# Lagrange-Labs/mapreduce-plonky2

Measured on AMD Instinct MI355X. Metric: leaf proofs/sec (whole node) + NTT GB/s vs HBM peak, 2^20-row table build, 1/2/4/8 GPU, higher is better.
Workload: dtype u64 (Goldilocks field)

## Files before the change

mapreduce-plonky2_amd/csrc/fri.hip:

```cpp
#include "fri.h"
#include "poseidon_wave.cuh"

namespace mp2g {

template <int V>
__device__ void ch_duplex(ChState& c) {
  for (u32 i = 0; i < c.n_in; i++) c.state[i] = c.in[i];
  c.n_in = 0;
  u64 s[12];
#pragma unroll
  for (int i = 0; i < 12; i++) s[i] = c.state[i];
  perm<V>(s);
#pragma unroll
  for (int i = 0; i < 12; i++) c.state[i] = s[i];
#pragma unroll
  for (int i = 0; i < 8; i++) c.out[i] = s[i];
  c.n_out = 8;
}
template <int V>
__global__ void ch_kernel(ChState* st, u32 B, const u64* obs, u64 obs_bstride, u32 n_obs, u64* out, u64 out_bstride, u32 n_get) {
  u32 b = blockIdx.x * blockDim.x + threadIdx.x;
  if (b >= B) return;
  ChState c = st[b];
  const u64* o = obs + b * obs_bstride;
  for (u32 i = 0; i < n_obs; i++) {
    c.n_out = 0;
    c.in[c.n_in++] = o[i];
    if (c.n_in == 8) ch_duplex<V>(c);
  }
  u64* dst = out + b * out_bstride;
  for (u32 i = 0; i < n_get; i++) {
    if (c.n_in || !c.n_out) ch_duplex<V>(c);
    dst[i] = c.out[--c.n_out];
  }
  st[b] = c;
}
__global__ void __launch_bounds__(64) ch_wave_kernel(ChState* st, u32 B, const u64* obs, u64 obs_bstride, u32 n_obs, u64* out,
                                                     u64 out_bstride, u32 n_get) {
  const u32 gid = blockIdx.x * blockDim.x + threadIdx.x;
  const u32 braw = gid >> 4, l = gid & 15;
  const bool active = braw < B;
  const u32 b = active ? braw : B - 1;
  ChState* c = st + b;
  u64 x = l < 12 ? c->state[l] : 0;
  u64 inb = l < 8 ? c->in[l] : 0, outb = l < 8 ? c->out[l] : 0;
  u32 n_in = c->n_in, n_out = c->n_out;
  const u64* o = obs + b * obs_bstride;
  auto duplex = [&]() {
    if (l < n_in) x = inb;
    n_in = 0;
    x = wp2_perm(x, (int)l);
    outb = x;
    n_out = 8;
  };
  for (u32 i = 0; i < n_obs; i++) {
    u64 e = o[i];
    n_out = 0;
    if (l == n_in) inb = e;
    if (++n_in == 8) duplex();
  }
  u64* dst = out + b * out_bstride;
  for (u32 i = 0; i < n_get; i++) {
    if (n_in || !n_out) duplex();
    --n_out;
    if (active && l == n_out) dst[i] = outb;
  }
  if (!active) return;
  if (l < 12) c->state[l] = x;
  if (l < 8) { c->in[l] = inb; c->out[l] = outb; }
  if (l == 0) { c->n_in = n_in; c->n_out = n_out; }
}
__global__ void ch_init_kernel(ChState* st, u32 B) {
  u32 b = blockIdx.x * blockDim.x + threadIdx.x;
  if (b >= B) return;
  ChState c;
  for (int i = 0; i < 12; i++) c.state[i] = 0;
  for (int i = 0; i < 8; i++) { c.in[i] = 0; c.out[i] = 0; }
  c.n_in = c.n_out = 0;
  st[b] = c;
}
hipError_t challenger_init(hipStream_t s, ChState* st, u32 B) {
  hipLaunchKernelGGL(ch_init_kernel, dim3((B + 63) / 64), dim3(64), 0, s, st, B);
  return hipGetLastError();
}
hipError_t challenger_step(hipStream_t s, int variant, ChState* st, u32 B, const u64* obs, u64 obs_bstride, u32 n_obs,
                           u64* out, u64 out_bstride, u32 n_get) {
  if (variant == MP2G_POSEIDON2)
    hipLaunchKernelGGL(ch_wave_kernel, dim3((B * 16 + 63) / 64), dim3(64), 0, s, st, B, obs, obs_bstride, n_obs, out, out_bstride, n_get);
  else
    hipLaunchKernelGGL((ch_kernel<MP2G_POSEIDON>), dim3((B + 63) / 64), dim3(64), 0, s, st, B, obs, obs_bstride, n_obs, out, out_bstride, n_get);
  return hipGetLastError();
}

#define EP_RUN 16
__global__ void __launch_bounds__(256) ext_powers_kernel(const u64* __restrict__ x, u64 x_bstride, u64 scale, u32 count,
                                                         u64* __restrict__ out, u64 out_bstride) {
  const u32 b = blockIdx.y, e0 = blockIdx.x * 256 * EP_RUN + threadIdx.x;
  if (e0 >= count) return;
  const gl2 xb = gl2_scale(gl2_make(x[b * x_bstride], x[b * x_bstride + 1]), scale);
  const gl2 step = gl2_pow(xb, 256);
  gl2 pw = gl2_pow(xb, e0);
  u64* o = out + b * out_bstride;
  for (u32 r = 0, e = e0; r < EP_RUN && e < count; r++, e += 256) {
    o[e] = pw.a;
    o[count + e] = pw.b;
    pw = gl2_mul(pw, step);
  }
}
static hipError_t ext_powers(hipStream_t s, u32 B, const u64* x, u64 x_bstride, u64 scale, u32 count, u64* out, u64 out_bstride) {
  hipLaunchKernelGGL(ext_powers_kernel, dim3((count + 256 * EP_RUN - 1) / (256 * EP_RUN), B), dim3(256), 0, s, x, x_bstride, scale, count, out,
                     out_bstride);
  return hipGetLastError();
}

#define OP_POLYS 4
__global__ void __launch_bounds__(256) openings_kernel(FriShape sh, const u64* __restrict__ zpw, u64 zpw_bstride, u64* out ) {
  const u32 b = blockIdx.y, t = threadIdx.x;
  const u32 n = 1u << sh.log_n, n_open = sh.n_polys + sh.zs_count + sh.lookup_count;
  const u32 blocks0 = (sh.n_polys + OP_POLYS - 1) / OP_POLYS;
  const bool shifted = blockIdx.x >= blocks0;
  const u32 j0 = shifted ? sh.n_polys + (blockIdx.x - blocks0) * OP_POLYS : blockIdx.x * OP_POLYS;
  const u32 nq = min(OP_POLYS, (shifted ? n_open : sh.n_polys) - j0);
  const u64* pa = zpw + b * zpw_bstride + (shifted ? 2 * (u64)n : 0);
  const u64* pb = pa + n;
  const u64* c[OP_POLYS];
#pragma unroll
  for (u32 q = 0; q < OP_POLYS; q++) {
    u32 o, p;
    const u32 j = j0 + (q < nq ? q : 0);
    if (shifted) fri_batch_poly(sh, 1, j - sh.n_polys, o, p);
    else fri_batch_poly(sh, 0, j, o, p);
    c[q] = sh.o[o].coeffs + b * sh.o[o].coeff_bstride + ((u64)p << sh.log_n);
  }
  gl_cols sa[OP_POLYS], sb[OP_POLYS];
  for (u32 i = t; i < n; i += 256) {
    const u64 za = pa[i], zb = pb[i];
#pragma unroll
    for (u32 q = 0; q < OP_POLYS; q++)
      if (q < nq) {
        const u64 v = c[q][i];
        sa[q].add(v, za);
        sb[q].add(v, zb);
      }
  }
  __shared__ u64 ra[OP_POLYS][256], rb[OP_POLYS][256];
#pragma unroll
  for (u32 q = 0; q < OP_POLYS; q++) { ra[q][t] = sa[q].value(); rb[q][t] = sb[q].value(); }
  __syncthreads();
  for (u32 s = 128; s > 0; s >>= 1) {
    if (t < s)
#pragma unroll
      for (u32 q = 0; q < OP_POLYS; q++) { ra[q][t] = gl_add(ra[q][t], ra[q][t + s]); rb[q][t] = gl_add(rb[q][t], rb[q][t + s]); }
    __syncthreads();
  }
  if (t < nq) {
    u64* d = out + ((u64)b * n_open + j0 + t) * 2;
    d[0] = ra[t][0]; d[1] = rb[t][0];
  }
}

__global__ void __launch_bounds__(256) compose_kernel(FriShape sh, const u64* __restrict__ apw, u64 apw_bstride, u32 apw_len, u64* comp) {
  const u32 n = 1u << sh.log_n;
  const u32 i = blockIdx.x * 256 + threadIdx.x, b = blockIdx.y, batch = blockIdx.z;
  if (i >= n) return;
  const u64* pa = apw + b * apw_bstride;
  const u64* pb = pa + apw_len;
  gl_cols sa, sb;
  u32 m = 0;
  const u32 zo = sh.zs_oracle, wz = sh.o[zo].w - sh.lookup_count;
  auto run = [&](u32 o, u32 first, u32 count) {
    const u64* base = sh.o[o].coeffs + b * sh.o[o].coeff_bstride + i;
    for (u32 p = first; p < first + count; p++, m++) {
      const u64 v = base[(u64)p << sh.log_n];
      sa.add(v, pa[m]);
      sb.add(v, pb[m]);
    }
  };
  if (batch == 0) {
    for (u32 o = 0; o < sh.n_oracles; o++) run(o, 0, o == zo ? wz : sh.o[o].w);
  } else {
    run(zo, 0, sh.zs_count);
  }
  if (sh.lookup_count) run(zo, wz, sh.lookup_count);
  u64* d = comp + (((u64)b * 2 + batch) * 2) * n;
  d[i] = sa.value();
  d[n + i] = sb.value();
}

__global__ void __launch_bounds__(1024) divide_kernel(u32 log_n, const u64* zeta, u64 zeta_bstride, const u64* comp, u64* quot) {
  const u32 n = 1u << log_n, batch = blockIdx.x, b = blockIdx.y, t = threadIdx.x;
  const u32 T = n < 1024 ? n : 1024, S = n / T;
  gl2 z = gl2_make(zeta[b * zeta_bstride], zeta[b * zeta_bstride + 1]);
  if (batch == 1) z = gl2_scale(z, gl_root_of_unity(log_n));
  const u64* c0 = comp + (((u64)b * 2 + batch) * 2) * n;
  const u64* c1 = c0 + n;
  u64* q0 = quot + (((u64)b * 2 + batch) * 2) * n;
  u64* q1 = q0 + n;
  __shared__ u64 la[1024], lb[1024];
  gl2 L = gl2_make(0, 0);
  if (t < T) {
    for (int k = (int)S - 1; k >= 0; k--) {
      L = gl2_mul(L, z);
      L.a = gl_add(L.a, c0[t * S + k]);
      L.b = gl_add(L.b, c1[t * S + k]);
    }
  }
  la[t] = 0; lb[t] = 0;
  __syncthreads();
  if (t < T && t >= 1) { la[t - 1] = L.a; lb[t - 1] = L.b; }
  __syncthreads();
  gl2 zp = gl2_pow(z, S);
  for (u32 d = 1; d < T; d <<= 1) {
    gl2 add = gl2_make(0, 0);
    if (t + d < T) add = gl2_mul(zp, gl2_make(la[t + d], lb[t + d]));
    __syncthreads();
    if (t < T) { la[t] = gl_add(la[t], add.a); lb[t] = gl_add(lb[t], add.b); }
    __syncthreads();
    zp = gl2_mul(zp, zp);
  }
  if (t < T) {
    gl2 s = gl2_make(la[t], lb[t]);
    for (int k = (int)S - 1; k >= 0; k--) {
      u32 i = t * S + k;
      s = gl2_mul(s, z);
      s.a = gl_add(s.a, c0[i]);
      s.b = gl_add(s.b, c1[i]);
      if (i >= 1) { q0[i - 1] = s.a; q1[i - 1] = s.b; }
    }
    if (t == T - 1) { q0[n - 1] = 0; q1[n - 1] = 0; }
  }
}
__global__ void __launch_bounds__(256) combine_kernel(u32 log_n, u32 zs_count, const u64* __restrict__ apw, u64 apw_bstride, u32 apw_len,
                                                      const u64* quot, u64* final_poly) {
  const u32 n = 1u << log_n, i = blockIdx.x * 256 + threadIdx.x, b = blockIdx.y;
  if (i >= n) return;
  const gl2 sh = gl2_make(apw[b * apw_bstride + zs_count], apw[b * apw_bstride + apw_len + zs_count]);
  const u64* q = quot + (u64)b * 4 * n;
  gl2 r = gl2_add(gl2_mul(gl2_make(q[i], q[n + i]), sh), gl2_make(q[2 * n + i], q[3 * n + i]));
  final_poly[(u64)b * 2 * n + i] = r.a;
  final_poly[(u64)b * 2 * n + n + i] = r.b;
}

template <int AB>
__global__ void __launch_bounds__(256) fold_values_kernel(u32 log_m, const u64* in, u64 in_bstride, u64* out, u64 out_bstride,
                                                            const u64* beta, u64 beta_bstride, u64 shift_inv, u64 w_m_inv, u64 arity_inv) {
  constexpr int A = 1 << AB;
  const u32 m = 1u << log_m, chunks = m >> AB;
  const u32 c = blockIdx.x * 256 + threadIdx.x, b = blockIdx.y;
  if (c >= chunks) return;
  const u64* v0 = in + b * in_bstride + ((u64)c << AB);
  const u64* v1 = v0 + m;
  gl2 x[A];
#pragma unroll
  for (int k = 0; k < A; k++) x[k] = gl2_make(v0[k], v1[k]);
  const u64 wA_inv = gl_pow(w_m_inv, m >> AB);
#pragma unroll
  for (int s = 1; s <= AB; s++) {
    const int mm = 1 << s, h = mm >> 1;
    u64 wstep = wA_inv;
    for (int e = s; e < AB; e++) wstep = gl_sqr(wstep);
    u64 w = 1;
#pragma unroll
    for (int j = 0; j < h; j++) {
#pragma unroll
      for (int k = 0; k < A; k += mm) {
        gl2 t = j == 0 ? x[k + j + h] : gl2_scale(x[k + j + h], w);
        gl2 u = x[k + j];
        x[k + j] = gl2_add(u, t);
        x[k + j + h] = gl2_sub(u, t);
      }
      w = gl_mul(w, wstep);
    }
  }
  u64 x0_inv = gl_mul(shift_inv, gl_pow(w_m_inv, bitrev32(c, log_m - AB)));
  gl2 g = gl2_scale(gl2_make(beta[b * beta_bstride], beta[b * beta_bstride + 1]), x0_inv);
  gl2 acc = x[A - 1];
#pragma unroll
  for (int j = A - 2; j >= 0; j--) acc = gl2_add(gl2_mul(acc, g), x[j]);
  acc = gl2_scale(acc, arity_inv);
  u64* o = out + b * out_bstride;
  o[c] = acc.a;
  o[chunks + c] = acc.b;
}
__global__ void __launch_bounds__(256) fold_coeffs_kernel(u32 n_out, u32 ab, const u64* in, u64 in_bstride, u32 n_in, u64* out, u64 out_bstride,
                                                            const u64* beta, u64 beta_bstride, int aos_out) {
  const u32 i = blockIdx.x * 256 + threadIdx.x, b = blockIdx.y;
  if (i >= n_out) return;
  const u32 A = 1u << ab;
  const u64* c0 = in + b * in_bstride + ((u64)i << ab);
  const u64* c1 = c0 + n_in;
  gl2 be = gl2_make(beta[b * beta_bstride], beta[b * beta_bstride + 1]);
  gl2 acc = gl2_make(0, 0);
  for (int j = (int)A - 1; j >= 0; j--) acc = gl2_add(gl2_mul(acc, be), gl2_make(c0[j], c1[j]));
  u64* o = out + b * out_bstride;
  if (aos_out) { o[2 * i] = acc.a; o[2 * i + 1] = acc.b; }
  else { o[i] = acc.a; o[n_out + i] = acc.b; }
}
__global__ void soa_to_aos_kernel(u32 n, const u64* in, u64 in_bstride, u32 n_in, u64* out, u64 out_bstride) {
  const u32 i = blockIdx.x * blockDim.x + threadIdx.x, b = blockIdx.y;
  if (i >= n) return;
  out[b * out_bstride + 2 * i] = in[b * in_bstride + i];
  out[b * out_bstride + 2 * i + 1] = in[b * in_bstride + n_in + i];
}

#define POW_THREADS 256
#define POW_STRIDE 16
template <int V>
__global__ void __launch_bounds__(POW_THREADS) pow_kernel(const ChState* st, u32 bits, unsigned long long* witness) {
  const u32 b = blockIdx.y;
  const ChState& c = st[b];
  unsigned long long* wit = witness + (u64)b * POW_STRIDE;
  __shared__ unsigned long long s_best;
  u64 base[12];
#pragma unroll
  for (int i = 0; i < 12; i++) base[i] = c.state[i];
  const u32 pos = c.n_in;
#pragma unroll
  for (int i = 0; i < 8; i++)
    if ((u32)i < pos) base[i] = c.in[i];
  const u64 stride = (u64)gridDim.x * blockDim.x;
  for (u64 cand = (u64)blockIdx.x * blockDim.x + threadIdx.x;; cand += stride) {
    if (threadIdx.x == 0) s_best = atomicMin(wit, ~0ull);
    __syncthreads();
    const unsigned long long best = s_best;
    __syncthreads();
    if (cand - threadIdx.x > best) break;
    u64 s[12];
#pragma unroll
    for (int i = 0; i < 12; i++) s[i] = base[i];
#pragma unroll
    for (int i = 0; i < 8; i++)
      if ((u32)i == pos) s[i] = cand;
    perm<V>(s);
    if (cand < GL_P && (bits == 0 || (s[7] >> (64 - bits)) == 0)) atomicMin(wit, (unsigned long long)cand);
  }
}
__global__ void fill_u64_kernel(u64* p, u64 v, u32 n) {
  u32 i = blockIdx.x * blockDim.x + threadIdx.x;
  if (i < n) p[i] = v;
}

__global__ void __launch_bounds__(256) query_kernel(FriShape sh, FriLayers ly, FriProofLayout L, const u64* chal ,
                                                      u64 chal_bstride, u64* proof) {
  const u32 q = blockIdx.x, b = blockIdx.y, t = threadIdx.x;
  const u32 lg = L.lg;
  const u64 N = (u64)1 << lg;
  u64 x = chal[b * chal_bstride + q] % N;
  u64* const qs = proof + b * L.proof_words + L.q_off + q * L.q_words;
  auto siblings = [&](u64* o, const u64* lv, u32 clg, u32 n_sib, u64 x) {
    for (u32 e = t; e < n_sib * 4; e += 256) {
      u32 l = e >> 2, k = e & 3;
      u64 off = 0;
      for (u32 j = 0; j < l; j++) off += (u64)4 << (clg - j);
      o[e] = lv[off + 4 * ((x >> l) ^ 1) + k];
    }
  };
  for (u32 oi = 0; oi < sh.n_oracles; oi++) {
    const OracleRef& r = sh.o[oi];
    u64* o = qs + L.leaf_off[oi];
    const u64* vals = r.values + b * r.value_bstride;
    for (u32 p = t; p < r.w; p += 256) o[p] = vals[(u64)p * N + x];
    siblings(o + r.w, r.levels + b * r.level_bstride, lg, L.n_sib[oi], x);
  }
  u32 clg = lg;
  for (u32 li = 0; li < ly.n_layers; li++) {
    const u32 ab = ly.arity_bits[li], A = 1u << ab, p = sh.n_oracles + li;
    const u64 m = (u64)1 << clg;
    x >>= ab;
    clg -= ab;
    u64* o = qs + L.leaf_off[p];
    const u64* v = ly.values[li] + b * ly.value_bstride[li];
    for (u32 e = t; e < 2 * A; e += 256) o[e] = v[(e & 1) * m + (x << ab) + (e >> 1)];
    siblings(o + 2 * A, ly.levels[li] + b * ly.level_bstride[li], clg, L.n_sib[p], x);
  }
}
__global__ void copy_rows_kernel(const u64* src, u64 src_bstride, u64* dst, u64 dst_bstride, u32 words) {
  u32 i = blockIdx.x * blockDim.x + threadIdx.x, b = blockIdx.y;
  if (i < words) dst[b * dst_bstride + i] = src[b * src_bstride + i];
}

__global__ void bind_pi_kernel(u64* wires, u64 wires_bstride, u64 n, u32 row, const u64* pi_hash, u32 B) {
  u32 t = blockIdx.x * blockDim.x + threadIdx.x;
  if (t < 4 * B) wires[(t >> 2) * wires_bstride + (u64)(t & 3) * n + row] = pi_hash[t];
}

#define HIPCHK(x) do { hipError_t e_ = (x); if (e_ != hipSuccess) return e_; } while (0)

hipError_t fri_openings(hipStream_t s, const FriShape& sh, u32 B, const u64* zeta, u64 zeta_bstride, u64* zpw, u64* out) {
  const u32 n = 1u << sh.log_n, n_shifted = sh.zs_count + sh.lookup_count;
  HIPCHK(ext_powers(s, B, zeta, zeta_bstride, 1, n, zpw, 4 * (u64)n));
  if (n_shifted) HIPCHK(ext_powers(s, B, zeta, zeta_bstride, gl_root_of_unity(sh.log_n), n, zpw + 2 * (u64)n, 4 * (u64)n));
  const u32 blocks = (sh.n_polys + OP_POLYS - 1) / OP_POLYS + (n_shifted + OP_POLYS - 1) / OP_POLYS;
  hipLaunchKernelGGL(openings_kernel, dim3(blocks, B), dim3(256), 0, s, sh, zpw, 4 * (u64)n, out);
  return hipGetLastError();
}
hipError_t fri_final_poly(hipStream_t s, const FriShape& sh, u32 B, const u64* alpha, u64 alpha_bstride, const u64* zeta, u64 zeta_bstride,
                          u64* apw, u64* comp, u64* quot, u64* final_poly) {
  const u32 n = 1u << sh.log_n, apw_len = fri_alpha_powers_len(sh);
  HIPCHK(ext_powers(s, B, alpha, alpha_bstride, 1, apw_len, apw, 2 * (u64)apw_len));
  hipLaunchKernelGGL(compose_kernel, dim3((n + 255) / 256, B, 2), dim3(256), 0, s, sh, apw, 2 * (u64)apw_len, apw_len, comp);
  hipLaunchKernelGGL(divide_kernel, dim3(2, B), dim3(1024), 0, s, sh.log_n, zeta, zeta_bstride, comp, quot);
  hipLaunchKernelGGL(combine_kernel, dim3((n + 255) / 256, B), dim3(256), 0, s, sh.log_n, sh.zs_count + sh.lookup_count, apw, 2 * (u64)apw_len,
                     apw_len, quot, final_poly);
  return hipGetLastError();
}
hipError_t fri_fold_values(hipStream_t s, u32 B, u32 log_m, u32 ab, const u64* in, u64 in_bstride, u64* out, u64 out_bstride,
                           const u64* beta, u64 beta_bstride, u64 shift) {
  const u32 chunks = (1u << log_m) >> ab;
  const u64 shift_inv = gl_inv(shift), w_m_inv = gl_inv(gl_root_of_unity(log_m)), a_inv = gl_inv((u64)1 << ab);
  dim3 g((chunks + 255) / 256, B), bl(256);
#define FV(N) case N: hipLaunchKernelGGL((fold_values_kernel<N>), g, bl, 0, s, log_m, in, in_bstride, out, out_bstride, beta, beta_bstride, shift_inv, w_m_inv, a_inv); break;
  switch (ab) { FV(1) FV(2) FV(3) FV(4) default: return hipErrorInvalidValue; }
#undef FV
  return hipGetLastError();
}
hipError_t fri_fold_coeffs(hipStream_t s, u32 B, u32 n_in, u32 ab, const u64* in, u64 in_bstride, u64* out, u64 out_bstride,
                           const u64* beta, u64 beta_bstride, bool aos_out) {
  const u32 n_out = n_in >> ab;
  hipLaunchKernelGGL(fold_coeffs_kernel, dim3((n_out + 255) / 256, B), dim3(256), 0, s, n_out, ab, in, in_bstride, n_in, out, out_bstride, beta, beta_bstride, aos_out ? 1 : 0);
  return hipGetLastError();
}
hipError_t fri_soa_to_aos(hipStream_t s, u32 B, u32 n, const u64* in, u64 in_bstride, u32 n_in, u64* out, u64 out_bstride) {
  hipLaunchKernelGGL(soa_to_aos_kernel, dim3((n + 255) / 256, B), dim3(256), 0, s, n, in, in_bstride, n_in, out, out_bstride);
  return hipGetLastError();
}
hipError_t fri_pow(hipStream_t s, int variant, const ChState* st, u32 B, u32 bits, u64* witness) {
  hipLaunchKernelGGL(fill_u64_kernel, dim3((B * POW_STRIDE + 63) / 64), dim3(64), 0, s, witness, ~(u64)0, B * POW_STRIDE);
  const u32 lanes = 1u << 19;
  u32 blocks = lanes / POW_THREADS / (B ? B : 1);
  if (blocks < 8) blocks = 8;
  if (blocks > 1024) blocks = 1024;
  dim3 g(blocks, B), bl(POW_THREADS);
  if (variant == MP2G_POSEIDON2) hipLaunchKernelGGL((pow_kernel<MP2G_POSEIDON2>), g, bl, 0, s, st, bits, (unsigned long long*)witness);
  else hipLaunchKernelGGL((pow_kernel<MP2G_POSEIDON>), g, bl, 0, s, st, bits, (unsigned long long*)witness);
  return hipGetLastError();
}
hipError_t fri_queries(hipStream_t s, const FriShape& sh, const FriLayers& ly, const FriProofLayout& L, u32 B, u32 num_queries,
                       const u64* chal, u64 chal_bstride, u64* proof) {
  if (!num_queries) return hipSuccess;
  hipLaunchKernelGGL(query_kernel, dim3(num_queries, B), dim3(256), 0, s, sh, ly, L, chal, chal_bstride, proof);
  return hipGetLastError();
}
hipError_t bind_public_inputs(hipStream_t s, u32 B, u64* wires, u64 wires_bstride, u64 n, u32 row, const u64* pi_hash) {
  hipLaunchKernelGGL(bind_pi_kernel, dim3((4 * B + 63) / 64), dim3(64), 0, s, wires, wires_bstride, n, row, pi_hash, B);
  return hipGetLastError();
}
hipError_t copy_rows(hipStream_t s, u32 B, const u64* src, u64 src_bstride, u64* dst, u64 dst_bstride, u32 words) {
  if (!words) return hipSuccess;
  hipLaunchKernelGGL(copy_rows_kernel, dim3((words + 255) / 256, B), dim3(256), 0, s, src, src_bstride, dst, dst_bstride, words);
  return hipGetLastError();
}
}
```

mapreduce-plonky2_amd/csrc/gates.h:

```cpp
#pragma once
#include "gl.cuh"
#include "mp2g.h"
namespace mp2g {
struct GateTable {
  u32 n_gates, num_selectors;
  u32 num_lookup_selectors;
  mp2g_gate g[MP2G_MAX_GATES];
};
const char* gate_table_check(const GateTable& t, u32 num_constants, u32 wires_w);
u32 gate_num_constraints(const mp2g_gate& g);
u32 gate_degree(const mp2g_gate& g);
inline u32 gate_filtered_degree(const mp2g_gate& g, u32 num_selectors) {
  return gate_degree(g) + (g.group_end - g.group_start - 1) + (num_selectors > 1 ? 1 : 0);
}
inline const char* gate_table_make(const mp2g_gate* gates, u32 n_gates, u32 num_selectors, u32 num_lookup_selectors, u32 num_constants,
                                   u32 wires_w, GateTable& out, u32* max_j) {
  out = GateTable{};
  out.n_gates = n_gates; out.num_selectors = num_selectors; out.num_lookup_selectors = num_lookup_selectors;
  u32 mj = 0;
  for (u32 i = 0; i < n_gates; i++) {
    out.g[i] = gates[i];
    const u32 k = gate_num_constraints(gates[i]);
    if (k > mj) mj = k;
  }
  if (max_j) *max_j = mj;
  return n_gates ? gate_table_check(out, num_constants, wires_w) : nullptr;
}
hipError_t gate_constraints_lde(hipStream_t s, u32 B, const GateTable& t, const u64* C, const u64* W, u64 w_bstride, u32 lg,
                                const u64* apw, u32 nc, const u64* pi_hash, u64* q);
hipError_t alpha_powers(hipStream_t s, u32 B, const u64* alphas, u64 al_bstride, u32 nc, u64* apw);
hipError_t gate_constraints_points(hipStream_t s, const GateTable& t, const u64* consts, const u64* wires, u64 npts, u32 max_j,
                                   const u64* pi_hash, u64* out);
hipError_t gate_constraints_points_batch(hipStream_t s, u32 B, const GateTable& t, const u64* consts, u64 c_bstride, const u64* wires,
                                         u64 w_bstride, u32 npts, u32 max_j, const u64* pi_hash, u64* out);
hipError_t gate_check(hipStream_t s, u32 B, const GateTable& t, const u64* consts, const u64* wires, u64 w_bstride, u64 npts,
                      const u64* pi_hash, u32* flags);
}
```

mapreduce-plonky2_amd/csrc/gates.hip:

```cpp
#include "gates.h"
#include "poseidon.cuh"
#include "coset_constants.h"

namespace mp2g {

u32 gate_num_constraints(const mp2g_gate& g) {
  switch (g.kind) {
    case MP2G_GATE_CONSTANT: return g.p0;
    case MP2G_GATE_PUBLIC_INPUT: return 4;
    case MP2G_GATE_ARITHMETIC: return g.p0;
    case MP2G_GATE_BASE_SUM: return 1 + g.p0;
    case MP2G_GATE_ARITHMETIC_EXT: case MP2G_GATE_MUL_EXT: return 2 * g.p0;
    case MP2G_GATE_POSEIDON2: case MP2G_GATE_POSEIDON: return 1 + 4 + 36 + 22 + 48 + 12;
    case MP2G_GATE_POSEIDON_MDS: return 24;
    case MP2G_GATE_COSET_INTERPOLATION: return 4 + 4 * (((1u << g.p0) - 2) / (g.p1 - 1));
    case MP2G_GATE_U32_ARITHMETIC: return 36 * g.p0;
    case MP2G_GATE_U32_RANGE_CHECK: return 17 * g.p0;
    case MP2G_GATE_U32_SUBTRACTION: return 19 * g.p0;
    case MP2G_GATE_U32_ADD_MANY: return 21 * g.p1;
    case MP2G_GATE_COMPARISON: return g.p1 ? 6 + 5 * g.p1 + (g.p0 + g.p1 - 1) / g.p1 : 0;
    case MP2G_GATE_EXPONENTIATION: return g.p0 + 1;
    case MP2G_GATE_REDUCING: case MP2G_GATE_REDUCING_EXT: return 2 * g.p0;
    case MP2G_GATE_RANDOM_ACCESS: return (g.p0 + 2) * g.p1 + g.p2;
    case MP2G_GATE_U32_INTERLEAVE: return 34 * g.p0;
    case MP2G_GATE_UNINTERLEAVE_TO_B32: case MP2G_GATE_UNINTERLEAVE_TO_U32: return 67 * g.p0;
    default: return 0;
  }
}
u32 gate_degree(const mp2g_gate& g) {
  switch (g.kind) {
    case MP2G_GATE_CONSTANT: case MP2G_GATE_PUBLIC_INPUT: return 1;
    case MP2G_GATE_ARITHMETIC: case MP2G_GATE_ARITHMETIC_EXT: case MP2G_GATE_MUL_EXT: return 3;
    case MP2G_GATE_BASE_SUM: return g.p1;
    case MP2G_GATE_POSEIDON2: case MP2G_GATE_POSEIDON: return 7;
    case MP2G_GATE_POSEIDON_MDS: return 1;
    case MP2G_GATE_COSET_INTERPOLATION: return g.p1;
    case MP2G_GATE_U32_ARITHMETIC: case MP2G_GATE_U32_RANGE_CHECK: case MP2G_GATE_U32_SUBTRACTION: case MP2G_GATE_U32_ADD_MANY: return 4;
    case MP2G_GATE_COMPARISON: return g.p1 ? 1u << ((g.p0 + g.p1 - 1) / g.p1) : 0;
    case MP2G_GATE_EXPONENTIATION: return 4;
    case MP2G_GATE_REDUCING: case MP2G_GATE_REDUCING_EXT: return 2;
    case MP2G_GATE_RANDOM_ACCESS: return g.p0 + 1;
    case MP2G_GATE_U32_INTERLEAVE: case MP2G_GATE_UNINTERLEAVE_TO_B32: case MP2G_GATE_UNINTERLEAVE_TO_U32: return 2;
    default: return 0;
  }
}
static void gate_footprint(const mp2g_gate& g, u32& wires, u32& consts) {
  wires = 0; consts = 0;
  switch (g.kind) {
    case MP2G_GATE_CONSTANT: wires = g.p0; consts = g.p0; break;
    case MP2G_GATE_PUBLIC_INPUT: wires = 4; break;
    case MP2G_GATE_ARITHMETIC: wires = 4 * g.p0; consts = 2; break;
    case MP2G_GATE_BASE_SUM: wires = 1 + g.p0; break;
    case MP2G_GATE_ARITHMETIC_EXT: wires = 8 * g.p0; consts = 2; break;
    case MP2G_GATE_MUL_EXT: wires = 6 * g.p0; consts = 1; break;
    case MP2G_GATE_POSEIDON2: case MP2G_GATE_POSEIDON: wires = 135; break;
    case MP2G_GATE_POSEIDON_MDS: wires = 48; break;
    case MP2G_GATE_COSET_INTERPOLATION: wires = 1 + 2 * (1u << g.p0) + 6 + 4 * (((1u << g.p0) - 2) / (g.p1 - 1)); break;
    case MP2G_GATE_U32_ARITHMETIC: wires = 38 * g.p0; break;
    case MP2G_GATE_U32_RANGE_CHECK: wires = 17 * g.p0; break;
    case MP2G_GATE_U32_SUBTRACTION: wires = 21 * g.p0; break;
    case MP2G_GATE_U32_ADD_MANY: wires = (g.p0 + 3 + 18) * g.p1; break;
    case MP2G_GATE_COMPARISON: wires = g.p1 ? 4 + 5 * g.p1 + (g.p0 + g.p1 - 1) / g.p1 + 1 : 0; break;
    case MP2G_GATE_EXPONENTIATION: wires = 2 * g.p0 + 2; break;
    case MP2G_GATE_REDUCING: wires = 6 + g.p0 + 2 * (g.p0 - 1); break;
    case MP2G_GATE_REDUCING_EXT: wires = 6 + 2 * g.p0 + 2 * (g.p0 - 1); break;
    case MP2G_GATE_RANDOM_ACCESS: wires = (2 + (1u << g.p0)) * g.p1 + g.p2 + g.p0 * g.p1; consts = g.p2; break;
    case MP2G_GATE_LOOKUP: wires = 2 * g.p0; break;
    case MP2G_GATE_LOOKUP_TABLE: wires = 3 * g.p0; break;
    case MP2G_GATE_U32_INTERLEAVE: wires = 34 * g.p0; break;
    case MP2G_GATE_UNINTERLEAVE_TO_B32: case MP2G_GATE_UNINTERLEAVE_TO_U32: wires = 67 * g.p0; break;
    default: break;
  }
}
const char* gate_table_check(const GateTable& t, u32 num_constants, u32 wires_w) {
  if (t.n_gates > MP2G_MAX_GATES) return "too many gates";
  if (t.num_selectors == 0 || t.num_selectors > num_constants) return "num_selectors must be in 1..num_constants";
  for (u32 i = 0; i < t.n_gates; i++) {
    const mp2g_gate& g = t.g[i];
    if (g.kind > MP2G_GATE_UNINTERLEAVE_TO_U32) return "unknown gate kind";
    if (g.kind >= MP2G_GATE_LOOKUP && g.p0 < 1) return "gate needs at least one slot / operation";
    if ((g.kind == MP2G_GATE_U32_ARITHMETIC || g.kind == MP2G_GATE_U32_RANGE_CHECK || g.kind == MP2G_GATE_U32_SUBTRACTION) && g.p0 < 1)
      return "u32 gate needs at least one operation";
    if (g.kind == MP2G_GATE_U32_ADD_MANY && (g.p0 < 1 || g.p0 > 16 || g.p1 < 1)) return "U32AddManyGate needs 1..16 addends and an operation";
    if (g.kind == MP2G_GATE_COMPARISON && (g.p1 < 1 || g.p0 < g.p1 || (g.p0 + g.p1 - 1) / g.p1 > 4))
      return "ComparisonGate needs num_chunks >= 1 and chunks of at most 4 bits";
    if (g.kind == MP2G_GATE_COSET_INTERPOLATION && (g.p0 < 2 || g.p0 > 5 || g.p1 < 2 || g.p1 > (1u << g.p0)))
      return "CosetInterpolationGate needs 2..5 subgroup bits and 2 <= degree <= 2^bits";
    if (g.kind == MP2G_GATE_BASE_SUM && (g.p1 < 2 || g.p0 < 1)) return "BaseSumGate needs base >= 2 and a limb";
    if ((g.kind == MP2G_GATE_REDUCING || g.kind == MP2G_GATE_REDUCING_EXT || g.kind == MP2G_GATE_EXPONENTIATION) && g.p0 < 1)
      return "gate needs at least one coefficient / power bit";
    if (g.kind == MP2G_GATE_RANDOM_ACCESS && (g.p0 < 1 || g.p0 > 6 || g.p1 < 1)) return "RandomAccessGate needs 1..6 bits and a copy";
    u32 w, c;
    gate_footprint(g, w, c);
    if (w > wires_w) return "gate needs more wires than the wires oracle has";
    if (t.num_selectors + t.num_lookup_selectors + c > num_constants) return "gate needs more constants than the preprocessed oracle has";
    if (g.selector_index >= t.num_selectors) return "selector_index out of range";
    if (!(g.group_start <= i && i < g.group_end && g.group_end <= t.n_gates)) return "gate is not inside its selector group";
    if (gate_num_constraints(g) > MP2G_MAX_GATE_CONSTRAINTS) return "gate has too many constraints";
  }
  return nullptr;
}

struct Alg { u64 a, b; };
GLD Alg alg_mul_addw(Alg x, Alg y, u64 y7, Alg z) {
  return Alg{gl_mul_addw(x.a, y.a, gl_mul_addw(x.b, y7, z.a)), gl_mul_addw(x.a, y.b, gl_mul_addw(x.b, y.a, z.b))};
}
GLD Alg alg_mulw(Alg x, Alg y, u64 y7) { return Alg{gl_mul_addw(x.a, y.a, gl_mulw(x.b, y7)), gl_mul_addw(x.a, y.b, gl_mulw(x.b, y.a))}; }
GLD Alg alg_scale_addw(Alg x, u64 s, Alg z) { return Alg{gl_mul_addw(x.a, s, z.a), gl_mul_addw(x.b, s, z.b)}; }

GLD u64 gl_subw(u64 a, u64 b) {
  u64 r;
  bool br = __builtin_sub_overflow(a, b, &r);
  return r - (br ? GL_EPS : 0);
}
typedef gl_cols LazySum;
template <int BITS, class WireF, class Emit>
GLD void ra_copy(WireF& wire, Emit& emit, u32 w0, u32 b0) {
  constexpr int VS = 1 << BITS;
  u64 bit[BITS], items[VS];
#pragma unroll
  for (int i = 0; i < BITS; i++) bit[i] = wire(b0 + i);
#pragma unroll
  for (int k = 0; k < VS; k++) items[k] = wire(w0 + 2 + k);
  const u64 access = wire(w0), claimed = wire(w0 + 1);
#pragma unroll
  for (int i = 0; i < BITS; i++) emit(gl_mul(bit[i], gl_sub(bit[i], 1)));
  u64 idx = 0;
#pragma unroll
  for (int i = BITS; i-- > 0;) idx = gl_add(gl_add(idx, idx), bit[i]);
  emit(gl_sub(idx, access));
#pragma unroll
  for (int i = 0; i < BITS; i++) {
#pragma unroll
    for (int k = 0; k < (VS >> (i + 1)); k++) items[k] = gl_mul_add(bit[i], gl_sub(items[2 * k + 1], items[2 * k]), items[2 * k]);
  }
  emit(gl_sub(items[0], claimed));
}

template <bool WEAK, class WireF, class ConstF, class Emit>
__device__ __forceinline__ void eval_gate(const mp2g_gate g, WireF wire, ConstF cst, const u64* __restrict__ pih, Emit emit) {
  auto diff = [](u64 s, u64 rc, u64 in) { return WEAK ? gl_subw(gl_addw(s, rc), in) : gl_sub(gl_add(gl_canon(s), rc), in); };
  auto diff0 = [](u64 s, u64 in) { return WEAK ? gl_subw(s, in) : gl_sub(gl_canon(s), in); };
  auto mulx = [](u64 a, u64 b) { return WEAK ? gl_mulw(a, b) : gl_mul(a, b); };
  auto subx = [](u64 a, u64 b) { return WEAK ? gl_subw(a, b) : gl_sub(a, b); };
  auto outx = [](u64 v) { return WEAK ? v : gl_canon(v); };
  auto load16 = [&](u32 first, u32 count, u64(&buf)[16]) {
#pragma unroll
    for (u32 k = 0; k < 16; k++) buf[k] = k < count ? wire(first + k) : 0;
  };
  auto range4 = [&](u64 limb) {
    const u64 z = mulx(limb, gl_sub(limb, 3));
    return mulx(z, WEAK ? gl_addw(z, 2) : gl_add(z, 2));
  };
  auto horner4 = [](u64 acc, u64 limb) {
    if (!WEAK) return gl_add(gl_mul_small(acc, 4), limb);
    return gl_addw(gl_reduce96w(acc << 2, acc >> 62), limb);
  };
  auto emit_alg = [&](Alg d) { emit(outx(d.a)); emit(outx(d.b)); };
  auto alg_subx = [&](Alg x, Alg y) { return Alg{subx(x.a, y.a), subx(x.b, y.b)}; };
  switch (g.kind) {
    case MP2G_GATE_CONSTANT:
      for (u32 i = 0; i < g.p0; i++) emit(subx(cst(i), wire(i)));
      break;
    case MP2G_GATE_PUBLIC_INPUT:
      for (u32 i = 0; i < 4; i++) emit(subx(wire(i), pih[i]));
      break;
    case MP2G_GATE_ARITHMETIC: {
      const u64 n0 = gl_neg(cst(0)), n1 = gl_neg(cst(1));
      u64 lm[16];
      for (u32 i0 = 0; i0 < g.p0; i0 += 4) {
        const u32 cnt = g.p0 - i0 < 4 ? g.p0 - i0 : 4;
        load16(4 * i0, 4 * cnt, lm);
#pragma unroll
        for (u32 k = 0; k < 4; k++)
          if (k < cnt) emit(outx(gl_mul_addw(gl_mulw(lm[4 * k], lm[4 * k + 1]), n0, gl_mul_addw(lm[4 * k + 2], n1, lm[4 * k + 3]))));
      }
      break;
    }
    case MP2G_GATE_BASE_SUM: {
      u64 acc = 0, lm[16];
      for (u32 hi = g.p0; hi > 0;) {
        const u32 lo = hi > 16 ? hi - 16 : 0, cnt = hi - lo;
        load16(1 + lo, cnt, lm);
#pragma unroll
        for (int j = 15; j >= 0; j--)
          if ((u32)j < cnt) acc = gl_addw(gl_mul_small_w(acc, g.p1), lm[j]);
        hi = lo;
      }
      emit(subx(outx(acc), wire(0)));
      for (u32 lo = 0; lo < g.p0; lo += 16) {
        const u32 cnt = g.p0 - lo < 16 ? g.p0 - lo : 16;
        load16(1 + lo, cnt, lm);
#pragma unroll
        for (int j = 0; j < 16; j++) {
          if ((u32)j < cnt) {
            u64 pr = lm[j];
            for (u32 k = 1; k < g.p1; k++) pr = mulx(pr, subx(lm[j], k));
            emit(pr);
          }
        }
      }
      break;
    }
    case MP2G_GATE_ARITHMETIC_EXT: {
      const u64 n0 = gl_neg(cst(0)), n1 = gl_neg(cst(1));
      u64 lm[16];
      for (u32 i0 = 0; i0 < g.p0; i0 += 2) {
        const u32 cnt = g.p0 - i0 < 2 ? g.p0 - i0 : 2;
        load16(8 * i0, 8 * cnt, lm);
#pragma unroll
        for (u32 k = 0; k < 2; k++) {
          if (k < cnt) {
            const u64* w8 = lm + 8 * k;
            Alg m0{w8[0], w8[1]}, m1{w8[2], w8[3]}, ad{w8[4], w8[5]}, o{w8[6], w8[7]};
            emit_alg(alg_scale_addw(alg_mulw(m0, m1, gl_mul_small_w(m1.b, 7)), n0, alg_scale_addw(ad, n1, o)));
          }
        }
      }
      break;
    }
    case MP2G_GATE_MUL_EXT: {
      const u64 n0 = gl_neg(cst(0));
      u64 lm[16];
      for (u32 i0 = 0; i0 < g.p0; i0 += 2) {
        const u32 cnt = g.p0 - i0 < 2 ? g.p0 - i0 : 2;
        load16(6 * i0, 6 * cnt, lm);
#pragma unroll
        for (u32 k = 0; k < 2; k++) {
          if (k < cnt) {
            const u64* w6 = lm + 6 * k;
            Alg m0{w6[0], w6[1]}, m1{w6[2], w6[3]}, o{w6[4], w6[5]};
            emit_alg(alg_scale_addw(alg_mulw(m0, m1, gl_mul_small_w(m1.b, 7)), n0, o));
          }
        }
      }
      break;
    }
    case MP2G_GATE_POSEIDON2: {
      const u64 swap = wire(24);
      emit(gl_mul(swap, gl_sub(swap, 1)));
      u64 s[12];
#pragma unroll
      for (int i = 0; i < 4; i++) {
        u64 lhs = wire(i), rhs = wire(i + 4), delta = wire(25 + i);
        emit(gl_sub(gl_mul(swap, gl_sub(rhs, lhs)), delta));
        s[i] = gl_add(lhs, delta);
        s[i + 4] = gl_sub(rhs, delta);
      }
#pragma unroll
      for (int i = 8; i < 12; i++) s[i] = wire(i);
      p2_external(s);
#pragma unroll 1
      for (int r = 0; r < 4; r++) {
        if (r != 0) {
#pragma unroll
          for (int i = 0; i < 12; i++) {
            u64 in = wire(29 + 12 * (r - 1) + i);
            emit(diff(s[i], c_p2_ext[12 * r + i], in));
            s[i] = p2_sbox(in, 0);
          }
        } else {
#pragma unroll
          for (int i = 0; i < 12; i++) s[i] = p2_sbox(s[i], c_p2_ext[i]);
        }
        p2_external(s);
      }
      u64 nxt = wire(65);
#pragma unroll 1
      for (int r = 0; r < 22; r++) {
        const u64 in = nxt;
        if (r < 21) nxt = wire(65 + r + 1);
        emit(diff(s[0], c_p2_int[r], in));
        s[0] = p2_sbox(in, 0);
        p2_internal(s);
      }
#pragma unroll 1
      for (int r = 0; r < 4; r++) {
#pragma unroll
        for (int i = 0; i < 12; i++) {
          u64 in = wire(87 + 12 * r + i);
          emit(diff(s[i], c_p2_ext[12 * (4 + r) + i], in));
          s[i] = p2_sbox(in, 0);
        }
        p2_external(s);
      }
#pragma unroll
      for (int i = 0; i < 12; i++) emit(diff0(s[i], wire(12 + i)));
      break;
    }
    case MP2G_GATE_POSEIDON: {
      const u64 swap = wire(24);
      emit(gl_mul(swap, gl_sub(swap, 1)));
      u64 s[12];
#pragma unroll
      for (int i = 0; i < 4; i++) {
        u64 lhs = wire(i), rhs = wire(i + 4), delta = wire(25 + i);
        emit(gl_sub(gl_mul(swap, gl_sub(rhs, lhs)), delta));
        s[i] = gl_add(lhs, delta);
        s[i + 4] = gl_sub(rhs, delta);
      }
#pragma unroll
      for (int i = 8; i < 12; i++) s[i] = wire(i);
#pragma unroll 1
      for (int r = 0; r < 30; r++) {
        if (r >= 4 && r < 26) {
          u64 in = wire(65 + (r - 4));
          emit(diff(s[0], c_p_rc[12 * r], in));
          s[0] = p2_sbox(in, 0);
#pragma unroll
          for (int i = 1; i < 12; i++) s[i] = gl_addw(s[i], c_p_rc[12 * r + i]);
        } else if (r == 0) {
#pragma unroll
          for (int i = 0; i < 12; i++) s[i] = p2_sbox(s[i], c_p_rc[i]);
        } else {
          const int base = r < 4 ? 29 + 12 * (r - 1) : 87 + 12 * (r - 26);
#pragma unroll
          for (int i = 0; i < 12; i++) {
            u64 in = wire(base + i);
            emit(diff(s[i], c_p_rc[12 * r + i], in));
            s[i] = p2_sbox(in, 0);
          }
        }
        poseidon_mds(s);
      }
#pragma unroll
      for (int i = 0; i < 12; i++) emit(diff0(s[i], wire(12 + i)));
      break;
    }
    case MP2G_GATE_POSEIDON_MDS: {
      u64 s0[12], s1[12];
#pragma unroll
      for (int i = 0; i < 12; i++) { s0[i] = wire(2 * i); s1[i] = wire(2 * i + 1); }
      poseidon_mds(s0);
      poseidon_mds(s1);
#pragma unroll
      for (int i = 0; i < 12; i++) {
        emit(gl_sub(wire(24 + 2 * i), gl_canon(s0[i])));
        emit(gl_sub(wire(25 + 2 * i), gl_canon(s1[i])));
      }
      break;
    }
    case MP2G_GATE_COSET_INTERPOLATION: {
      const u32 npts = 1u << g.p0, deg = g.p1, nint = (npts - 2) / (deg - 1);
      const u32 w_pt = 1 + 2 * npts, w_val = w_pt + 2, w_int = w_val + 2, w_sh = w_int + 4 * nint;
      const Alg pt{wire(w_pt), wire(w_pt + 1)}, sh{wire(w_sh), wire(w_sh + 1)};
      emit_alg(alg_scale_addw(sh, gl_neg(wire(0)), pt));
      const u64 sh7 = gl_mul_small_w(sh.b, 7);
      const u64* xs = COSET_POINTS + MP2G_COSET_TABLE(g.p0);
      const u64* ws = COSET_WEIGHTS + MP2G_COSET_TABLE(g.p0);
      Alg ev{0, 0}, pr{1, 0};
      u32 start = 0, end = deg;
      for (u32 c = 0; c <= nint; c++) {
        for (u32 i = start; i < end; i++) {
          const u64 wi = ws[i];
          const Alg val{gl_mulw(wire(1 + 2 * i), wi), gl_mulw(wire(2 + 2 * i), wi)};
          const Alg term{subx(sh.a, xs[i]), sh.b};
          ev = alg_mul_addw(ev, term, sh7, alg_mulw(val, pr, gl_mul_small_w(pr.b, 7)));
          pr = alg_mulw(pr, term, sh7);
        }
        ev = Alg{gl_canon(ev.a), gl_canon(ev.b)};
        if (c == nint) break;
        pr = Alg{gl_canon(pr.a), gl_canon(pr.b)};
        Alg iev{wire(w_int + 2 * c), wire(w_int + 2 * c + 1)}, ipr{wire(w_int + 2 * (nint + c)), wire(w_int + 2 * (nint + c) + 1)};
        emit(subx(iev.a, ev.a)); emit(subx(iev.b, ev.b)); emit(subx(ipr.a, pr.a)); emit(subx(ipr.b, pr.b));
        ev = iev; pr = ipr;
        start = 1 + (deg - 1) * (c + 1);
        end = start + deg - 1 < npts ? start + deg - 1 : npts;
      }
      emit(subx(wire(w_val), ev.a)); emit(subx(wire(w_val + 1), ev.b));
      break;
    }
    case MP2G_GATE_U32_ARITHMETIC: {
      const u32 ops = g.p0;
      for (u32 i = 0; i < ops; i++) {
        const u32 b = 6 * i;
        const u64 computed = gl_mul_add(wire(b), wire(b + 1), wire(b + 2));
        const u64 lo = wire(b + 3), hi = wire(b + 4), inv = wire(b + 5);
        const u64 hi_not_max = gl_sub(gl_mul(inv, gl_sub(0xFFFFFFFFull, hi)), 1);
        emit(gl_mul(hi_not_max, lo));
        emit(gl_sub(gl_mul_add(hi, (u64)1 << 32, lo), computed));
        u64 clo = 0, chi = 0, lm[16];
        load16(6 * ops + 32 * i + 16, 16, lm);
#pragma unroll
        for (int j = 15; j >= 0; j--) { emit(range4(lm[j])); chi = horner4(chi, lm[j]); }
        load16(6 * ops + 32 * i, 16, lm);
#pragma unroll
        for (int j = 15; j >= 0; j--) { emit(range4(lm[j])); clo = horner4(clo, lm[j]); }
        emit(subx(clo, lo));
        emit(subx(chi, hi));
      }
      break;
    }
    case MP2G_GATE_U32_RANGE_CHECK: {
      const u32 k = g.p0;
      for (u32 i = 0; i < k; i++) {
        u64 lm[16];
        load16(k + 16 * i, 16, lm);
        u64 acc = 0;
#pragma unroll
        for (int j = 15; j >= 0; j--) acc = horner4(acc, lm[j]);
        emit(subx(acc, wire(i)));
#pragma unroll
        for (int j = 0; j < 16; j++) emit(range4(lm[j]));
      }
      break;
    }
    case MP2G_GATE_U32_SUBTRACTION: {
      const u32 ops = g.p0;
      for (u32 i = 0; i < ops; i++) {
        const u32 b = 5 * i;
        const u64 initial = gl_sub(gl_sub(wire(b), wire(b + 1)), wire(b + 2));
        const u64 res = wire(b + 3), bo = wire(b + 4);
        emit(gl_sub(res, gl_add(initial, gl_mul((u64)1 << 32, bo))));
        u64 comb = 0, lm[16];
        load16(5 * ops + 16 * i, 16, lm);
#pragma unroll
        for (int j = 15; j >= 0; j--) { emit(range4(lm[j])); comb = horner4(comb, lm[j]); }
        emit(subx(comb, res));
        emit(gl_mul(bo, gl_sub(1, bo)));
      }
      break;
    }
    case MP2G_GATE_U32_ADD_MANY: {
      const u32 na = g.p0, ops = g.p1, per = na + 3;
      for (u32 i = 0; i < ops; i++) {
        const u32 b = per * i;
        u64 computed = wire(b + na);
        for (u32 j = 0; j < na; j++) computed = gl_add(computed, wire(b + j));
        const u64 res = wire(b + na + 1), co = wire(b + na + 2);
        emit(gl_sub(gl_mul_add(co, (u64)1 << 32, res), computed));
        u64 cres = 0, ccar = 0, lm[16];
        {
          const u64 l17 = wire(per * ops + 18 * i + 17), l16 = wire(per * ops + 18 * i + 16);
          load16(per * ops + 18 * i, 16, lm);
          emit(range4(l17)); ccar = l17;
          emit(range4(l16)); ccar = horner4(ccar, l16);
        }
#pragma unroll
        for (int j = 15; j >= 0; j--) { emit(range4(lm[j])); cres = horner4(cres, lm[j]); }
        emit(subx(cres, res));
        emit(subx(ccar, co));
      }
      break;
    }
    case MP2G_GATE_COMPARISON: {
      const u32 nch = g.p1, cb = (g.p0 + nch - 1) / nch, cs = 1u << cb;
      const u32 o_fc = 4, o_sc = 4 + nch, o_ed = 4 + 2 * nch, o_ce = 4 + 3 * nch, o_iv = 4 + 4 * nch, o_bits = 4 + 5 * nch;
      u64 a1 = 0, a2 = 0;
      for (u32 i = nch; i-- > 0;) { a1 = gl_add(gl_mul_small(a1, cs), wire(o_fc + i)); a2 = gl_add(gl_mul_small(a2, cs), wire(o_sc + i)); }
      emit(gl_sub(a1, wire(0)));
      emit(gl_sub(a2, wire(1)));
      u64 msd = 0;
      for (u32 i = 0; i < nch; i++) {
        const u64 f = wire(o_fc + i), sc = wire(o_sc + i), ce = wire(o_ce + i), iv = wire(o_iv + i);
        u64 p1 = f, p2 = sc;
        for (u32 x = 1; x < cs; x++) { p1 = mulx(p1, gl_sub(f, x)); p2 = mulx(p2, gl_sub(sc, x)); }
        emit(p1);
        emit(p2);
        const u64 diff = gl_sub(sc, f);
        emit(gl_sub(gl_mul(diff, wire(o_ed + i)), gl_sub(1, ce)));
        emit(gl_mul(ce, diff));
        emit(gl_sub(iv, gl_mul(ce, msd)));
        msd = gl_add(iv, gl_mul(gl_sub(1, ce), diff));
      }
      const u64 msd_w = wire(3);
      emit(gl_sub(msd_w, msd));
      u64 bc = 0;
      for (u32 i = cb + 1; i-- > 0;) bc = gl_add(gl_add(bc, bc), wire(o_bits + i));
      for (u32 i = 0; i <= cb; i++) { const u64 bit = wire(o_bits + i); emit(gl_mul(bit, gl_sub(1, bit))); }
      emit(gl_sub(gl_add(cs, msd_w), bc));
      emit(gl_sub(wire(2), wire(o_bits + cb)));
      break;
    }
    case MP2G_GATE_EXPONENTIATION: {
      const u32 nb = g.p0;
      const u64 base = wire(0);
      u64 prev_int = 1;
      for (u32 i = 0; i < nb; i++) {
        u64 prev = i == 0 ? 1 : gl_mul(prev_int, prev_int);
        u64 bit = wire(1 + (nb - 1 - i));
        u64 mulby = gl_mul_add(bit, base, gl_sub(1, bit));
        u64 cur = wire(nb + 2 + i);
        emit(gl_sub(gl_mul(prev, mulby), cur));
        prev_int = cur;
      }
      emit(gl_sub(wire(nb + 1), prev_int));
      break;
    }
    case MP2G_GATE_REDUCING:
    case MP2G_GATE_REDUCING_EXT: {
      const u32 n = g.p0;
      const bool ext = g.kind == MP2G_GATE_REDUCING_EXT;
      const u32 start_accs = 6 + (ext ? 2 * n : n);
      Alg alpha{wire(2), wire(3)}, acc{wire(4), wire(5)};
      const u64 alpha7 = gl_mul_small_w(alpha.b, 7);
      for (u32 i = 0; i < n; i++) {
        Alg coeff = ext ? Alg{wire(6 + 2 * i), wire(7 + 2 * i)} : Alg{wire(6 + i), 0};
        Alg nxt = i == n - 1 ? Alg{wire(0), wire(1)} : Alg{wire(start_accs + 2 * i), wire(start_accs + 2 * i + 1)};
        emit_alg(alg_mul_addw(acc, alpha, alpha7, alg_subx(coeff, nxt)));
        acc = nxt;
      }
      break;
    }
    case MP2G_GATE_RANDOM_ACCESS: {
      const u32 bits = g.p0, copies = g.p1, extra = g.p2, vs = 1u << bits;
      const u32 routed = (2 + vs) * copies + extra;
      for (u32 c = 0; c < copies; c++) {
        const u32 w0 = (2 + vs) * c, b0 = routed + c * bits;
        switch (bits) {
          case 1: ra_copy<1>(wire, emit, w0, b0); break;
          case 2: ra_copy<2>(wire, emit, w0, b0); break;
          case 3: ra_copy<3>(wire, emit, w0, b0); break;
          case 4: ra_copy<4>(wire, emit, w0, b0); break;
          default: {
            u64 items[32];
            for (u32 i = 0; i < bits; i++) {
              u64 b = wire(b0 + i);
              emit(gl_mul(b, gl_sub(b, 1)));
            }
            u64 idx = 0;
            for (u32 i = bits; i-- > 0;) idx = gl_add(gl_add(idx, idx), wire(b0 + i));
            emit(gl_sub(idx, wire(w0)));
            {
              const u64 b = wire(b0);
              for (u32 k = 0; k < vs / 2; k++) {
                u64 x = wire(w0 + 2 + 2 * k), y = wire(w0 + 3 + 2 * k);
                items[k] = gl_mul_add(b, gl_sub(y, x), x);
              }
            }
            for (u32 i = 1, len = vs / 2; i < bits; i++, len >>= 1) {
              const u64 b = wire(b0 + i);
              for (u32 k = 0; k < len / 2; k++) items[k] = gl_mul_add(b, gl_sub(items[2 * k + 1], items[2 * k]), items[2 * k]);
            }
            emit(gl_sub(items[0], wire(w0 + 1)));
          }
        }
      }
      for (u32 i = 0; i < extra; i++) emit(gl_sub(cst(i), wire((2 + vs) * copies + i)));
      break;
    }
    case MP2G_GATE_U32_INTERLEAVE: {
      const u32 ops = g.p0;
      u64 bt[16];
      for (u32 i = 0; i < ops; i++) {
        u64 x = 0, xi = 0;
        for (u32 h = 0; h < 2; h++) {
          load16(2 * ops + 32 * i + 16 * h, 16, bt);
#pragma unroll
          for (int j = 0; j < 16; j++) {
            emit(mulx(bt[j], gl_sub(1, bt[j])));
            x = gl_add(gl_add(x, x), bt[j]);
            xi = gl_add(gl_mul_small(xi, 4), bt[j]);
          }
        }
        emit(gl_sub(x, wire(2 * i)));
        emit(gl_sub(xi, wire(2 * i + 1)));
      }
      break;
    }
    case MP2G_GATE_UNINTERLEAVE_TO_B32:
    case MP2G_GATE_UNINTERLEAVE_TO_U32: {
      const u32 ops = g.p0;
      const bool spread = g.kind == MP2G_GATE_UNINTERLEAVE_TO_B32;
      u64 bt[16];
      for (u32 i = 0; i < ops; i++) {
        u64 x = 0, ev = 0, od = 0;
        for (u32 h = 0; h < 4; h++) {
          load16(3 * ops + 64 * i + 16 * h, 16, bt);
#pragma unroll
          for (int j = 0; j < 16; j++) {
            emit(mulx(bt[j], gl_sub(1, bt[j])));
            x = gl_add(gl_add(x, x), bt[j]);
            u64& d = (j & 1) ? ev : od;
            d = gl_add(spread ? gl_mul_small(d, 4) : gl_add(d, d), bt[j]);
          }
        }
        emit(gl_sub(x, wire(3 * i)));
        emit(gl_sub(ev, wire(3 * i + 1)));
        emit(gl_sub(od, wire(3 * i + 2)));
      }
      break;
    }
    default: break;
  }
}

template <class ConstAll>
GLD u64 gate_filter(const GateTable& t, u32 gi, ConstAll call) {
  const mp2g_gate& g = t.g[gi];
  const u64 s = call(g.selector_index);
  u64 f = 1;
  for (u32 r = g.group_start; r < g.group_end; r++)
    if (r != gi) f = gl_mul(f, gl_sub(r, s));
  if (t.num_selectors > 1) f = gl_mul(f, gl_sub(0xFFFFFFFFull, s));
  return f;
}

template <u32 KIND>
__global__ void __launch_bounds__(256) gate_constraints_lde_kernel(mp2g_gate g, u32 gi, u32 num_selectors, u32 cst_off, u32 n_cons,
                                                                   const u64* __restrict__ C, const u64* __restrict__ W,
                                                                   u64 w_bstride, u32 lg, const u64* __restrict__ apw_tab,
                                                                   u32 nc, const u64* __restrict__ pi_hash,
                                                                   u64* __restrict__ q, int first) {
  __shared__ u64 apw[2][MP2G_MAX_GATE_CONSTRAINTS];
  const u64 N = (u64)1 << lg;
  const u32 p = blockIdx.x * 256 + threadIdx.x, b = blockIdx.y;
  for (u32 j = threadIdx.x; j < 2 * n_cons; j += 256) {
    const u32 a = j >= n_cons ? 1 : 0, e = j - a * n_cons;
    apw[a][e] = apw_tab[((u64)b * 2 + a) * MP2G_MAX_GATE_CONSTRAINTS + e];
  }
  __syncthreads();
  if (p >= N) return;
  g.kind = KIND;
  const u64* w = W + b * w_bstride + p;
  const u64* c = C + p;
  const u64* pih = pi_hash + 4 * b;
  auto wire = [&](u32 j) { return w[(u64)j << lg]; };
  auto cst = [&](u32 j) { return c[(u64)(cst_off + j) << lg]; };
  u64 f = 1;
  {
    const u64 s = c[(u64)g.selector_index << lg];
    for (u32 r = g.group_start; r < g.group_end; r++)
      if (r != gi) f = gl_mul(f, gl_sub(r, s));
    if (num_selectors > 1) f = gl_mul(f, gl_sub(0xFFFFFFFFull, s));
  }
  LazySum acc[2];
  u32 j = 0;
  eval_gate<true>(g, wire, cst, pih, [&](u64 v) {
#pragma unroll
    for (u32 a = 0; a < 2; a++) acc[a].add(v, apw[a][j]);
    j++;
  });
  const u32 i = bitrev32(p, lg);
  for (u32 a = 0; a < nc; a++) {
    u64 r = gl_mul(f, acc[a].value());
    u64* dst = q + (((u64)b * nc + a) << lg) + i;
    *dst = first ? r : gl_add(*dst, r);
  }
}

#define MP2G_MAX_LIGHT_GATES 12
struct LightGates {
  u32 n;
  mp2g_gate g[MP2G_MAX_LIGHT_GATES];
  u32 gi[MP2G_MAX_LIGHT_GATES];
};
static bool gate_is_light(const mp2g_gate& g) {
  switch (g.kind) {
    case MP2G_GATE_CONSTANT: case MP2G_GATE_PUBLIC_INPUT: case MP2G_GATE_ARITHMETIC: case MP2G_GATE_BASE_SUM:
    case MP2G_GATE_ARITHMETIC_EXT: case MP2G_GATE_MUL_EXT: return true;
    default: return false;
  }
}
__global__ void __launch_bounds__(256) gate_constraints_lde_light_kernel(LightGates lg_, u32 num_selectors, u32 cst_off, u32 max_cons,
                                                                         const u64* __restrict__ C, const u64* __restrict__ W,
                                                                         u64 w_bstride, u32 lg, const u64* __restrict__ apw_tab,
                                                                         u32 nc, const u64* __restrict__ pi_hash,
                                                                         u64* __restrict__ q, int first) {
  __shared__ u64 apw[2][MP2G_MAX_GATE_CONSTRAINTS];
  const u64 N = (u64)1 << lg;
  const u32 p = blockIdx.x * 256 + threadIdx.x, b = blockIdx.y;
  for (u32 j = threadIdx.x; j < 2 * max_cons; j += 256) {
    const u32 a = j >= max_cons ? 1 : 0, e = j - a * max_cons;
    apw[a][e] = apw_tab[((u64)b * 2 + a) * MP2G_MAX_GATE_CONSTRAINTS + e];
  }
  __syncthreads();
  if (p >= N) return;
  const u64* w = W + b * w_bstride + p;
  const u64* c = C + p;
  const u64* pih = pi_hash + 4 * b;
  auto wire = [&](u32 j) { return w[(u64)j << lg]; };
  auto cst = [&](u32 j) { return c[(u64)(cst_off + j) << lg]; };
  u64 total[2] = {0, 0};
  for (u32 k = 0; k < lg_.n; k++) {
    mp2g_gate g = lg_.g[k];
    const u32 gi = lg_.gi[k];
    u64 f = 1;
    {
      const u64 s = c[(u64)g.selector_index << lg];
      for (u32 r = g.group_start; r < g.group_end; r++)
        if (r != gi) f = gl_mul(f, gl_sub(r, s));
      if (num_selectors > 1) f = gl_mul(f, gl_sub(0xFFFFFFFFull, s));
    }
    LazySum acc[2];
    u32 j = 0;
    auto emit = [&](u64 v) {
#pragma unroll
      for (u32 a = 0; a < 2; a++) acc[a].add(v, apw[a][j]);
      j++;
    };
    switch (g.kind) {
#define LIGHT_CASE(K) case K: g.kind = K; eval_gate<true>(g, wire, cst, pih, emit); break;
      LIGHT_CASE(MP2G_GATE_CONSTANT)
      LIGHT_CASE(MP2G_GATE_PUBLIC_INPUT)
      LIGHT_CASE(MP2G_GATE_ARITHMETIC)
      LIGHT_CASE(MP2G_GATE_BASE_SUM)
      LIGHT_CASE(MP2G_GATE_ARITHMETIC_EXT)
      LIGHT_CASE(MP2G_GATE_MUL_EXT)
#undef LIGHT_CASE
      default: break;
    }
    for (u32 a = 0; a < nc; a++) total[a] = gl_add(total[a], gl_mul(f, acc[a].value()));
  }
  const u32 i = bitrev32(p, lg);
  for (u32 a = 0; a < nc; a++) {
    u64* dst = q + (((u64)b * nc + a) << lg) + i;
    *dst = first ? total[a] : gl_add(*dst, total[a]);
  }
}

__global__ void __launch_bounds__(256) gate_constraints_points_kernel(GateTable t, const u64* __restrict__ consts,
                                                                      const u64* __restrict__ wires, u64 npts, u32 max_j,
                                                                      const u64* __restrict__ pih, u64* __restrict__ out) {
  const u64 p = (u64)blockIdx.x * 256 + threadIdx.x;
  if (p >= npts) return;
  auto wire = [&](u32 j) { return wires[(u64)j * npts + p]; };
  auto call = [&](u32 j) { return consts[(u64)j * npts + p]; };
  const u32 ns = t.num_selectors + t.num_lookup_selectors;
  auto cst = [&](u32 j) { return consts[(u64)(ns + j) * npts + p]; };
  for (u32 j = 0; j < max_j; j++) out[(u64)j * npts + p] = 0;
  for (u32 gi = 0; gi < t.n_gates; gi++) {
    if (t.g[gi].kind == MP2G_GATE_NOOP) continue;
    const u64 f = gate_filter(t, gi, call);
    u32 j = 0;
    eval_gate<false>(t.g[gi], wire, cst, pih, [&](u64 v) {
      u64* o = out + (u64)j * npts + p;
      *o = gl_add(*o, gl_mul(f, v));
      j++;
    });
  }
}

__global__ void __launch_bounds__(256) gate_constraints_points_batch_kernel(GateTable t, u32 B, const u64* __restrict__ consts, u64 c_bstride,
                                                                            const u64* __restrict__ wires, u64 w_bstride, u32 npts,
                                                                            u32 max_j, const u64* __restrict__ pih, u64* __restrict__ out) {
  const u32 idx = blockIdx.x * 256 + threadIdx.x;
  if (idx >= B * npts) return;
  const u32 b = idx / npts, p = idx % npts;
  const u64* cb = consts + b * c_bstride;
  const u64* wb = wires + b * w_bstride;
  u64* ob = out + (u64)b * max_j * npts;
  auto wire = [&](u32 j) { return wb[(u64)j * npts + p]; };
  auto call = [&](u32 j) { return cb[(u64)j * npts + p]; };
  const u32 ns = t.num_selectors + t.num_lookup_selectors;
  auto cst = [&](u32 j) { return cb[(u64)(ns + j) * npts + p]; };
  for (u32 j = 0; j < max_j; j++) ob[(u64)j * npts + p] = 0;
  for (u32 gi = 0; gi < t.n_gates; gi++) {
    if (t.g[gi].kind == MP2G_GATE_NOOP) continue;
    const u64 f = gate_filter(t, gi, call);
    u32 j = 0;
    eval_gate<false>(t.g[gi], wire, cst, pih + 4 * b, [&](u64 v) {
      u64* o = ob + (u64)j * npts + p;
      *o = gl_add(*o, gl_mul(f, v));
      j++;
    });
  }
}

__global__ void __launch_bounds__(256) gate_check_kernel(GateTable t, const u64* __restrict__ consts, const u64* __restrict__ wires,
                                                         u64 w_bstride, u64 npts, const u64* __restrict__ pi_hash, u32* __restrict__ flags) {
  const u64 p = (u64)blockIdx.x * 256 + threadIdx.x;
  const u32 b = blockIdx.y;
  if (p >= npts) return;
  const u64* w = wires + b * w_bstride;
  auto wire = [&](u32 j) { return w[(u64)j * npts + p]; };
  auto call = [&](u32 j) { return consts[(u64)j * npts + p]; };
  const u32 ns = t.num_selectors + t.num_lookup_selectors;
  auto cst = [&](u32 j) { return consts[(u64)(ns + j) * npts + p]; };
  bool bad = false;
  for (u32 gi = 0; gi < t.n_gates; gi++) {
    if (t.g[gi].kind == MP2G_GATE_NOOP) continue;
    if (gate_filter(t, gi, call) == 0) continue;
    eval_gate<false>(t.g[gi], wire, cst, pi_hash + 4 * b, [&](u64 v) { bad |= v != 0; });
  }
  if (bad) atomicOr(&flags[b], 2u);
}
hipError_t gate_check(hipStream_t s, u32 B, const GateTable& t, const u64* consts, const u64* wires, u64 w_bstride, u64 npts,
                      const u64* pi_hash, u32* flags) {
  if (!npts || !B) return hipSuccess;
  hipLaunchKernelGGL(gate_check_kernel, dim3((u32)((npts + 255) / 256), B), dim3(256), 0, s, t, consts, wires, w_bstride, npts, pi_hash,
                     flags);
  return hipGetLastError();
}

__global__ void alpha_powers_kernel(const u64* __restrict__ alphas, u64 al_bstride, u32 nc, u32 B, u64* __restrict__ apw) {
  const u32 t = blockIdx.x * blockDim.x + threadIdx.x;
  if (t >= B * 2 * MP2G_MAX_GATE_CONSTRAINTS) return;
  const u32 e = t % MP2G_MAX_GATE_CONSTRAINTS, a = (t / MP2G_MAX_GATE_CONSTRAINTS) & 1, b = t / (2 * MP2G_MAX_GATE_CONSTRAINTS);
  apw[t] = a < nc ? gl_pow(alphas[b * al_bstride + a], e) : 0;
}
hipError_t alpha_powers(hipStream_t s, u32 B, const u64* alphas, u64 al_bstride, u32 nc, u64* apw) {
  if (nc < 1 || nc > 2) return hipErrorInvalidValue;
  const u32 total = B * 2 * MP2G_MAX_GATE_CONSTRAINTS;
  hipLaunchKernelGGL(alpha_powers_kernel, dim3((total + 255) / 256), dim3(256), 0, s, alphas, al_bstride, nc, B, apw);
  return hipGetLastError();
}

hipError_t gate_constraints_lde(hipStream_t s, u32 B, const GateTable& t, const u64* C, const u64* W, u64 w_bstride, u32 lg,
                                const u64* apw, u32 nc, const u64* pi_hash, u64* q) {
  if (nc < 1 || nc > 2) return hipErrorInvalidValue;
  const u64 N = (u64)1 << lg;
  const dim3 grid((u32)((N + 255) / 256), B), block(256);
  int first = 1;
  LightGates lgs{};
  u32 light_cons = 0;
  for (u32 gi = 0; gi < t.n_gates; gi++) {
    const u32 n_cons = gate_num_constraints(t.g[gi]);
    if (n_cons && gate_is_light(t.g[gi]) && lgs.n < MP2G_MAX_LIGHT_GATES) {
      lgs.g[lgs.n] = t.g[gi]; lgs.gi[lgs.n] = gi; lgs.n++;
      if (n_cons > light_cons) light_cons = n_cons;
    }
  }
  if (lgs.n < 2) lgs.n = 0;
  if (lgs.n) {
    hipLaunchKernelGGL(gate_constraints_lde_light_kernel, grid, block, 0, s, lgs, t.num_selectors, t.num_selectors + t.num_lookup_selectors,
                       light_cons, C, W, w_bstride, lg, apw, nc, pi_hash, q, first);
    first = 0;
  }
  for (u32 gi = 0; gi < t.n_gates; gi++) {
    const mp2g_gate& g = t.g[gi];
    const u32 n_cons = gate_num_constraints(g);
    if (!n_cons) continue;
    bool fused = false;
    for (u32 k = 0; k < lgs.n; k++) fused |= lgs.gi[k] == gi;
    if (fused) continue;
#define GATE_CASE(K)                                                                                                        \
  case K:                                                                                                                   \
    hipLaunchKernelGGL(gate_constraints_lde_kernel<K>, grid, block, 0, s, g, gi, t.num_selectors,                          \
                       t.num_selectors + t.num_lookup_selectors, n_cons, C, W, w_bstride, lg, apw, nc, pi_hash, q,             \
                       first);                                                                                              \
    break;
    switch (g.kind) {
      GATE_CASE(MP2G_GATE_CONSTANT)
      GATE_CASE(MP2G_GATE_PUBLIC_INPUT)
      GATE_CASE(MP2G_GATE_ARITHMETIC)
      GATE_CASE(MP2G_GATE_BASE_SUM)
      GATE_CASE(MP2G_GATE_ARITHMETIC_EXT)
      GATE_CASE(MP2G_GATE_MUL_EXT)
      GATE_CASE(MP2G_GATE_POSEIDON2)
      GATE_CASE(MP2G_GATE_EXPONENTIATION)
      GATE_CASE(MP2G_GATE_REDUCING)
      GATE_CASE(MP2G_GATE_REDUCING_EXT)
      GATE_CASE(MP2G_GATE_RANDOM_ACCESS)
      GATE_CASE(MP2G_GATE_POSEIDON)
      GATE_CASE(MP2G_GATE_POSEIDON_MDS)
      GATE_CASE(MP2G_GATE_COSET_INTERPOLATION)
      GATE_CASE(MP2G_GATE_U32_ARITHMETIC)
      GATE_CASE(MP2G_GATE_U32_RANGE_CHECK)
      GATE_CASE(MP2G_GATE_U32_SUBTRACTION)
      GATE_CASE(MP2G_GATE_U32_ADD_MANY)
      GATE_CASE(MP2G_GATE_COMPARISON)
      GATE_CASE(MP2G_GATE_U32_INTERLEAVE)
      GATE_CASE(MP2G_GATE_UNINTERLEAVE_TO_B32)
      GATE_CASE(MP2G_GATE_UNINTERLEAVE_TO_U32)
      default: return hipErrorInvalidValue;
    }
#undef GATE_CASE
    first = 0;
  }
  if (first) return hipMemsetAsync(q, 0, (size_t)B * nc * N * sizeof(u64), s);
  return hipGetLastError();
}
hipError_t gate_constraints_points(hipStream_t s, const GateTable& t, const u64* consts, const u64* wires, u64 npts, u32 max_j,
                                   const u64* pi_hash, u64* out) {
  if (!npts) return hipSuccess;
  hipLaunchKernelGGL(gate_constraints_points_kernel, dim3((u32)((npts + 255) / 256)), dim3(256), 0, s, t, consts, wires, npts, max_j,
                     pi_hash, out);
  return hipGetLastError();
}
hipError_t gate_constraints_points_batch(hipStream_t s, u32 B, const GateTable& t, const u64* consts, u64 c_bstride, const u64* wires,
                                         u64 w_bstride, u32 npts, u32 max_j, const u64* pi_hash, u64* out) {
  if (!npts || !B) return hipSuccess;
  hipLaunchKernelGGL(gate_constraints_points_batch_kernel, dim3((B * npts + 255) / 256), dim3(256), 0, s, t, B, consts, c_bstride, wires,
                     w_bstride, npts, max_j, pi_hash, out);
  return hipGetLastError();
}
}
```

mapreduce-plonky2_amd/csrc/gl.cuh:

```cuda
#pragma once
#include <hip/hip_runtime.h>
#include <stdint.h>

typedef uint64_t u64;
typedef uint32_t u32;

#define GL_P 0xFFFFFFFF00000001ULL
#define GL_EPS 0xFFFFFFFFULL
#define GL_MULT_GEN 14293326489335486720ULL
#define GL_TWO_GEN 7277203076849721926ULL

#define GLD __device__ __forceinline__
#define GLHD __host__ __device__ __forceinline__

GLHD u64 gl_mk(u32 lo, u32 hi) { return ((u64)hi << 32) | lo; }
GLHD u64 gl_canon(u64 a) {
  u32 c0, c1;
  u32 t0 = __builtin_addc((u32)a, 0xFFFFFFFFu, 0u, &c0);
  u32 t1 = __builtin_addc((u32)(a >> 32), 0u, c0, &c1);
  return c1 ? gl_mk(t0, t1) : a;
}
GLHD u64 gl_add(u64 a, u64 b) {
  u32 c0, c1, d0, d1;
  u32 s0 = __builtin_addc((u32)a, (u32)b, 0u, &c0);
  u32 s1 = __builtin_addc((u32)(a >> 32), (u32)(b >> 32), c0, &c1);
  u32 t0 = __builtin_addc(s0, 0xFFFFFFFFu, 0u, &d0);
  u32 t1 = __builtin_addc(s1, 0u, d0, &d1);
  return (c1 | d1) ? gl_mk(t0, t1) : gl_mk(s0, s1);
}
GLHD u64 gl_sub(u64 a, u64 b) {
  u32 c0, c1, d0, d1;
  u32 s0 = __builtin_subc((u32)a, (u32)b, 0u, &c0);
  u32 s1 = __builtin_subc((u32)(a >> 32), (u32)(b >> 32), c0, &c1);
  u32 m = c1 ? 0xFFFFFFFFu : 0u;
  u32 t0 = __builtin_subc(s0, m, 0u, &d0);
  u32 t1 = __builtin_subc(s1, 0u, d0, &d1);
  return gl_mk(t0, t1);
}
GLHD u64 gl_neg(u64 a) { return a ? GL_P - a : 0; }
GLHD u64 gl_dbl(u64 a) { return gl_add(a, a); }

GLHD u64 gl_addw(u64 a, u64 b) {
  u32 c0, c1;
  u32 s0 = __builtin_addc((u32)a, (u32)b, 0u, &c0);
  u32 s1 = __builtin_addc((u32)(a >> 32), (u32)(b >> 32), c0, &c1);
#if defined(__HIP_DEVICE_COMPILE__)
  return gl_mk(s0, s1) + (u64)(c1 ? 0xFFFFFFFFu : 0u);
#else
  u32 m = c1 ? 0xFFFFFFFFu : 0u, d0, d1;
  u32 t0 = __builtin_addc(s0, m, 0u, &d0);
  u32 t1 = __builtin_addc(s1, 0u, d0, &d1);
  return gl_mk(t0, t1);
#endif
}
GLHD u64 gl_reduce128w(u64 lo, u64 hi) {
#if defined(__HIP_DEVICE_COMPILE__)
  u32 hl = (u32)hi, hh = (u32)(hi >> 32);
  u64 t, c;
  asm("v_mad_u64_u32 %0, %1, %2, -1, %3" : "=&v"(t), "=s"(c) : "v"(hl), "v"(lo));
  u32 t0 = (u32)t, t1 = (u32)(t >> 32), r0, r1, mb, mc;
  asm("v_sub_co_u32 %0, vcc, %4, %6\n\t"
      "v_subbrev_co_u32 %1, vcc, 0, %5, vcc\n\t"
      "v_subb_co_u32 %2, vcc, %0, %0, vcc\n\t"
      "v_cndmask_b32 %3, 0, -1, %7"
      : "=&v"(r0), "=&v"(r1), "=&v"(mb), "=&v"(mc)
      : "v"(t0), "v"(t1), "v"(hh), "s"(c)
      : "vcc");
  return gl_mk(r0, r1) + gl_mk(mc - mb, mb & ~mc);
#else
  u64 hi_hi = hi >> 32, hi_lo = hi & GL_EPS;
  u64 t0;
  bool b = __builtin_sub_overflow(lo, hi_hi, &t0);
  t0 -= b ? GL_EPS : 0;
  u64 t1 = (hi_lo << 32) - hi_lo;
  u64 r;
  bool c = __builtin_add_overflow(t0, t1, &r);
  return r + (c ? GL_EPS : 0);
#endif
}
GLHD u64 gl_reduce96w(u64 lo, u64 hi) {
#if defined(__HIP_DEVICE_COMPILE__)
  u64 t, c;
  asm("v_mad_u64_u32 %0, %1, %2, -1, %3" : "=&v"(t), "=s"(c) : "v"((u32)hi), "v"(lo));
  u32 m;
  asm("s_nop 1\n\t"
      "v_cndmask_b32 %0, 0, -1, %1" : "=v"(m) : "s"(c));
  return t + (u64)m;
#else
  u64 t1 = (hi << 32) - hi;
  u64 r;
  bool c = __builtin_add_overflow(lo, t1, &r);
  return r + (c ? GL_EPS : 0);
#endif
}
GLHD u64 gl_reduce128(u64 lo, u64 hi) { return gl_canon(gl_reduce128w(lo, hi)); }
GLHD void gl_mul_wide(u64 a, u64 b, u64& lo, u64& hi) {
#if defined(__HIP_DEVICE_COMPILE__)
  u64 a0 = (u32)a, a1 = a >> 32, b0 = (u32)b, b1 = b >> 32;
  u64 p00 = a0 * b0;
  u64 m1 = a0 * b1 + (p00 >> 32);
  u64 m2 = a1 * b0 + (m1 & GL_EPS);
  lo = (m2 << 32) | (p00 & GL_EPS);
  hi = a1 * b1 + (m1 >> 32) + (m2 >> 32);
#else
  unsigned __int128 x = (unsigned __int128)a * b;
  lo = (u64)x;
  hi = (u64)(x >> 64);
#endif
}
GLHD void gl_mul_add_wide(u64 a, u64 b, u64 c, u64& lo, u64& hi) {
#if defined(__HIP_DEVICE_COMPILE__)
  u64 a0 = (u32)a, a1 = a >> 32, b0 = (u32)b, b1 = b >> 32;
  u64 p00 = a0 * b0 + (u64)(u32)c;
  u64 m1 = a0 * b1 + ((p00 >> 32) + (c >> 32));
  u64 m2 = a1 * b0 + (m1 & GL_EPS);
  lo = (m2 << 32) | (p00 & GL_EPS);
  hi = a1 * b1 + (m1 >> 32) + (m2 >> 32);
#else
  unsigned __int128 x = (unsigned __int128)a * b + c;
  lo = (u64)x;
  hi = (u64)(x >> 64);
#endif
}
GLHD u64 gl_mul(u64 a, u64 b) {
  u64 lo, hi;
  gl_mul_wide(a, b, lo, hi);
  return gl_reduce128(lo, hi);
}
GLHD u64 gl_sqr(u64 a) { return gl_mul(a, a); }
GLHD u64 gl_mul_small(u64 a, u32 c) {
  u64 p0 = (u64)(u32)a * c;
  u64 p1 = (a >> 32) * c + (p0 >> 32);
  return gl_canon(gl_reduce96w((p1 << 32) | (p0 & GL_EPS), p1 >> 32));
}
GLHD u64 gl_mul_small_w(u64 a, u32 c) {
  u64 p0 = (u64)(u32)a * c;
  u64 p1 = (a >> 32) * c + (p0 >> 32);
  return gl_reduce96w((p1 << 32) | (p0 & GL_EPS), p1 >> 32);
}
GLHD u64 gl_pow7(u64 x) {
  u64 x2 = gl_sqr(x), x4 = gl_sqr(x2), x3 = gl_mul(x, x2);
  return gl_mul(x3, x4);
}
GLHD u64 gl_pow(u64 b, u64 e) {
  u64 r = 1;
  while (e) {
    if (e & 1) r = gl_mul(r, b);
    b = gl_sqr(b);
    e >>= 1;
  }
  return r;
}
GLHD u64 gl_inv(u64 a) { return gl_pow(a, GL_P - 2); }
GLHD u64 gl_root_of_unity(unsigned k) {
  u64 g = GL_TWO_GEN;
  for (unsigned i = k; i < 32; i++) g = gl_sqr(g);
  return g;
}
GLHD u32 bitrev32(u32 x, unsigned bits) {
#if defined(__HIP_DEVICE_COMPILE__)
  return bits ? (__brev(x) >> (32 - bits)) : 0;
#else
  u32 r = 0;
  for (unsigned i = 0; i < bits; i++) { r = (r << 1) | (x & 1); x >>= 1; }
  return r;
#endif
}

GLHD u64 gl_mul_addw(u64 a, u64 b, u64 c) {
  u64 lo, hi;
  gl_mul_add_wide(a, b, c, lo, hi);
  return gl_reduce128w(lo, hi);
}
GLHD u64 gl_mul_add(u64 a, u64 b, u64 c) { return gl_canon(gl_mul_addw(a, b, c)); }
GLHD u64 gl_mulw(u64 a, u64 b) {
  u64 lo, hi;
  gl_mul_wide(a, b, lo, hi);
  return gl_reduce128w(lo, hi);
}

struct gl_cols {
  u64 c0 = 0, c1 = 0, c2 = 0, c3 = 0;
  GLHD void add(u64 a, u64 b) {
    u64 pl, ph;
    gl_mul_wide(a, b, pl, ph);
    c0 += (u32)pl; c1 += pl >> 32; c2 += (u32)ph; c3 += ph >> 32;
  }
  GLHD void add_scaled(u64 a, u64 b, u32 f) {
    u64 pl, ph;
    gl_mul_wide(a, b, pl, ph);
    c0 += (u64)(u32)pl * f; c1 += (pl >> 32) * f; c2 += (u64)(u32)ph * f; c3 += (ph >> 32) * f;
  }
  GLHD u64 value() const {
    const u64 w1 = c1 + (c0 >> 32), w2 = c2 + (w1 >> 32), w3 = c3 + (w2 >> 32);
    return gl_sub(gl_reduce128(gl_mk((u32)c0, (u32)w1), gl_mk((u32)w2, (u32)w3)), (w3 >> 32) << 32);
  }
};

struct gl2 { u64 a, b; };
GLHD gl2 gl2_make(u64 a, u64 b) { gl2 r; r.a = a; r.b = b; return r; }
GLHD gl2 gl2_add(gl2 x, gl2 y) { return gl2_make(gl_add(x.a, y.a), gl_add(x.b, y.b)); }
GLHD gl2 gl2_sub(gl2 x, gl2 y) { return gl2_make(gl_sub(x.a, y.a), gl_sub(x.b, y.b)); }
GLHD gl2 gl2_mul(gl2 x, gl2 y) {
  return gl2_make(gl_mul_add(x.a, y.a, gl_mul_small_w(gl_mulw(x.b, y.b), 7)), gl_mul_add(x.a, y.b, gl_mulw(x.b, y.a)));
}
GLHD gl2 gl2_scale(gl2 x, u64 s) { return gl2_make(gl_mul(x.a, s), gl_mul(x.b, s)); }
GLHD gl2 gl2_inv(gl2 x) {
  u64 n = gl_sub(gl_sqr(x.a), gl_mul_small(gl_sqr(x.b), 7));
  u64 ni = gl_inv(n);
  return gl2_make(gl_mul(x.a, ni), gl_mul(gl_neg(x.b), ni));
}
GLHD gl2 gl2_pow(gl2 b, u64 e) {
  gl2 r = gl2_make(1, 0);
  while (e) {
    if (e & 1) r = gl2_mul(r, b);
    b = gl2_mul(b, b);
    e >>= 1;
  }
  return r;
}
```

mapreduce-plonky2_amd/csrc/gl5.cuh:

```cuda
#pragma once
#include "gl.cuh"
#include "perm_constants.h"

namespace mp2g {

#if defined(__HIP_DEVICE_COMPILE__)
#define GL5D __device__ __forceinline__
#define GL5N __device__ __noinline__
#else
#define GL5D __host__ __device__ __forceinline__
#define GL5N __host__ __device__ inline
#endif
struct gl5 { u64 c[5]; };

GL5D gl5 gl5_zero() { gl5 r; for (int i = 0; i < 5; i++) r.c[i] = 0; return r; }
GL5D gl5 gl5_from(u64 a) { gl5 r = gl5_zero(); r.c[0] = a; return r; }
GL5D gl5 gl5_make(u64 a, u64 b, u64 c, u64 d, u64 e) { gl5 r; r.c[0] = a; r.c[1] = b; r.c[2] = c; r.c[3] = d; r.c[4] = e; return r; }
GL5D bool gl5_is_zero(const gl5& a) { return (a.c[0] | a.c[1] | a.c[2] | a.c[3] | a.c[4]) == 0; }
GL5D bool gl5_eq(const gl5& a, const gl5& b) {
  bool e = true;
#pragma unroll
  for (int i = 0; i < 5; i++) e = e && a.c[i] == b.c[i];
  return e;
}
GL5D gl5 gl5_add(const gl5& a, const gl5& b) { gl5 r;
#pragma unroll
  for (int i = 0; i < 5; i++) r.c[i] = gl_add(a.c[i], b.c[i]);
  return r; }
GL5D gl5 gl5_sub(const gl5& a, const gl5& b) { gl5 r;
#pragma unroll
  for (int i = 0; i < 5; i++) r.c[i] = gl_sub(a.c[i], b.c[i]);
  return r; }
GL5D gl5 gl5_neg(const gl5& a) { gl5 r;
#pragma unroll
  for (int i = 0; i < 5; i++) r.c[i] = gl_neg(a.c[i]);
  return r; }
GL5D gl5 gl5_dbl(const gl5& a) { return gl5_add(a, a); }
GL5D gl5 gl5_scale(const gl5& a, u64 s) { gl5 r;
#pragma unroll
  for (int i = 0; i < 5; i++) r.c[i] = gl_mul(a.c[i], s);
  return r; }
GL5D gl5 gl5_small(const gl5& a, u32 s) { gl5 r;
#pragma unroll
  for (int i = 0; i < 5; i++) r.c[i] = gl_mul_small(a.c[i], s);
  return r; }
GL5D gl5 gl5_mul_kz(const gl5& a, u32 k) {
  gl5 r;
  r.c[0] = gl_mul_small(a.c[4], 3 * k);
#pragma unroll
  for (int i = 1; i < 5; i++) r.c[i] = gl_mul_small(a.c[i - 1], k);
  return r;
}
GL5N gl5 gl5_mul_limbs(u64 x0, u64 x1, u64 x2, u64 x3, u64 x4, u64 y0, u64 y1, u64 y2, u64 y3, u64 y4) {
  const u64 a[5] = {x0, x1, x2, x3, x4}, b[5] = {y0, y1, y2, y3, y4};
  u64 a3[5];
#pragma unroll
  for (int j = 1; j < 5; j++) a3[j] = gl_mul_small_w(a[j], 3);
  a3[0] = 0;
  gl5 r;
#pragma unroll
  for (int i = 0; i < 5; i++) {
    gl_cols acc;
#pragma unroll
    for (int j = 0; j < 5; j++) {
      if (j <= i) acc.add(a[j], b[i - j]); else acc.add(a3[j], b[i + 5 - j]);
    }
    r.c[i] = acc.value();
  }
  return r;
}
GL5D gl5 gl5_mul(const gl5& a, const gl5& b) {
  return gl5_mul_limbs(a.c[0], a.c[1], a.c[2], a.c[3], a.c[4], b.c[0], b.c[1], b.c[2], b.c[3], b.c[4]);
}
GL5N gl5 gl5_sqr_limbs(u64 x0, u64 x1, u64 x2, u64 x3, u64 x4) {
  const u64 a[5] = {x0, x1, x2, x3, x4};
  gl5 r;
#pragma unroll
  for (int i = 0; i < 5; i++) {
    gl_cols acc;
#pragma unroll
    for (int j = 0; j < 5; j++) {
#pragma unroll
      for (int k = j; k < 5; k++) {
        if ((j + k) % 5 != i) continue;
        const u32 f = (j < k ? 2u : 1u) * (j + k >= 5 ? 3u : 1u);
        if (f == 1) acc.add(a[j], a[k]); else acc.add_scaled(a[j], a[k], f);
      }
    }
    r.c[i] = acc.value();
  }
  return r;
}
GL5D gl5 gl5_sqr(const gl5& a) { return gl5_sqr_limbs(a.c[0], a.c[1], a.c[2], a.c[3], a.c[4]); }
GL5D gl5 gl5_frob1(const gl5& a) {
  return gl5_make(a.c[0], gl_mul(a.c[1], 1041288259238279555ULL), gl_mul(a.c[2], 15820824984080659046ULL),
                  gl_mul(a.c[3], 211587555138949697ULL), gl_mul(a.c[4], 1373043270956696022ULL));
}
GL5D gl5 gl5_frob2(const gl5& a) {
  return gl5_make(a.c[0], gl_mul(a.c[1], 15820824984080659046ULL), gl_mul(a.c[2], 1373043270956696022ULL),
                  gl_mul(a.c[3], 1041288259238279555ULL), gl_mul(a.c[4], 211587555138949697ULL));
}
GL5D u64 gl_sqn(u64 x, int k) {
#pragma unroll 1
  for (int i = 0; i < k; i++) x = gl_sqr(x);
  return x;
}
GL5D void gl_ones(u64 a, u64& o31, u64& o32) {
  u64 x2 = gl_mul(gl_sqr(a), a), x4 = gl_mul(gl_sqn(x2, 2), x2), x8 = gl_mul(gl_sqn(x4, 4), x4);
  u64 x16 = gl_mul(gl_sqn(x8, 8), x8), x24 = gl_mul(gl_sqn(x16, 8), x8), x28 = gl_mul(gl_sqn(x24, 4), x4);
  u64 x30 = gl_mul(gl_sqn(x28, 2), x2);
  o31 = gl_mul(gl_sqr(x30), a);
  o32 = gl_mul(gl_sqr(o31), a);
}
GL5D u64 gl_pow_2_32_m1(u64 a) { u64 o31, o32; gl_ones(a, o31, o32); return o32; }
GL5D u64 gl_inv_chain(u64 a) {
  u64 o31, o32;
  gl_ones(a, o31, o32);
  return gl_mul(gl_sqn(gl_sqr(o31), 32), o32);
}
GL5N gl5 gl5_inv(gl5 a) {
  gl5 f1 = gl5_frob1(a), f2 = gl5_frob2(a);
  gl5 f12 = gl5_mul(f1, f2);
  gl5 f34 = gl5_frob2(f12);
  gl5 q = gl5_mul(f12, f34);
  u64 n = 0;
  {
    gl_cols acc;
    acc.add(a.c[0], q.c[0]);
#pragma unroll
    for (int j = 1; j < 5; j++) acc.add(gl_mul_small_w(a.c[j], 3), q.c[5 - j]);
    n = acc.value();
  }
  return gl5_scale(q, gl_inv_chain(n));
}
GL5D u64 gl5_norm(const gl5& a) {
  gl5 f12 = gl5_mul(gl5_frob1(a), gl5_frob2(a));
  gl5 q = gl5_mul(f12, gl5_frob2(f12));
  return gl5_mul(a, q).c[0];
}
GL5D bool gl_is_square(u64 a) {
  if (a == 0) return true;
  u64 t = gl_pow_2_32_m1(a);
#pragma unroll 1
  for (int i = 0; i < 31; i++) t = gl_sqr(t);
  return t == 1;
}
#if defined(__HIP_DEVICE_COMPILE__)
#define GL_TWO_GEN_POW2_AT(k) GL_TWO_GEN_POW2[k]
#else
inline u64 gl_two_gen_pow2_host(u32 k) {
  u64 g = GL_TWO_GEN;
  for (u32 i = 0; i < k; i++) g = gl_sqr(g);
  return g;
}
#define GL_TWO_GEN_POW2_AT(k) gl_two_gen_pow2_host(k)
#endif
GL5N bool gl_sqrt(u64 a, u64& out) {
  if (a == 0) { out = 0; return true; }
  u64 t = gl_pow_2_32_m1(a);
  u64 chk = t;
#pragma unroll 1
  for (int i = 0; i < 31; i++) chk = gl_sqr(chk);
  if (chk != 1) { out = 0; return false; }
  u64 R = a;
#pragma unroll 1
  for (int i = 0; i < 31; i++) R = gl_sqr(R);
#pragma unroll 1
  while (t != 1) {
    u32 i = 0;
    u64 t2 = t;
    while (t2 != 1) { t2 = gl_sqr(t2); i++; }
    u64 b = GL_TWO_GEN_POW2_AT(31 - i);
    t = gl_mul(t, GL_TWO_GEN_POW2_AT(32 - i));
    R = gl_mul(R, b);
  }
  out = R;
  return true;
}
GL5N bool gl5_sqrt(gl5 x, gl5& out) {
  gl5 v = x;
#pragma unroll 1
  for (int i = 0; i < 31; i++) v = gl5_sqr(v);
  gl5 v32 = v;
#pragma unroll 1
  for (int i = 0; i < 32; i++) v32 = gl5_sqr(v32);
  gl5 d = gl5_mul(gl5_mul(x, v32), gl5_inv(v));
  gl5 e = gl5_frob1(gl5_mul(d, gl5_frob2(d)));
  gl5 f = gl5_sqr(e);
  u64 g = gl5_mul(x, f).c[0];
  u64 s;
  if (!gl_sqrt(g, s)) { out = gl5_zero(); return false; }
  out = gl5_scale(gl5_inv(e), s);
  return true;
}
GL5N bool gl5_is_square(const gl5& x) { return gl_is_square(gl5_norm(x)); }
GL5D bool gl5_sgn0(const gl5& x) {
  bool sign = false, zero = true;
#pragma unroll
  for (int i = 0; i < 5; i++) {
    bool sign_i = (x.c[i] & 1) != 0, zero_i = x.c[i] == 0;
    sign = sign || (zero && sign_i);
    zero = zero && zero_i;
  }
  return sign;
}
}
```

mapreduce-plonky2_amd/csrc/prover.hip:

```cpp
#include "ctx.h"
#include "fri.h"
#include "zperm.h"
#include "gates.h"
#include "lookup.h"
#include "lookup_wires.h"
#include <cstring>
#include <new>
#include <vector>

using namespace mp2g;


struct mp2g_challenger {
  mp2g_ctx* ctx = nullptr;
  int variant = 0;
  uint32_t count = 0;
  DevBuf st;
};

struct mp2g_prover {
  mp2g_ctx* ctx = nullptr;
  mp2g_fri_params P{};
  uint32_t B = 0;
  uint32_t Bcap = 0;
  bool have_pre = false;
  FriProofLayout L{};
  size_t levels_words = 0, n_open = 0;
  DevBuf coeffs[8], values[8], levels[8];
  DevBuf ch, chal, zeta, alpha, betas, comp, quot, final_poly, witness, qchal;
  DevBuf fvals[9], flevels[8], fcoeffs[9];
  DevBuf zpw, fapw;
  uint32_t num_routed = 0, degree = 0;
  bool quotient = false;
  DevBuf pre_values, zs_values, chunk_q, bg, alphas, qvals;
  DevBuf ptab, qtab;
  DevBuf apw;
  GateTable gates{};
  LookupDev lookups{};
  DevBuf lut_tables, lut_eval;
  DevBuf lut_index;
  bool lut_inputs_unique = false;
  int64_t pi_row = -1;
  bool wcheck = false;
  DevBuf wflags;
  bool timing = false;
  hipEvent_t ev[MP2G_N_STAGES + 1] = {};
  bool graph_on = false;
  int plain_calls = 0;
  hipGraphExec_t gexec = nullptr;
  const void* gkey[12] = {};
  u64 ggen = 0;
  void drop_graph() {
    if (gexec) (void)hipGraphExecDestroy(gexec);
    gexec = nullptr;
  }
  std::vector<std::pair<DevBuf*, size_t>> shared;
  const u64* bound_base = nullptr;
  size_t bound_total = 0;
  bool counted = false;
  hipError_t want(DevBuf& d, size_t bytes) {
    if (!ctx->share_scratch) return d.alloc(bytes);
    for (auto& e : shared)
      if (e.first == &d) { e.second = bytes; bound_base = nullptr; return hipSuccess; }
    shared.emplace_back(&d, bytes);
    bound_base = nullptr;
    return hipSuccess;
  }
  ~mp2g_prover() {
    drop_graph();
    for (hipEvent_t e : ev)
      if (e) (void)hipEventDestroy(e);
  }
};
#define STAGE_MARK(pr, i) do { if ((pr)->timing) CK(hipEventRecord((pr)->ev[i], (pr)->ctx->stream)); } while (0)

namespace {
struct ProverGuard {
  mp2g_prover* pr = nullptr;
  ~ProverGuard();
};
template <class F>
hipError_t upload_table(mp2g_ctx* c, DevBuf& d, size_t words, F fill) {
  std::vector<u64> h(words);
  fill(h.data());
  hipError_t e = d.alloc(words * sizeof(u64));
  if (e == hipSuccess) e = hipMemcpyAsync(d.p, h.data(), words * sizeof(u64), hipMemcpyHostToDevice, c->stream);
  if (e == hipSuccess) e = hipStreamSynchronize(c->stream);
  return e;
}
}

namespace mp2g {
int params_check(const mp2g_fri_params* p) {
  NEED(p, "params");
  NEED(p->variant <= 1, "variant");
  NEED(p->log_n >= 1 && p->log_n <= 20, "1 <= log_n <= 20");
  NEED(p->rate_bits >= 1 && p->rate_bits <= 6, "rate_bits");
  NEED(p->n_oracles >= 1 && p->n_oracles <= 8, "n_oracles");
  NEED(p->n_layers <= 8, "n_layers");
  NEED(p->pow_bits <= 32, "pow_bits <= 32");
  NEED(p->num_queries <= 64, "num_queries <= 64");
  NEED(p->zs_oracle < p->n_oracles && p->zs_count <= p->oracle_w[p->zs_oracle], "zs_oracle/zs_count");
  uint32_t deg = p->log_n, lg = p->log_n + p->rate_bits;
  NEED(p->cap_height <= lg, "cap_height");
  for (uint32_t i = 0; i < p->n_layers; i++) {
    NEED(p->arity_bits[i] >= 1 && p->arity_bits[i] <= 4, "arity_bits in 1..4");
    NEED(deg >= p->arity_bits[i], "arity exceeds degree");
    deg -= p->arity_bits[i];
    lg -= p->arity_bits[i];
    NEED(lg >= p->cap_height, "layer smaller than cap");
  }
  for (uint32_t o = 0; o < p->n_oracles; o++) NEED(p->oracle_w[o] >= 1, "oracle_w >= 1");
  NEED(p->num_lookup_polys <= 16, "num_lookup_polys <= 16");
  NEED((uint64_t)p->zs_count * (1 + p->num_lookup_polys) <= p->oracle_w[p->zs_oracle], "Z + lookup polynomials exceed the zs oracle");
  return 0;
}
}

extern "C" {

uint32_t mp2g_reduction_arity_bits(uint32_t degree_bits, uint32_t rate_bits, uint32_t cap_height, uint32_t arity_bits,
                                   uint32_t final_poly_bits, uint32_t* out) {
  uint32_t n = 0;
  if (arity_bits == 0) return 0;
  while (degree_bits > final_poly_bits && degree_bits >= arity_bits && degree_bits + rate_bits >= cap_height + arity_bits && n < 8) {
    out[n++] = arity_bits;
    degree_bits -= arity_bits;
  }
  return n;
}
size_t mp2g_fri_n_openings(const mp2g_fri_params* p) { return opening_layout(*p, 0).n_open; }
size_t mp2g_fri_proof_words(const mp2g_fri_params* p) { return fri_proof_layout(*p).proof_words; }

int mp2g_challenger_create(mp2g_ctx* c, int variant, uint32_t count, mp2g_challenger** out) {
  NEED(c && out && count >= 1, "ctx/out/count");
  NEED(variant == 0 || variant == 1, "variant");
  mp2g_challenger* ch = new (std::nothrow) mp2g_challenger();
  if (!ch) return fail("out of memory");
  ch->ctx = c; ch->variant = variant; ch->count = count;
  hipError_t e = ch->st.alloc(sizeof(ChState) * count);
  if (e == hipSuccess) e = challenger_init(c->stream, (ChState*)ch->st.p, count);
  if (e != hipSuccess) { delete ch; return fail("challenger_create: %s", hipGetErrorString(e)); }
  *out = ch;
  return 0;
}
int mp2g_challenger_observe(mp2g_challenger* ch, const uint64_t* elems, uint32_t n) {
  NEED(ch && (elems || !n), "challenger/elems");
  if (!n) return 0;
  mp2g_ctx* c = ch->ctx;
  DevBuf d;
  CK(d.alloc((size_t)ch->count * n * sizeof(u64)));
  CK(hipMemcpyAsync(d.p, elems, (size_t)ch->count * n * sizeof(u64), hipMemcpyHostToDevice, c->stream));
  CK(challenger_step(c->stream, ch->variant, (ChState*)ch->st.p, ch->count, d.p, n, n, d.p, 0, 0));
  CK(hipStreamSynchronize(c->stream));
  return 0;
}
int mp2g_challenger_get(mp2g_challenger* ch, uint32_t n, uint64_t* out) {
  NEED(ch && (out || !n), "challenger/out");
  if (!n) return 0;
  mp2g_ctx* c = ch->ctx;
  DevBuf d;
  CK(d.alloc((size_t)ch->count * n * sizeof(u64)));
  CK(challenger_step(c->stream, ch->variant, (ChState*)ch->st.p, ch->count, d.p, 0, 0, d.p, n, n));
  CK(hipMemcpyAsync(out, d.p, (size_t)ch->count * n * sizeof(u64), hipMemcpyDeviceToHost, c->stream));
  CK(hipStreamSynchronize(c->stream));
  return 0;
}
void mp2g_challenger_free(mp2g_challenger* ch) {
  if (!ch) return;
  (void)hipStreamSynchronize(ch->ctx->stream);
  delete ch;
}

int mp2g_fri_fold(mp2g_ctx* c, const uint64_t* evals, uint32_t log_m, uint32_t arity_bits, const uint64_t beta[2],
                  uint64_t shift, uint64_t* out) {
  NEED(c && evals && beta && out, "ctx/pointers");
  NEED(arity_bits >= 1 && arity_bits <= 4 && log_m >= arity_bits && log_m <= 28, "arity_bits in 1..4, log_m >= arity_bits");
  NEED(shift != 0 && shift < GL_P, "shift");
  const size_t m = (size_t)1 << log_m, m2 = m >> arity_bits;
  std::vector<u64> soa(2 * m);
  for (size_t i = 0; i < m; i++) { soa[i] = evals[2 * i]; soa[m + i] = evals[2 * i + 1]; }
  DevBuf din, dout, db;
  CK(din.alloc(2 * m * sizeof(u64)));
  CK(dout.alloc(2 * m2 * sizeof(u64)));
  CK(db.alloc(2 * sizeof(u64)));
  CK(hipMemcpyAsync(din.p, soa.data(), 2 * m * sizeof(u64), hipMemcpyHostToDevice, c->stream));
  CK(hipMemcpyAsync(db.p, beta, 2 * sizeof(u64), hipMemcpyHostToDevice, c->stream));
  CK(fri_fold_values(c->stream, 1, log_m, arity_bits, din.p, 0, dout.p, 0, db.p, 0, shift));
  std::vector<u64> res(2 * m2);
  CK(hipMemcpyAsync(res.data(), dout.p, 2 * m2 * sizeof(u64), hipMemcpyDeviceToHost, c->stream));
  CK(hipStreamSynchronize(c->stream));
  for (size_t i = 0; i < m2; i++) { out[2 * i] = res[i]; out[2 * i + 1] = res[m2 + i]; }
  return 0;
}
int mp2g_fri_pow(mp2g_ctx* c, int variant, const uint64_t state[12], uint32_t pos, uint32_t bits, uint64_t* witness) {
  NEED(c && state && witness, "ctx/pointers");
  NEED(variant == 0 || variant == 1, "variant");
  NEED(pos < 8 && bits <= 32, "pos < 8, bits <= 32");
  ChState h{};
  for (int i = 0; i < 12; i++) h.state[i] = state[i];
  for (uint32_t i = 0; i < pos; i++) h.in[i] = state[i];
  h.n_in = pos;
  DevBuf ds, dw;
  CK(ds.alloc(sizeof(ChState)));
  CK(dw.alloc(FRI_POW_STRIDE * sizeof(u64)));
  CK(hipMemcpyAsync(ds.p, &h, sizeof h, hipMemcpyHostToDevice, c->stream));
  CK(fri_pow(c->stream, variant, (const ChState*)ds.p, 1, bits, dw.p));
  CK(hipMemcpyAsync(witness, dw.p, sizeof(u64), hipMemcpyDeviceToHost, c->stream));
  CK(hipStreamSynchronize(c->stream));
  return 0;
}

static int prover_create_impl(mp2g_ctx* c, const mp2g_fri_params* params, uint32_t batch, bool alloc_oracles, mp2g_prover** out) {
  NEED(c && out, "ctx/out");
  NEED(batch >= 1 && batch <= 4096, "1 <= batch <= 4096");
  int rc = params_check(params);
  if (rc) return rc;
  mp2g_prover* pr = new (std::nothrow) mp2g_prover();
  if (!pr) return fail("out of memory");
  pr->ctx = c; pr->P = *params; pr->B = pr->Bcap = batch;
  const mp2g_fri_params& P = pr->P;
  const size_t n = (size_t)1 << P.log_n, N = n << P.rate_bits, B = batch;
  const uint32_t lg = P.log_n + P.rate_bits;
  pr->L = fri_proof_layout(P);
  pr->levels_words = merkle_levels_words(lg, P.cap_height);
  pr->n_open = mp2g_fri_n_openings(&P);
  hipError_t e = hipSuccess;
  auto A = [&](DevBuf& d, size_t words) { if (e == hipSuccess) e = d.alloc(words * sizeof(u64)); };
  auto S = [&](DevBuf& d, size_t words) { if (e == hipSuccess) e = pr->want(d, words * sizeof(u64)); };
  for (uint32_t o = 0; o < P.n_oracles && alloc_oracles; o++) {
    if (o == 0) {
      A(pr->coeffs[o], (size_t)P.oracle_w[o] * n); A(pr->values[o], (size_t)P.oracle_w[o] * N); A(pr->levels[o], pr->levels_words);
    } else {
      S(pr->coeffs[o], B * P.oracle_w[o] * n); S(pr->values[o], B * P.oracle_w[o] * N); S(pr->levels[o], B * pr->levels_words);
    }
  }
  if (e == hipSuccess) e = pr->ch.alloc(B * sizeof(ChState));
  A(pr->chal, B * 8); A(pr->zeta, B * 2); A(pr->alpha, B * 2); A(pr->betas, B * 16);
  S(pr->comp, B * 4 * n); S(pr->quot, B * 4 * n); S(pr->final_poly, B * 2 * n);
  S(pr->zpw, B * 4 * n); A(pr->fapw, B * 2 * (pr->n_open + 1));
  A(pr->witness, B * FRI_POW_STRIDE); A(pr->qchal, B * (P.num_queries ? P.num_queries : 1));
  size_t m = N, nc = n;
  uint32_t clg = lg;
  S(pr->fvals[0], B * 2 * m);
  for (uint32_t li = 0; li < P.n_layers; li++) {
    clg -= P.arity_bits[li];
    S(pr->flevels[li], B * merkle_levels_words(clg, P.cap_height));
    m >>= P.arity_bits[li]; nc >>= P.arity_bits[li];
    S(pr->fvals[li + 1], B * 2 * m);
    S(pr->fcoeffs[li + 1], B * 2 * nc);
  }
  if (e != hipSuccess) { delete pr; return fail("prover_create: %s", hipGetErrorString(e)); }
  *out = pr;
  return 0;
}
int mp2g_prover_create(mp2g_ctx* c, const mp2g_fri_params* params, uint32_t batch, mp2g_prover** out) {
  return prover_create_impl(c, params, batch, true, out);
}
}
ProverGuard::~ProverGuard() { if (pr) mp2g_prover_free(pr); }
extern "C" {
void mp2g_prover_free(mp2g_prover* pr) {
  if (!pr) return;
  mp2g_ctx* c = pr->ctx;
  (void)hipStreamSynchronize(c->stream);
  const bool counted = pr->counted;
  delete pr;
  if (counted && c->scratch_users && --c->scratch_users == 0) c->prover_scratch.release();
}
static hipError_t commit_oracle_coeffs(mp2g_prover* pr, uint32_t o, uint32_t nb) {
  mp2g_ctx* c = pr->ctx;
  const mp2g_fri_params& P = pr->P;
  const u64 n = (u64)1 << P.log_n, N = n << P.rate_bits;
  const uint32_t w = P.oracle_w[o], lg = P.log_n + P.rate_bits;
  hipError_t e;
  CosetTables* pre;
  e = c->ntt.coset(P.log_n, P.rate_bits, GL_MULT_GEN, &pre);
  if (e != hipSuccess) return e;
  e = c->ntt.run(pr->coeffs[o].p, pr->values[o].p, P.log_n, nb * w, P.rate_bits, n, N, false, pre, true);
  if (e != hipSuccess) return e;
  e = leaf_hash_poly_major(c->stream, P.variant, pr->values[o].p, w, N, N, pr->levels[o].p, nb, (u64)w * N, pr->levels_words);
  if (e != hipSuccess) return e;
  return merkle_reduce(c->stream, P.variant, pr->levels[o].p, lg, P.cap_height, nb, pr->levels_words);
}
static hipError_t commit_oracle(mp2g_prover* pr, uint32_t o, const u64* d_values, uint32_t nb) {
  const mp2g_fri_params& P = pr->P;
  const u64 n = (u64)1 << P.log_n;
  hipError_t e = pr->ctx->ntt.run(d_values, pr->coeffs[o].p, P.log_n, nb * P.oracle_w[o], 0, n, n, true, nullptr, false);
  if (e != hipSuccess) return e;
  return commit_oracle_coeffs(pr, o, nb);
}
int mp2g_prover_set_preprocessed_dev(mp2g_prover* pr, const uint64_t* d_values) {
  NEED(pr && d_values, "prover/values");
  const size_t words = (size_t)pr->P.oracle_w[0] << pr->P.log_n;
  CK(pr->pre_values.alloc(words * sizeof(u64)));
  CK(hipMemcpyAsync(pr->pre_values.p, d_values, words * sizeof(u64), hipMemcpyDeviceToDevice, pr->ctx->stream));
  CK(commit_oracle(pr, 0, (const u64*)d_values, 1));
  pr->drop_graph();
  pr->have_pre = true;
  return 0;
}
int mp2g_prover_enable_permutation(mp2g_prover* pr, uint32_t num_routed, uint32_t degree) {
  NEED(pr && pr->have_pre, "call mp2g_prover_set_preprocessed_dev first");
  const mp2g_fri_params& P = pr->P;
  NEED(P.n_oracles >= 3 && P.zs_oracle == 2, "needs wires = oracle 1 and Z/partial products = oracle 2");
  NEED(degree >= 1 && num_routed >= degree && num_routed % degree == 0 && num_routed / degree <= 16, "num_routed/degree");
  NEED(num_routed <= P.oracle_w[0] && num_routed <= P.oracle_w[1], "num_routed exceeds the sigma / wire counts");
  NEED(P.zs_count >= 1 && P.zs_count <= 2, "1 or 2 challenges");
  NEED(P.oracle_w[2] == P.zs_count * (num_routed / degree + P.num_lookup_polys), "oracle_w[2] must be zs_count * (num_routed/degree + num_lookup_polys)");
  const size_t n = (size_t)1 << P.log_n;
  CK(pr->want(pr->zs_values, (size_t)pr->Bcap * P.oracle_w[2] * n * sizeof(u64)));
  CK(pr->want(pr->chunk_q, (size_t)pr->Bcap * P.zs_count * (num_routed / degree) * n * sizeof(u64)));
  CK(pr->bg.alloc((size_t)pr->Bcap * 8 * sizeof(u64)));
  CK(pr->alphas.alloc((size_t)pr->Bcap * 2 * sizeof(u64)));
  CK(upload_table(pr->ctx, pr->ptab, perm_table_words(P.log_n, num_routed), [&](u64* h) { perm_tables_host(P.log_n, num_routed, h); }));
  pr->num_routed = num_routed; pr->degree = degree;
  pr->drop_graph();
  return 0;
}
int mp2g_prover_enable_quotient(mp2g_prover* pr) {
  NEED(pr && pr->num_routed, "call mp2g_prover_enable_permutation first");
  const mp2g_fri_params& P = pr->P;
  NEED(P.n_oracles == 4 && P.rate_bits == 3, "needs the four plonky2 oracles and rate_bits 3 (quotient degree factor 8)");
  NEED(P.oracle_w[3] == P.zs_count * 8, "oracle_w[3] must be zs_count * 8 quotient chunks");
  NEED(P.log_n + 3 <= 24, "log_n <= 21");
  CK(pr->want(pr->qvals, (size_t)pr->Bcap * P.zs_count * ((size_t)8 << P.log_n) * sizeof(u64)));
  CK(pr->apw.alloc((size_t)pr->Bcap * 2 * MP2G_MAX_GATE_CONSTRAINTS * sizeof(u64)));
  CK(upload_table(pr->ctx, pr->qtab, quotient_table_words(P.log_n), [&](u64* h) { quotient_tables_host(P.log_n, h); }));
  pr->quotient = true;
  pr->drop_graph();
  return 0;
}
int mp2g_prover_set_gates(mp2g_prover* pr, const mp2g_gate* gates, uint32_t n_gates, uint32_t num_selectors) {
  NEED(pr && pr->quotient, "call mp2g_prover_enable_quotient first");
  NEED(n_gates <= MP2G_MAX_GATES, "at most MP2G_MAX_GATES gates");
  NEED(gates || !n_gates, "gates");
  GateTable t;
  const char* msg = gate_table_make(gates, n_gates, num_selectors, pr->gates.num_lookup_selectors, pr->P.oracle_w[0] - pr->num_routed,
                                    pr->P.oracle_w[1], t, nullptr);
  if (msg) return fail("invalid gate table: %s", msg);
  for (uint32_t i = 0; i < n_gates; i++)
    if (gate_filtered_degree(t.g[i], num_selectors) > 9) return fail("invalid gate table: filtered degree of gate %u exceeds quotient degree factor + 1 = 9", i);
  pr->gates = t;
  pr->drop_graph();
  return 0;
}
}

static int fri_tail(mp2g_prover* pr, const FriShape& sh, ChState* st, u64* d_proof) {
  mp2g_ctx* c = pr->ctx;
  hipStream_t s = c->stream;
  const mp2g_fri_params& P = pr->P;
  const uint32_t B = pr->B, lg = P.log_n + P.rate_bits, V = P.variant;
  const u64 n = (u64)1 << P.log_n, N = n << P.rate_bits;
  const size_t capw = pr->L.capw;
  u64* chal = pr->chal.p;
  CK(challenger_step(s, V, st, B, chal, 0, 0, pr->alpha.p, 2, 2));
  CK(fri_final_poly(s, sh, B, pr->alpha.p, 2, pr->zeta.p, 2, pr->fapw.p, pr->comp.p, pr->quot.p, pr->final_poly.p));
  CosetTables* pre;
  CK(c->ntt.coset(P.log_n, P.rate_bits, GL_MULT_GEN, &pre));
  CK(c->ntt.run(pr->final_poly.p, pr->fvals[0].p, P.log_n, 2 * B, P.rate_bits, n, N, false, pre, true));

  FriLayers ly{};
  ly.n_layers = P.n_layers;
  u64 m = N, nc = n, shift = GL_MULT_GEN;
  uint32_t clg = lg;
  u64* proof = (u64*)d_proof;
  const u64* cur_coeffs = pr->final_poly.p;
  for (uint32_t li = 0; li < P.n_layers; li++) {
    const uint32_t ab = P.arity_bits[li];
    const uint32_t log_leaves = clg - ab;
    const size_t lw = merkle_levels_words(log_leaves, P.cap_height);
    CK(leaf_hash_ext_soa(s, V, pr->fvals[li].p, pr->fvals[li].p + m, ab, (u64)1 << log_leaves, pr->flevels[li].p, B, 2 * m, lw));
    CK(merkle_reduce(s, V, pr->flevels[li].p, log_leaves, P.cap_height, B, lw));
    CK(copy_rows(s, B, pr->flevels[li].p + lw - capw, lw, proof + li * capw, pr->L.proof_words, (u32)capw));
    u64* beta = pr->betas.p + 2 * li;
    CK(challenger_step(s, V, st, B, proof + li * capw, pr->L.proof_words, (u32)capw, beta, 16, 2));
    ly.arity_bits[li] = ab;
    ly.values[li] = pr->fvals[li].p; ly.value_bstride[li] = 2 * m;
    ly.levels[li] = pr->flevels[li].p; ly.level_bstride[li] = lw;
    CK(fri_fold_values(s, B, clg, ab, pr->fvals[li].p, 2 * m, pr->fvals[li + 1].p, 2 * (m >> ab), beta, 16, shift));
    const bool last = li + 1 == P.n_layers;
    if (last) CK(fri_fold_coeffs(s, B, (u32)nc, ab, cur_coeffs, 2 * nc, proof + pr->L.final_off, pr->L.proof_words, beta, 16, true));
    else CK(fri_fold_coeffs(s, B, (u32)nc, ab, cur_coeffs, 2 * nc, pr->fcoeffs[li + 1].p, 2 * (nc >> ab), beta, 16, false));
    cur_coeffs = pr->fcoeffs[li + 1].p;
    shift = gl_pow(shift, (u64)1 << ab);
    m >>= ab; nc >>= ab; clg -= ab;
  }
  if (P.n_layers == 0) CK(fri_soa_to_aos(s, B, (u32)n, pr->final_poly.p, 2 * n, (u32)n, proof + pr->L.final_off, pr->L.proof_words));
  CK(challenger_step(s, V, st, B, proof + pr->L.final_off, pr->L.proof_words, (u32)(2 * pr->L.final_len), chal, 8, 0));
  STAGE_MARK(pr, 5);
  CK(fri_pow(s, V, st, B, P.pow_bits, pr->witness.p));
  STAGE_MARK(pr, 6);
  CK(copy_rows(s, B, pr->witness.p, FRI_POW_STRIDE, proof + pr->L.pow_off, pr->L.proof_words, 1));
  CK(challenger_step(s, V, st, B, pr->witness.p, FRI_POW_STRIDE, 1, chal, 8, 1));
  if (P.num_queries) {
    CK(challenger_step(s, V, st, B, chal, 0, 0, pr->qchal.p, P.num_queries, P.num_queries));
    CK(fri_queries(s, sh, ly, pr->L, B, P.num_queries, pr->qchal.p, P.num_queries, proof));
  }
  return 0;
}

extern "C" {

static int prove_impl(mp2g_prover* pr, const uint64_t* const* d_values, const uint64_t* d_circuit_digest,
                      const uint64_t* d_pi_hash, uint64_t* d_caps, uint64_t* d_openings, uint64_t* d_proof);
static int bind_scratch(mp2g_prover* pr) {
  if (pr->shared.empty()) return 0;
  mp2g_ctx* c = pr->ctx;
  if (!pr->counted) { pr->counted = true; c->scratch_users++; }
  size_t total = 0;
  for (auto& e : pr->shared) total += (e.second + 255) & ~(size_t)255;
  if (c->prover_scratch.bytes < total) {
    CK(hipStreamSynchronize(c->stream));
    hipError_t e = c->prover_scratch.alloc(total);
    if (e != hipSuccess) return fail("prover scratch of %zu bytes: %s", total, hipGetErrorString(e));
  }
  if (pr->bound_base == c->prover_scratch.p && pr->bound_total == total) return 0;
  size_t off = 0;
  for (auto& e : pr->shared) {
    e.first->borrow(c->prover_scratch.p + off / sizeof(u64), e.second);
    off += (e.second + 255) & ~(size_t)255;
  }
  pr->bound_base = c->prover_scratch.p;
  pr->bound_total = total;
  pr->drop_graph();
  return 0;
}
int mp2g_prover_prove_dev(mp2g_prover* pr, const uint64_t* const* d_values, const uint64_t* d_circuit_digest,
                          const uint64_t* d_pi_hash, uint64_t* d_caps, uint64_t* d_openings, uint64_t* d_proof) {
  NEED(pr && d_values && d_circuit_digest && d_pi_hash && d_caps && d_openings && d_proof, "prover/pointers");
  NEED(pr->have_pre, "call mp2g_prover_set_preprocessed_dev first");
  { int rcb = bind_scratch(pr); if (rcb) return rcb; }
  if (!pr->graph_on || pr->timing || pr->plain_calls == 0) {
    pr->plain_calls++;
    return prove_impl(pr, d_values, d_circuit_digest, d_pi_hash, d_caps, d_openings, d_proof);
  }
  const void* key[12] = {d_circuit_digest, d_pi_hash, d_caps, d_openings, d_proof};
  for (uint32_t o = 1; o < pr->P.n_oracles && o < 8; o++) key[4 + o] = d_values[o - 1];
  hipStream_t s = pr->ctx->stream;
  if (pr->gexec && memcmp(key, pr->gkey, sizeof key) == 0 && pr->ggen == pr->ctx->ntt.generation) {
    CK(hipGraphLaunch(pr->gexec, s));
    return 0;
  }
  pr->drop_graph();
  hipGraph_t g = nullptr;
  if (pr->quotient)
    CK(pr->ctx->ntt.ensure_scratch((size_t)pr->B * pr->P.zs_count * ((size_t)8 << pr->P.log_n)));
  for (uint32_t o = 1; o < pr->P.n_oracles; o++) CK(pr->ctx->ntt.ensure_scratch((size_t)pr->B * pr->P.oracle_w[o] << pr->P.log_n));
  const u64 gen0 = pr->ctx->ntt.generation;
  CK(hipStreamBeginCapture(s, hipStreamCaptureModeThreadLocal));
  int rc = prove_impl(pr, d_values, d_circuit_digest, d_pi_hash, d_caps, d_openings, d_proof);
  hipError_t e = hipStreamEndCapture(s, &g);
  if (!rc && e == hipSuccess && pr->ctx->ntt.generation != gen0) {
    if (g) (void)hipGraphDestroy(g);
    return fail("graph capture: an NTT buffer was reallocated inside the capture");
  }
  if (rc || e != hipSuccess) {
    if (g) (void)hipGraphDestroy(g);
    return rc ? rc : fail("graph capture: %s", hipGetErrorString(e));
  }
  e = hipGraphInstantiate(&pr->gexec, g, nullptr, nullptr, 0);
  (void)hipGraphDestroy(g);
  if (e != hipSuccess) { pr->gexec = nullptr; return fail("hipGraphInstantiate: %s", hipGetErrorString(e)); }
  memcpy(pr->gkey, key, sizeof key);
  pr->ggen = gen0;
  CK(hipGraphLaunch(pr->gexec, s));
  return 0;
}
int mp2g_prover_enable_graph(mp2g_prover* pr, int on) {
  NEED(pr, "prover");
  pr->graph_on = on != 0;
  if (!on) pr->drop_graph();
  return 0;
}
static int prove_impl(mp2g_prover* pr, const uint64_t* const* d_values, const uint64_t* d_circuit_digest,
                      const uint64_t* d_pi_hash, uint64_t* d_caps, uint64_t* d_openings, uint64_t* d_proof) {
  mp2g_ctx* c = pr->ctx;
  hipStream_t s = c->stream;
  const mp2g_fri_params& P = pr->P;
  const uint32_t B = pr->B, V = P.variant;
  const u64 n = (u64)1 << P.log_n, N = n << P.rate_bits;
  const size_t capw = pr->L.capw, LW = pr->levels_words;
  ChState* st = (ChState*)pr->ch.p;
  u64* chal = pr->chal.p;
  const u64 caps_b = P.n_oracles * capw;

  STAGE_MARK(pr, 0);
  if (pr->pi_row >= 0)
    CK(bind_public_inputs(s, B, (u64*)d_values[0], (u64)P.oracle_w[1] * n, n, (u32)pr->pi_row, (const u64*)d_pi_hash));
  if (pr->wcheck) {
    CK(hipMemsetAsync(pr->wflags.p, 0, B * sizeof(u32), s));
    if (pr->gates.n_gates)
      CK(gate_check(s, B, pr->gates, pr->pre_values.p, (const u64*)d_values[0], (u64)P.oracle_w[1] * n, n, (const u64*)d_pi_hash,
                    (u32*)pr->wflags.p));
  }
  CK(challenger_init(s, st, B));
  CK(challenger_step(s, V, st, B, (const u64*)d_circuit_digest, 0, 4, chal, 8, 0));
  CK(challenger_step(s, V, st, B, (const u64*)d_pi_hash, 4, 4, chal, 8, 0));
  CK(copy_rows(s, B, pr->levels[0].p + LW - capw, 0, (u64*)d_caps, caps_b, (u32)capw));
  for (uint32_t o = 1; o < P.n_oracles; o++) {
    const u64* vals = (const u64*)d_values[o - 1];
    if (o == 2 && pr->num_routed) {
      CK(zpp_compute(s, B, (const u64*)d_values[0], (u64)P.oracle_w[1] * n, pr->pre_values.p + (u64)(P.oracle_w[0] - pr->num_routed) * n,
                     P.log_n, pr->num_routed, pr->degree, pr->bg.p, pr->bg.p + P.zs_count, 8, P.zs_count, pr->ptab.p, pr->chunk_q.p,
                     pr->zs_values.p, (u64)P.oracle_w[2] * n));
      if (pr->lookups.n_luts) {
        CK(lookup_table_polys(s, B, pr->lookups, pr->bg.p, 8, P.zs_count, pr->lut_eval.p));
        CK(lookup_polys(s, B, pr->lookups, (const u64*)d_values[0], (u64)P.oracle_w[1] * n, P.log_n, pr->bg.p, 8, P.zs_count,
                        pr->zs_values.p + (u64)P.zs_count * (pr->num_routed / pr->degree) * n, (u64)P.oracle_w[2] * n, pr->lut_eval.p,
                        pr->wcheck ? (u32*)pr->wflags.p : nullptr));
      }
      vals = pr->zs_values.p;
      if (pr->wcheck)
        CK(zpp_wrap_check(s, B, pr->chunk_q.p, pr->zs_values.p, (u64)P.oracle_w[2] * n, P.log_n, pr->num_routed / pr->degree, P.zs_count,
                          (u32*)pr->wflags.p));
    }
    if (o == 3 && pr->quotient) {
      const u32 nc = P.zs_count;
      CK(alpha_powers(s, B, pr->alphas.p, 2, nc, pr->apw.p));
      if (pr->gates.n_gates)
        CK(gate_constraints_lde(s, B, pr->gates, pr->values[0].p, pr->values[1].p, (u64)P.oracle_w[1] * N, P.log_n + 3, pr->apw.p, nc,
                                (const u64*)d_pi_hash, pr->qvals.p));
      if (pr->lookups.n_luts)
        CK(quotient_lookup_values(s, B, pr->lookups, pr->values[0].p, pr->gates.num_selectors, pr->values[1].p, (u64)P.oracle_w[1] * N,
                                  pr->values[2].p, (u64)P.oracle_w[2] * N, nc * (pr->num_routed / pr->degree), P.log_n, pr->bg.p, 8,
                                  pr->lut_eval.p, pr->alphas.p, 2, nc, pr->qvals.p));
      CK(quotient_perm_values(s, B, pr->values[1].p, (u64)P.oracle_w[1] * N, pr->values[0].p + (u64)(P.oracle_w[0] - pr->num_routed) * N,
                              pr->values[2].p, (u64)P.oracle_w[2] * N, P.log_n, pr->num_routed, pr->degree, pr->bg.p, 8,
                              pr->apw.p, MP2G_MAX_GATE_CONSTRAINTS, nc, pr->gates.n_gates != 0, pr->ptab.p, pr->qtab.p, pr->qvals.p));
      CK(c->ntt.run(pr->qvals.p, pr->coeffs[3].p, P.log_n + 3, B * nc, 0, N, N, true, nullptr, false));
      CK(c->ntt.scale_table(pr->coeffs[3].p, P.log_n + 3, B * nc, pr->qtab.p + quotient_unshift_offset(P.log_n)));
      CK(commit_oracle_coeffs(pr, 3, B));
    } else {
      NEED(vals, "d_values[o]");
      CK(commit_oracle(pr, o, vals, B));
    }
    u64* cap_dst = (u64*)d_caps + o * capw;
    CK(copy_rows(s, B, pr->levels[o].p + LW - capw, LW, cap_dst, caps_b, (u32)capw));
    const uint32_t nch = P.zs_count >= 1 && P.zs_count <= 2 ? P.zs_count : 2;
    const uint32_t n_get = plonk_challenges_after_cap(o, nch, pr->lookups.n_luts != 0);
    u64* dst = chal;
    u64 dst_stride = 8;
    if (pr->num_routed && o == 1) { dst = pr->bg.p; dst_stride = 8; }
    if (pr->num_routed && o == 2) { dst = pr->alphas.p; dst_stride = 2; }
    CK(challenger_step(s, V, st, B, cap_dst, caps_b, (u32)capw, dst, dst_stride, n_get));
    if (o <= 3) STAGE_MARK(pr, o);
  }
  if (P.n_oracles < 4) for (uint32_t o = P.n_oracles; o <= 3; o++) STAGE_MARK(pr, o);
  CK(challenger_step(s, V, st, B, chal, 0, 0, pr->zeta.p, 2, 2));

  FriShape sh = fri_shape(P);
  for (uint32_t o = 0; o < P.n_oracles; o++) {
    OracleRef& r = sh.o[o];
    r.coeffs = pr->coeffs[o].p; r.values = pr->values[o].p; r.levels = pr->levels[o].p;
    r.coeff_bstride = o ? (u64)r.w * n : 0;
    r.value_bstride = o ? (u64)r.w * N : 0;
    r.level_bstride = o ? LW : 0;
  }
  CK(fri_openings(s, sh, B, pr->zeta.p, 2, pr->zpw.p, (u64*)d_openings));
  CK(challenger_step(s, V, st, B, (const u64*)d_openings, 2 * pr->n_open, (u32)(2 * pr->n_open), chal, 8, 0));
  STAGE_MARK(pr, 4);
  int rc = fri_tail(pr, sh, st, (u64*)d_proof);
  if (rc) return rc;
  STAGE_MARK(pr, 7);
  return 0;
}
int mp2g_prover_set_lookups(mp2g_prover* pr, const mp2g_lookup* luts, uint32_t n_luts) {
  NEED(pr && pr->quotient, "call mp2g_prover_enable_quotient first");
  NEED(n_luts <= MP2G_MAX_LUTS, "at most MP2G_MAX_LUTS lookup tables");
  const mp2g_fri_params& P = pr->P;
  LookupDev L{};
  if (!n_luts) {
    NEED(P.num_lookup_polys == 0, "params.num_lookup_polys != 0 needs lookup tables");
    pr->lookups = L;
    pr->gates.num_lookup_selectors = 0;
    pr->drop_graph();
    return 0;
  }
  NEED(luts && pr->gates.n_gates, "luts; call mp2g_prover_set_gates first");
  lookup_geometry(pr->num_routed, pr->degree, L);
  NEED(L.lu_degree >= 1 && L.num_lu_slots <= 40 && L.num_lut_slots >= 1, "slot geometry (num_routed <= 80, degree >= 2)");
  NEED(P.num_lookup_polys == L.num_sldc + 1, "params.num_lookup_polys must be ceil((num_routed/2) / (degree-1)) + 1");
  NEED(P.oracle_w[1] >= 3 * L.num_lut_slots && P.oracle_w[1] >= 2 * L.num_lu_slots, "wires");
  const uint32_t n_sel = 4 + n_luts, num_constants = P.oracle_w[0] - pr->num_routed;
  NEED(pr->gates.num_selectors + n_sel <= num_constants, "the constants must hold 4 + n_luts lookup selectors after the selectors");
  const uint64_t n = (uint64_t)1 << P.log_n;
  for (uint32_t r = 0; r < n_luts; r++) {
    const mp2g_lookup& u = luts[r];
    NEED(u.table && u.table_len >= 1 && u.table_len <= 65536, "table");
    NEED(u.last_lu_row < u.last_lut_row && u.last_lut_row <= u.first_lut_row && (uint64_t)u.first_lut_row + 1 < n, "lookup rows");
    NEED((uint64_t)(u.first_lut_row - u.last_lut_row + 1) * L.num_lut_slots >= u.table_len, "the table does not fit its LookupTableGate rows");
  }
  pr->drop_graph();
  pr->lookups = LookupDev{};
  pr->gates.num_lookup_selectors = 0;
  { int rc = lookup_upload(pr->ctx->stream, luts, n_luts, pr->lut_tables, L); if (rc) return rc; }
  CK(pr->lut_eval.alloc((size_t)pr->Bcap * P.zs_count * MP2G_MAX_LUTS * sizeof(u64)));
  {
    std::vector<u32> index;
    pr->lut_inputs_unique = lut_build_index(luts, n_luts, index);
    CK(pr->lut_index.alloc(index.size() * sizeof(u32)));
    CK(hipMemcpy(pr->lut_index.p, index.data(), index.size() * sizeof(u32), hipMemcpyHostToDevice));
  }
  pr->lookups = L;
  pr->gates.num_lookup_selectors = n_sel;
  const char* msg = gate_table_check(pr->gates, num_constants, P.oracle_w[1]);
  if (msg) { pr->lookups = LookupDev{}; pr->gates.num_lookup_selectors = 0; return fail("invalid gate table with lookups: %s", msg); }
  pr->drop_graph();
  return 0;
}
int mp2g_prover_lookup_wires_dev(mp2g_prover* pr, const uint32_t* n_lookups, uint64_t* d_wires, uint32_t batch) {
  NEED(pr && n_lookups && d_wires && batch >= 1, "prover / n_lookups / wires / batch");
  const LookupDev& D = pr->lookups;
  NEED(D.n_luts, "call mp2g_prover_set_lookups first");
  NEED(pr->lut_inputs_unique, "a lookup table holds an input twice: its multiplicities are not defined");
  LutIndex L{};
  L.n_luts = D.n_luts; L.lu_slots = D.num_lu_slots; L.lut_slots = D.num_lut_slots;
  for (uint32_t t = 0; t < D.n_luts; t++) {
    NEED((uint64_t)n_lookups[t] <= (uint64_t)(D.last_lut_row[t] - D.last_lu_row[t]) * D.num_lu_slots, "n_lookups exceeds the table's LookupGate slots");
    L.last_lu_row[t] = D.last_lu_row[t]; L.last_lut_row[t] = D.last_lut_row[t]; L.first_lut_row[t] = D.first_lut_row[t];
    L.table_len[t] = D.table_len[t]; L.n_lookups[t] = n_lookups[t];
    L.table[t] = D.table[t];
    L.index[t] = (const u32*)pr->lut_index.p + (size_t)t * LUT_INPUTS;
  }
  const u64 n = (u64)1 << pr->P.log_n;
  CK(lookup_wires_launch(pr->ctx->stream, L, (u64*)d_wires, batch, (u64)pr->P.oracle_w[1] * n, n, 1));
  return 0;
}
int mp2g_prover_bind_public_inputs(mp2g_prover* pr, int64_t row) {
  NEED(pr, "prover");
  NEED(row < (int64_t)1 << pr->P.log_n, "row < 2^log_n");
  NEED(pr->P.n_oracles >= 2 && pr->P.oracle_w[1] >= 4, "needs a wires oracle of at least 4 columns");
  pr->pi_row = row < 0 ? -1 : row;
  pr->drop_graph();
  return 0;
}
int mp2g_prover_set_active(mp2g_prover* pr, uint32_t n) {
  NEED(pr && n >= 1 && n <= pr->Bcap, "1 <= n <= the batch the prover was created for");
  if (n != pr->B) pr->drop_graph();
  pr->B = n;
  return 0;
}
int mp2g_prover_enable_witness_check(mp2g_prover* pr, int on) {
  NEED(pr && pr->num_routed, "call mp2g_prover_enable_permutation first");
  if (on && !pr->wflags.p) CK(pr->wflags.alloc((size_t)pr->Bcap * sizeof(u32)));
  pr->wcheck = on != 0;
  pr->drop_graph();
  return 0;
}
int mp2g_prover_witness_check_enabled(const mp2g_prover* pr) { return pr && pr->wcheck ? 1 : 0; }
int mp2g_prover_witness_status(mp2g_prover* pr, uint32_t* flags) {
  NEED(pr && pr->wcheck, "call mp2g_prover_enable_witness_check first");
  std::vector<uint32_t> h(pr->B);
  CK(hipMemcpyAsync(h.data(), pr->wflags.p, pr->B * sizeof(u32), hipMemcpyDeviceToHost, pr->ctx->stream));
  CK(hipStreamSynchronize(pr->ctx->stream));
  if (flags) memcpy(flags, h.data(), pr->B * sizeof(u32));
  for (uint32_t b = 0; b < pr->B; b++)
    if (h[b])
      return fail("invalid witness: proof %u of the batch violates%s%s%s", b, (h[b] & 1) ? " a copy constraint" : "",
                  (h[b] & 2) ? " a gate constraint" : "", (h[b] & 4) ? " the lookup argument" : "");
  return 0;
}
}
namespace mp2g { int prover_flags_to_host_async(mp2g_prover* pr, uint32_t* h_dst); }
int mp2g::prover_flags_to_host_async(mp2g_prover* pr, uint32_t* h_dst) {
  NEED(pr && pr->wcheck && h_dst, "prover with the witness check on / destination");
  CK(hipMemcpyAsync(h_dst, pr->wflags.p, pr->B * sizeof(u32), hipMemcpyDeviceToHost, pr->ctx->stream));
  return 0;
}
extern "C" {
int mp2g_prover_enable_timing(mp2g_prover* pr, int on) {
  NEED(pr, "prover");
  if (on)
    for (hipEvent_t& e : pr->ev)
      if (!e) CK(hipEventCreate(&e));
  pr->timing = on != 0;
  return 0;
}
int mp2g_prover_stage_ms(mp2g_prover* pr, float out[MP2G_N_STAGES]) {
  NEED(pr && out, "prover/out");
  NEED(pr->timing, "call mp2g_prover_enable_timing first");
  CK(hipStreamSynchronize(pr->ctx->stream));
  for (int i = 0; i < MP2G_N_STAGES; i++) CK(hipEventElapsedTime(&out[i], pr->ev[i], pr->ev[i + 1]));
  return 0;
}

int mp2g_partial_products_and_zs(mp2g_ctx* c, const uint64_t* wires, uint32_t wires_w, const uint64_t* sigmas, uint32_t log_n,
                                 uint32_t num_routed, uint32_t degree, const uint64_t* betas, const uint64_t* gammas, uint32_t nc,
                                 uint64_t* out) {
  NEED(c && wires && sigmas && betas && gammas && out, "ctx/pointers");
  NEED(log_n >= 1 && log_n <= 20 && nc >= 1 && nc <= 4, "log_n/nc");
  NEED(degree >= 1 && num_routed >= degree && num_routed % degree == 0 && num_routed / degree <= 16 && num_routed <= wires_w, "num_routed/degree");
  const size_t n = (size_t)1 << log_n, chunks = num_routed / degree;
  DevBuf dw, ds, dc, dq, dout, dt;
  CK(upload_table(c, dt, perm_table_words(log_n, num_routed), [&](u64* h) { perm_tables_host(log_n, num_routed, h); }));
  CK(dw.alloc(wires_w * n * sizeof(u64)));
  CK(ds.alloc(num_routed * n * sizeof(u64)));
  CK(dc.alloc(2 * nc * sizeof(u64)));
  CK(dq.alloc(nc * chunks * n * sizeof(u64)));
  CK(dout.alloc(nc * chunks * n * sizeof(u64)));
  CK(hipMemcpyAsync(dw.p, wires, wires_w * n * sizeof(u64), hipMemcpyHostToDevice, c->stream));
  CK(hipMemcpyAsync(ds.p, sigmas, num_routed * n * sizeof(u64), hipMemcpyHostToDevice, c->stream));
  CK(hipMemcpyAsync(dc.p, betas, nc * sizeof(u64), hipMemcpyHostToDevice, c->stream));
  CK(hipMemcpyAsync(dc.p + nc, gammas, nc * sizeof(u64), hipMemcpyHostToDevice, c->stream));
  CK(zpp_compute(c->stream, 1, dw.p, 0, ds.p, log_n, num_routed, degree, dc.p, dc.p + nc, 0, nc, dt.p, dq.p, dout.p, 0));
  CK(hipMemcpyAsync(out, dout.p, nc * chunks * n * sizeof(u64), hipMemcpyDeviceToHost, c->stream));
  CK(hipStreamSynchronize(c->stream));
  return 0;
}

uint32_t mp2g_gate_num_constraints(const mp2g_gate* g) { return g ? gate_num_constraints(*g) : 0; }
uint32_t mp2g_gate_degree(const mp2g_gate* g) { return g ? gate_degree(*g) : 0; }
int mp2g_eval_gate_constraints(mp2g_ctx* c, const mp2g_gate* gates, uint32_t n_gates, uint32_t num_selectors, const uint64_t* consts,
                               uint32_t num_constants, const uint64_t* wires, uint32_t wires_w, uint64_t npts,
                               const uint64_t pi_hash[4], uint64_t* out) {
  NEED(c && gates && consts && wires && pi_hash && out, "ctx/pointers");
  NEED(n_gates >= 1 && n_gates <= MP2G_MAX_GATES, "1..MP2G_MAX_GATES gates");
  NEED(npts >= 1 && npts <= ((uint64_t)1 << 28), "npts");
  GateTable t;
  uint32_t max_j = 0;
  const char* msg = gate_table_make(gates, n_gates, num_selectors, 0, num_constants, wires_w, t, &max_j);
  if (msg) return fail("invalid gate table: %s", msg);
  if (!max_j) return 0;
  DevBuf dc, dw, dp, dout;
  CK(dc.alloc((size_t)num_constants * npts * sizeof(u64)));
  CK(dw.alloc((size_t)wires_w * npts * sizeof(u64)));
  CK(dp.alloc(4 * sizeof(u64)));
  CK(dout.alloc((size_t)max_j * npts * sizeof(u64)));
  CK(hipMemcpyAsync(dc.p, consts, (size_t)num_constants * npts * sizeof(u64), hipMemcpyHostToDevice, c->stream));
  CK(hipMemcpyAsync(dw.p, wires, (size_t)wires_w * npts * sizeof(u64), hipMemcpyHostToDevice, c->stream));
  CK(hipMemcpyAsync(dp.p, pi_hash, 4 * sizeof(u64), hipMemcpyHostToDevice, c->stream));
  CK(gate_constraints_points(c->stream, t, dc.p, dw.p, npts, max_j, dp.p, dout.p));
  CK(hipMemcpyAsync(out, dout.p, (size_t)max_j * npts * sizeof(u64), hipMemcpyDeviceToHost, c->stream));
  CK(hipStreamSynchronize(c->stream));
  return 0;
}

int mp2g_batch_eval_ext(const mp2g_batch* b, const uint64_t point[2], uint64_t* out) {
  NEED(b && point && out, "batch/point/out");
  NEED(point[0] < GL_P && point[1] < GL_P, "point canonical");
  mp2g_ctx* c = b->ctx;
  FriShape sh{};
  sh.log_n = b->log_n; sh.rate_bits = b->rate_bits; sh.cap_h = b->cap_h; sh.n_oracles = 1; sh.n_polys = b->w;
  sh.o[0].coeffs = b->coeffs.p; sh.o[0].w = b->w;
  DevBuf dz, dout, dzpw;
  CK(dz.alloc(2 * sizeof(u64)));
  CK(dout.alloc((size_t)b->w * 2 * sizeof(u64)));
  CK(dzpw.alloc(((size_t)4 << b->log_n) * sizeof(u64)));
  CK(hipMemcpyAsync(dz.p, point, 2 * sizeof(u64), hipMemcpyHostToDevice, c->stream));
  CK(fri_openings(c->stream, sh, 1, dz.p, 0, dzpw.p, dout.p));
  CK(hipMemcpyAsync(out, dout.p, (size_t)b->w * 2 * sizeof(u64), hipMemcpyDeviceToHost, c->stream));
  CK(hipStreamSynchronize(c->stream));
  return 0;
}

int mp2g_fri_prove(mp2g_ctx* c, const mp2g_fri_params* params, mp2g_batch* const* oracles, const uint64_t zeta[2],
                   mp2g_challenger* ch, uint64_t* proof) {
  NEED(c && params && oracles && zeta && ch && proof, "ctx/pointers");
  NEED(ch->ctx == c && ch->count == 1, "challenger must live on this context with count 1");
  NEED(ch->variant == (int)params->variant, "challenger / params hash variant differ");
  mp2g_prover* pr;
  int rc = prover_create_impl(c, params, 1, false, &pr);
  if (rc) return rc;
  ProverGuard guard;
  guard.pr = pr;
  const mp2g_fri_params& P = pr->P;
  FriShape sh = fri_shape(P);
  for (uint32_t o = 0; o < P.n_oracles; o++) {
    const mp2g_batch* b = oracles[o];
    if (!b || b->ctx != c || b->log_n != P.log_n || b->w != P.oracle_w[o] || b->rate_bits != P.rate_bits ||
        b->cap_h != P.cap_height || b->variant != (int)P.variant) {
      return fail("oracle %u does not match the FRI parameters", o);
    }
    OracleRef& r = sh.o[o];
    r.coeffs = b->coeffs.p; r.values = b->values.p; r.levels = b->levels.p;
  }
  DevBuf dproof;
  hipError_t e = dproof.alloc(pr->L.proof_words * sizeof(u64));
  if (e == hipSuccess) e = hipMemcpyAsync(pr->zeta.p, zeta, 2 * sizeof(u64), hipMemcpyHostToDevice, c->stream);
  if (e != hipSuccess) return fail("fri_prove setup: %s", hipGetErrorString(e));
  rc = bind_scratch(pr);
  if (!rc) rc = fri_tail(pr, sh, (ChState*)ch->st.p, dproof.p);
  if (!rc) {
    e = hipMemcpyAsync(proof, dproof.p, pr->L.proof_words * sizeof(u64), hipMemcpyDeviceToHost, c->stream);
    if (e == hipSuccess) e = hipStreamSynchronize(c->stream);
    if (e != hipSuccess) rc = fail("fri_prove copy-out: %s", hipGetErrorString(e));
  }
  return rc;
}

int mp2g_pcs_prove(mp2g_ctx* c, const mp2g_fri_params* params, const uint64_t* const* values, const uint64_t circuit_digest[4],
                   const uint64_t pi_hash[4], uint64_t* caps, uint64_t* openings, uint64_t* proof) {
  NEED(c && values && circuit_digest && pi_hash && caps && openings && proof, "ctx/pointers");
  mp2g_prover* pr;
  int rc = mp2g_prover_create(c, params, 1, &pr);
  if (rc) return rc;
  ProverGuard guard;
  guard.pr = pr;
  const mp2g_fri_params& P = pr->P;
  const size_t n = (size_t)1 << P.log_n;
  DevBuf dv[8], dd, dp, dcaps, dopen, dproof;
  const uint64_t* dptr[8] = {};
  hipError_t e = hipSuccess;
  for (uint32_t o = 0; o < P.n_oracles && e == hipSuccess; o++) {
    e = dv[o].alloc(P.oracle_w[o] * n * sizeof(u64));
    if (e == hipSuccess) e = hipMemcpyAsync(dv[o].p, values[o], P.oracle_w[o] * n * sizeof(u64), hipMemcpyHostToDevice, c->stream);
    if (o) dptr[o - 1] = dv[o].p;
  }
  if (e == hipSuccess) e = dd.alloc(32);
  if (e == hipSuccess) e = dp.alloc(32);
  if (e == hipSuccess) e = dcaps.alloc(P.n_oracles * pr->L.capw * sizeof(u64));
  if (e == hipSuccess) e = dopen.alloc(pr->n_open * 2 * sizeof(u64));
  if (e == hipSuccess) e = dproof.alloc(pr->L.proof_words * sizeof(u64));
  if (e == hipSuccess) e = hipMemcpyAsync(dd.p, circuit_digest, 32, hipMemcpyHostToDevice, c->stream);
  if (e == hipSuccess) e = hipMemcpyAsync(dp.p, pi_hash, 32, hipMemcpyHostToDevice, c->stream);
  if (e != hipSuccess) return fail("pcs_prove setup: %s", hipGetErrorString(e));
  rc = mp2g_prover_set_preprocessed_dev(pr, dv[0].p);
  if (!rc) rc = mp2g_prover_prove_dev(pr, dptr, dd.p, dp.p, dcaps.p, dopen.p, dproof.p);
  if (!rc) {
    e = hipMemcpyAsync(caps, dcaps.p, P.n_oracles * pr->L.capw * sizeof(u64), hipMemcpyDeviceToHost, c->stream);
    if (e == hipSuccess) e = hipMemcpyAsync(openings, dopen.p, pr->n_open * 2 * sizeof(u64), hipMemcpyDeviceToHost, c->stream);
    if (e == hipSuccess) e = hipMemcpyAsync(proof, dproof.p, pr->L.proof_words * sizeof(u64), hipMemcpyDeviceToHost, c->stream);
    if (e == hipSuccess) e = hipStreamSynchronize(c->stream);
    if (e != hipSuccess) rc = fail("pcs_prove copy-out: %s", hipGetErrorString(e));
  }
  return rc;
}

}
```

mapreduce-plonky2_amd/csrc/verifier.hip:

```cpp
#include "verifier.h"
#include "fri.h"
#include "gates.h"
#include "lookup.h"
#include "poseidon.cuh"
#include <algorithm>
#include <cstring>
#include <new>
#include <vector>

using namespace mp2g;


#define V_MAX_LINE_POINTS 32
#define V_NO_FAIL 0xFFFFFFFFu

namespace {
struct Parts {
  const u64* p[4];
  u64 s[4];
  u32 n[4];
};
struct VShape {
  u32 log_n, n_oracles, n_layers, num_queries, pow_bits;
  u32 arity_bits[8];
  u32 nc, nlp;
  u32 num_routed, degree, num_constants, num_selectors, max_j, T;
};

__device__ __forceinline__ gl2 open_at(const u64* op, u32 i) { return gl2_make(op[2 * i], op[2 * i + 1]); }
__device__ __forceinline__ bool gl2_same(gl2 x, gl2 y) { return x.a == y.a && x.b == y.b; }
__device__ __forceinline__ gl2 gl2_from(u64 a) { return gl2_make(a, 0); }

__global__ void __launch_bounds__(256) verifier_canon_kernel(Parts pt, u32* __restrict__ status) {
  const u32 b = blockIdx.y;
  bool bad = false;
  for (u32 k = 0; k < 4; k++) {
    const u64* w = pt.p[k] + b * pt.s[k];
    for (u32 i = blockIdx.x * 256 + threadIdx.x; i < pt.n[k]; i += gridDim.x * 256) bad |= w[i] >= GL_P;
  }
  if (bad) status[b] = 20;
}

template <int V>
__global__ void verifier_pi_hash_kernel(Parts pt, u32 n_pi, int given, u32 B, const u32* __restrict__ status, u64* __restrict__ pih) {
  const u32 b = blockIdx.x * blockDim.x + threadIdx.x;
  if (b >= B) return;
  u64* out = pih + 4 * b;
  if (status[b]) { out[0] = out[1] = out[2] = out[3] = 0; return; }
  const u64* in = pt.p[0] + b * pt.s[0];
  if (given) { for (int i = 0; i < 4; i++) out[i] = in[i]; return; }
  u64 s[12];
  for (int i = 0; i < 12; i++) s[i] = 0;
  for (u32 i = 0; i < n_pi; i += 8) {
    const u32 k = n_pi - i < 8 ? n_pi - i : 8;
    for (u32 j = 0; j < k; j++) s[j] = in[i + j];
    perm<V>(s);
  }
  for (int i = 0; i < 4; i++) out[i] = s[i];
}

__global__ void __launch_bounds__(256) verifier_line_kernel(VShape sh, OpeningLayout ol, Parts pt, u32 B, const u32* __restrict__ status,
                                                            u64* __restrict__ lc, u64* __restrict__ lw) {
  const u32 wires_w = ol.oracle[1].len, per = (sh.num_constants + wires_w) * sh.T;
  const u32 idx = blockIdx.x * 256 + threadIdx.x;
  if (idx >= B * per) return;
  const u32 b = idx / per, r = idx % per, j = r / sh.T, t = r % sh.T;
  u64 v = 0;
  if (!status[b]) {
    const u64* op = pt.p[2] + b * pt.s[2];
    const u32 o = j < sh.num_constants ? ol.constants + j : ol.oracle[1].off + (j - sh.num_constants);
    v = gl_mul_add(op[2 * o + 1], t, op[2 * o]);
  }
  if (j < sh.num_constants) lc[((u64)b * sh.num_constants + j) * sh.T + t] = v;
  else lw[((u64)b * wires_w + (j - sh.num_constants)) * sh.T + t] = v;
}

__global__ void __launch_bounds__(64) verifier_identity_kernel(VShape sh, OpeningLayout ol, LookupGeometry lu, Parts pt, u32 B,
                                                               const u64* __restrict__ bg,
                                                               const u64* __restrict__ alphas, const u64* __restrict__ zetas,
                                                               const u64* __restrict__ lut_eval, const u64* __restrict__ gate_vals,
                                                               const u64* __restrict__ interp, u32* __restrict__ status) {
  const u32 b = blockIdx.x * blockDim.x + threadIdx.x;
  if (b >= B || status[b]) return;
  const u64* op = pt.p[2] + b * pt.s[2];
  const u32 nc = sh.nc, chunks = sh.num_routed / sh.degree, num_prods = chunks - 1;
  const u64* betas = bg + 8 * b;
  const u64* gammas = betas + nc;
  const gl2 zeta = gl2_make(zetas[2 * b], zetas[2 * b + 1]);
  gl2 zn = zeta;
  for (u32 i = 0; i < sh.log_n; i++) zn = gl2_mul(zn, zn);
  const gl2 zh = gl2_sub(zn, gl2_from(1));
  const gl2 l0 = gl2_mul(zh, gl2_inv(gl2_scale(gl2_sub(zeta, gl2_from(1)), ((u64)1 << sh.log_n) % GL_P)));
  u64 al[2] = {alphas[2 * b], nc > 1 ? alphas[2 * b + 1] : 0}, apow[2] = {1, 1};
  gl2 van[2] = {gl2_from(0), gl2_from(0)};
  auto term = [&](gl2 v) {
#pragma unroll
    for (int a = 0; a < 2; a++) {
      van[a] = gl2_add(van[a], gl2_scale(v, apow[a]));
      apow[a] = gl_mul(apow[a], al[a]);
    }
  };
  for (u32 c = 0; c < nc; c++) term(gl2_mul(l0, gl2_sub(open_at(op, ol.zs + c), gl2_from(1))));
  for (u32 c = 0; c < nc; c++) {
    u64 kj = 1;
    for (u32 ch = 0; ch < chunks; ch++) {
      gl2 num = gl2_from(1), den = gl2_from(1);
      for (u32 j = ch * sh.degree; j < (ch + 1) * sh.degree; j++) {
        const gl2 wv = open_at(op, ol.wires + j);
        num = gl2_mul(num, gl2_add(gl2_add(wv, gl2_scale(zeta, gl_mul(betas[c], kj))), gl2_from(gammas[c])));
        den = gl2_mul(den, gl2_add(gl2_add(wv, gl2_scale(open_at(op, ol.sigmas + j), betas[c])), gl2_from(gammas[c])));
        kj = gl_mul(kj, GL_MULT_GEN);
      }
      const gl2 prev = ch == 0 ? open_at(op, ol.zs + c) : open_at(op, ol.partial_products + c * num_prods + ch - 1);
      const gl2 next = ch == chunks - 1 ? open_at(op, ol.zs_next + c) : open_at(op, ol.partial_products + c * num_prods + ch);
      term(gl2_sub(gl2_mul(prev, num), gl2_mul(next, den)));
    }
  }
  if (lu.n_luts) {
    const u32 ns = lu.num_sldc, nlp = sh.nlp;
    auto sel = [&](u32 i) { return open_at(op, sh.num_selectors + i); };
    auto wire = [&](u32 i) { return open_at(op, ol.wires + i); };
    for (u32 c = 0; c < nc; c++) {
      const u64* d = bg + 8 * b + 4 * c;
      const u64 dA = d[0], dB = d[1], dAl = d[2], dDe = d[3];
      auto zs = [&](u32 q) { return open_at(op, ol.lookup + c * nlp + q); };
      auto zsn = [&](u32 q) { return open_at(op, ol.lookup_next + c * nlp + q); };
      auto combo = [&](u32 i, u32 stride) {
        const gl2 x = gl2_add(wire(stride * i), gl2_scale(wire(stride * i + 1), dA));
        return gl2_make(gl_sub(dAl, x.a), gl_neg(x.b));
      };
      term(gl2_mul(sel(3), zs(ns)));
      term(gl2_mul(sel(2), zs(1)));
      term(gl2_mul(sel(2), zs(0)));
      for (u32 r = 0; r < lu.n_luts; r++)
        term(gl2_mul(sel(4 + r), gl2_sub(zs(0), gl2_from(lut_eval[((u64)b * nc + c) * MP2G_MAX_LUTS + r]))));
      gl2 cur = zsn(0);
      for (u32 s = 0; s < lu.num_lut_slots; s++)
        cur = gl2_add(gl2_scale(cur, dDe), gl2_add(wire(3 * s), gl2_scale(wire(3 * s + 1), dB)));
      term(gl2_mul(sel(0), gl2_sub(zs(0), cur)));
      for (u32 poly = 0; poly < ns; poly++) {
        u32 t0 = poly * lu.lut_degree, t1 = t0 + lu.lut_degree < lu.num_lut_slots ? t0 + lu.lut_degree : lu.num_lut_slots;
        const u32 u0 = poly * lu.lu_degree, u1 = u0 + lu.lu_degree < lu.num_lu_slots ? u0 + lu.lu_degree : lu.num_lu_slots;
        if (t0 > lu.num_lut_slots) t0 = t1 = lu.num_lut_slots;
        gl2 lut_prod = gl2_from(1), lut_sum = gl2_from(0), lu_prod = gl2_from(1), lu_sum = gl2_from(0);
        for (u32 i = t0; i < t1; i++) lut_prod = gl2_mul(lut_prod, combo(i, 3));
        for (u32 i = t0; i < t1; i++) {
          gl2 pr = gl2_from(1);
          for (u32 j = t0; j < t1; j++)
            if (j != i) pr = gl2_mul(pr, combo(j, 3));
          lut_sum = gl2_add(lut_sum, gl2_mul(wire(3 * i + 2), pr));
        }
        for (u32 i = u0; i < u1; i++) lu_prod = gl2_mul(lu_prod, combo(i, 2));
        for (u32 i = u0; i < u1; i++) {
          gl2 pr = gl2_from(1);
          for (u32 j = u0; j < u1; j++)
            if (j != i) pr = gl2_mul(pr, combo(j, 2));
          lu_sum = gl2_add(lu_sum, pr);
        }
        const gl2 prev = poly == 0 ? zsn(ns) : zs(poly);
        const gl2 diff = gl2_sub(zs(1 + poly), prev);
        term(gl2_mul(sel(0), gl2_sub(gl2_mul(lut_prod, diff), lut_sum)));
        term(gl2_mul(sel(1), gl2_add(gl2_mul(lu_prod, diff), lu_sum)));
      }
    }
  }
  const u64* gv = gate_vals + (u64)b * sh.max_j * sh.T;
  for (u32 j = 0; j < sh.max_j; j++) {
    gl_cols c0, c1;
    for (u32 t = 0; t < sh.T; t++) {
      const u64 v = gv[j * sh.T + t];
      c0.add(v, interp[t]);
      c1.add(v, interp[V_MAX_LINE_POINTS + t]);
    }
    term(gl2_make(c0.value(), c1.value()));
  }
  for (u32 a = 0; a < nc; a++) {
    gl2 tz = gl2_from(0);
    for (u32 i = 8; i-- > 0;) tz = gl2_add(gl2_mul(tz, zn), open_at(op, ol.quotient + a * 8 + i));
    if (!gl2_same(van[a], gl2_mul(zh, tz))) { status[b] = 10 + a; return; }
  }
}

__global__ void __launch_bounds__(64) verifier_pow_kernel(VShape sh, OpeningLayout ol, Parts pt, u32 B, const u64* __restrict__ pow_resp,
                                                          const u64* __restrict__ fri_alpha, u32* __restrict__ status,
                                                          u64* __restrict__ red) {
  const u32 b = blockIdx.x * blockDim.x + threadIdx.x;
  if (b >= B || status[b]) return;
  if (sh.pow_bits && (pow_resp[b] >> (64 - sh.pow_bits)) != 0) { status[b] = 1; return; }
  const u64* op = pt.p[2] + b * pt.s[2];
  const gl2 alpha = gl2_make(fri_alpha[2 * b], fri_alpha[2 * b + 1]);
  gl2 acc = gl2_from(0);
  for (u32 i = ol.n_zeta; i-- > 0;) acc = gl2_add(gl2_mul(acc, alpha), open_at(op, i));
  red[4 * b] = acc.a; red[4 * b + 1] = acc.b;
  acc = gl2_from(0);
  for (u32 i = ol.n_open; i-- > ol.n_zeta;) acc = gl2_add(gl2_mul(acc, alpha), open_at(op, i));
  red[4 * b + 2] = acc.a; red[4 * b + 3] = acc.b;
}

__device__ __forceinline__ void query_fail(u32* qstat, u32 b, u32 q, u32 pos, u32 code) { atomicMin(&qstat[b], (q << 16) | (pos << 8) | code); }

template <int V>
__global__ void __launch_bounds__(256) verifier_paths_kernel(FriProofLayout L, VShape sh, Parts pt, u32 B, const u64* __restrict__ cap0,
                                                             const u64* __restrict__ qchal, const u32* __restrict__ status,
                                                             u32* __restrict__ qstat) {
  const u32 idx = blockIdx.x * 256 + threadIdx.x, per = B * sh.num_queries;
  if (idx >= per * L.n_paths) return;
  const u32 p = idx / per, r = idx % per, b = r / sh.num_queries, q = r % sh.num_queries;
  if (status[b]) return;
  const u64* proof = pt.p[3] + b * pt.s[3];
  const u64* leaf = proof + L.q_off + (u64)q * L.q_words + L.leaf_off[p];
  const u32 len = L.leaf_len[p];
  const u64* sib = leaf + len;
  u32 x = (u32)(qchal[(u64)b * sh.num_queries + q] & (((u64)1 << L.lg) - 1)) >> L.x_shift[p];
  const u64* cap = p == 0 ? cap0 : p < sh.n_oracles ? pt.p[1] + b * pt.s[1] + (u64)(p - 1) * L.capw : proof + (u64)(p - sh.n_oracles) * L.capw;
  u64 s[12];
#pragma unroll
  for (int i = 0; i < 12; i++) s[i] = 0;
  if (len <= 4) {
    for (u32 i = 0; i < len; i++) s[i] = leaf[i];
  } else {
    for (u32 i = 0; i < len; i += 8) {
      const u32 k = len - i < 8 ? len - i : 8;
      if (k == 8) {
#pragma unroll
        for (int j = 0; j < 8; j++) s[j] = leaf[i + j];
      } else {
#pragma unroll
        for (int j = 0; j < 8; j++)
          if ((u32)j < k) s[j] = leaf[i + j];
      }
      perm<V>(s);
    }
  }
  for (u32 i = 0; i < L.n_sib[p]; i++) {
    const u64* sb = sib + 4 * i;
    const bool right = x & 1;
#pragma unroll
    for (int j = 0; j < 4; j++) {
      const u64 c = s[j], o = sb[j];
      s[j] = right ? o : c;
      s[4 + j] = right ? c : o;
      s[8 + j] = 0;
    }
    perm<V>(s);
    x >>= 1;
  }
  const u64* want = cap + 4 * x;
  if (s[0] != want[0] || s[1] != want[1] || s[2] != want[2] || s[3] != want[3]) {
    if (p < sh.n_oracles) query_fail(qstat, b, q, 0, 2);
    else query_fail(qstat, b, q, 2 + 2 * (p - sh.n_oracles), 4);
  }
}

__global__ void __launch_bounds__(64) verifier_fold_kernel(VShape sh, FriShape fs, FriProofLayout L, Parts pt, u32 B, const u64* __restrict__ qchal,
                                                           const u64* __restrict__ zetas, const u64* __restrict__ fri_alpha,
                                                           const u64* __restrict__ fri_betas, const u64* __restrict__ red,
                                                           const u32* __restrict__ status, u32* __restrict__ qstat) {
  const u32 idx = blockIdx.x * blockDim.x + threadIdx.x;
  if (idx >= B * sh.num_queries) return;
  const u32 b = idx / sh.num_queries, q = idx % sh.num_queries;
  if (status[b]) return;
  const u64* proof = pt.p[3] + b * pt.s[3];
  const u64* qw = proof + L.q_off + (u64)q * L.q_words;
  const u32 lg = fs.log_n + fs.rate_bits;
  u32 x = (u32)(qchal[(u64)b * sh.num_queries + q] & (((u64)1 << lg) - 1));
  const gl2 alpha = gl2_make(fri_alpha[2 * b], fri_alpha[2 * b + 1]);
  const gl2 zeta = gl2_make(zetas[2 * b], zetas[2 * b + 1]);
  const gl2 g_zeta = gl2_scale(zeta, gl_root_of_unity(fs.log_n));
  u64 sx = gl_mul(GL_MULT_GEN, gl_pow(gl_root_of_unity(lg), bitrev32(x, lg)));
  gl2 sum = gl2_from(0);
  for (u32 batch = 0; batch < 2; batch++) {
    const u32 count = fri_batch_len(fs, batch);
    gl2 acc = gl2_from(0);
    for (u32 j = count; j-- > 0;) {
      u32 o, p;
      fri_batch_poly(fs, batch, j, o, p);
      acc = gl2_mul(acc, alpha);
      acc.a = gl_add(acc.a, qw[L.leaf_off[o] + p]);
    }
    const gl2 num = gl2_sub(acc, gl2_make(red[4 * b + 2 * batch], red[4 * b + 2 * batch + 1]));
    const gl2 den = gl2_sub(gl2_from(sx), batch == 0 ? zeta : g_zeta);
    sum = gl2_mul(sum, gl2_pow(alpha, count));
    sum = gl2_add(sum, gl2_mul(num, gl2_inv(den)));
  }
  gl2 old_eval = sum;
  for (u32 li = 0; li < sh.n_layers; li++) {
    const u32 ab = sh.arity_bits[li], arity = 1u << ab;
    const u32 coset = x >> ab, within = x & (arity - 1);
    const u64* ev = qw + L.leaf_off[fs.n_oracles + li];
    if (ev[2 * within] != old_eval.a || ev[2 * within + 1] != old_eval.b) query_fail(qstat, b, q, 1 + 2 * li, 3);
    const gl2 beta = gl2_make(fri_betas[16 * b + 2 * li], fri_betas[16 * b + 2 * li + 1]);
    const u64 g = gl_root_of_unity(ab);
    const u64 start = gl_mul(sx, gl_pow(g, arity - bitrev32(within, ab)));
    u64 S = start;
    for (u32 i = 0; i < ab; i++) S = gl_sqr(S);
    const u64 inv_as = gl_inv(gl_mul(S, arity));
    gl2 res = gl2_from(0);
    u64 xi = start;
    for (u32 i = 0; i < arity; i++) {
      const u32 src = bitrev32(i, ab);
      gl2 numr = gl2_from(1);
      u64 xj = start;
      for (u32 j = 0; j < arity; j++) {
        if (j != i) numr = gl2_mul(numr, gl2_make(gl_sub(beta.a, xj), beta.b));
        xj = gl_mul(xj, g);
      }
      res = gl2_add(res, gl2_mul(gl2_make(ev[2 * src], ev[2 * src + 1]), gl2_scale(numr, gl_mul(xi, inv_as))));
      xi = gl_mul(xi, g);
    }
    old_eval = res;
    for (u32 i = 0; i < ab; i++) sx = gl_sqr(sx);
    x = coset;
  }
  const u64* fin = proof + L.final_off;
  gl2 fe = gl2_from(0);
  for (u32 i = L.final_len; i-- > 0;) fe = gl2_add(gl2_scale(fe, sx), gl2_make(fin[2 * i], fin[2 * i + 1]));
  if (!gl2_same(fe, old_eval)) query_fail(qstat, b, q, 1 + 2 * sh.n_layers, 5);
}

__global__ void verifier_status_kernel(u32 B, const u32* __restrict__ qstat, u32* __restrict__ status) {
  const u32 b = blockIdx.x * blockDim.x + threadIdx.x;
  if (b >= B) return;
  if (!status[b] && qstat[b] != V_NO_FAIL) status[b] = qstat[b] & 0xFF;
}

__global__ void verifier_challenges_kernel(VShape sh, u32 lg, u32 has_lookup, u32 B, const u64* bg, const u64* alphas, const u64* zetas, const u64* fri_alpha,
                                           const u64* fri_betas, const u64* pow_resp, const u64* qchal, u64* out, u32 wpp) {
  const u32 b = blockIdx.x * blockDim.x + threadIdx.x;
  if (b >= B) return;
  u64* o = out + (u64)b * wpp;
  for (u32 i = 0; i < 2; i++) {
    o[i] = i < sh.nc ? bg[8 * b + i] : 0;
    o[2 + i] = i < sh.nc ? bg[8 * b + sh.nc + i] : 0;
    o[4 + i] = i < sh.nc ? alphas[2 * b + i] : 0;
    o[6 + i] = zetas[2 * b + i];
    o[16 + i] = fri_alpha[2 * b + i];
  }
  for (u32 i = 0; i < 8; i++) o[8 + i] = has_lookup && i < 4 * sh.nc ? bg[8 * b + i] : 0;
  for (u32 i = 0; i < 2 * sh.n_layers; i++) o[18 + i] = fri_betas[16 * b + i];
  o[18 + 2 * sh.n_layers] = pow_resp[b];
  for (u32 i = 0; i < sh.num_queries; i++) o[19 + 2 * sh.n_layers + i] = qchal[(u64)b * sh.num_queries + i] & (((u64)1 << lg) - 1);
}

void interpolation_rows(u32 T, u64* out) {
  std::vector<u64> basis(T), next(T);
  for (u32 t = 0; t < T; t++) {
    std::fill(basis.begin(), basis.end(), 0);
    basis[0] = 1;
    u64 den = 1;
    u32 deg = 0;
    for (u32 s = 0; s < T; s++) {
      if (s == t) continue;
      std::fill(next.begin(), next.end(), 0);
      for (u32 k = 0; k <= deg; k++) {
        next[k + 1] = gl_add(next[k + 1], basis[k]);
        next[k] = gl_sub(next[k], gl_mul(basis[k], s));
      }
      basis.swap(next);
      deg++;
      den = gl_mul(den, gl_sub(t, s));
    }
    const u64 di = gl_inv(den);
    u64 r0 = 0, r1 = 0, p7 = 1;
    for (u32 k = 0; k < T; k++) {
      const u64 c = gl_mul(gl_mul(basis[k], di), p7);
      if (k & 1) { r1 = gl_add(r1, c); p7 = gl_mul(p7, 7); } else r0 = gl_add(r0, c);
    }
    out[t] = r0;
    out[V_MAX_LINE_POINTS + t] = r1;
  }
}
}

struct mp2g_verifier {
  mp2g_ctx* ctx = nullptr;
  mp2g_fri_params P{};
  uint32_t capacity = 0, n_pi = 0, last_count = 0, wpp = 0;
  bool pi_given = false;
  ProofParts parts{};
  FriProofLayout fl{};
  OpeningLayout ol{};
  VShape sh{};
  FriShape fs{};
  GateTable gates{};
  LookupDev lookups{};
  DevBuf lut_tables, lut_eval;
  DevBuf cap0, digest, interp;
  DevBuf ch, pih, chal, bg, alphas, zeta, fri_alpha, fri_betas, pow_resp, qchal, red;
  DevBuf lc, lw, gate_vals;
  DevBuf status, qstat, staging, chal_out;
};

namespace mp2g {
mp2g_ctx* verifier_ctx(const mp2g_verifier* v) { return v ? v->ctx : nullptr; }
uint32_t verifier_capacity(const mp2g_verifier* v) { return v ? v->capacity : 0; }
}

static Parts contiguous_parts(const mp2g_verifier* v, const u64* d_words) {
  Parts pt{};
  for (int k = 0; k < 4; k++) { pt.p[k] = d_words + v->parts.off[k]; pt.s[k] = v->parts.words; pt.n[k] = v->parts.n[k]; }
  return pt;
}

static int verify_parts(mp2g_verifier* v, const Parts& pt, uint32_t B, uint32_t* status) {
  mp2g_ctx* c = v->ctx;
  hipStream_t s = c->stream;
  const mp2g_fri_params& P = v->P;
  const VShape& sh = v->sh;
  const FriProofLayout& L = v->fl;
  const bool has_lookup = v->lookups.n_luts != 0;
  const int V = (int)P.variant;
  ChState* st = (ChState*)v->ch.p;
  u32* d_status = (u32*)v->status.p;
  u32* d_qstat = (u32*)v->qstat.p;
  u64* chal = v->chal.p;
  const u32 nch = sh.nc, capw = L.capw;
  v->last_count = 0;
  CK(hipMemsetAsync(d_status, 0, B * sizeof(u32), s));
  CK(hipMemsetAsync(d_qstat, 0xFF, B * sizeof(u32), s));
  hipLaunchKernelGGL(verifier_canon_kernel, dim3(16, B), dim3(256), 0, s, pt, d_status);
  if (V == MP2G_POSEIDON2)
    hipLaunchKernelGGL((verifier_pi_hash_kernel<MP2G_POSEIDON2>), dim3((B + 63) / 64), dim3(64), 0, s, pt, v->n_pi, (int)v->pi_given, B, d_status, v->pih.p);
  else
    hipLaunchKernelGGL((verifier_pi_hash_kernel<MP2G_POSEIDON>), dim3((B + 63) / 64), dim3(64), 0, s, pt, v->n_pi, (int)v->pi_given, B, d_status, v->pih.p);
  CK(hipGetLastError());
  CK(challenger_init(s, st, B));
  CK(challenger_step(s, V, st, B, v->digest.p, 0, 4, chal, 8, 0));
  CK(challenger_step(s, V, st, B, v->pih.p, 4, 4, chal, 8, 0));
  for (u32 o = 1; o < P.n_oracles; o++) {
    u64* dst = o == 1 ? v->bg.p : o == 2 ? v->alphas.p : chal;
    const u64 dst_stride = o == 2 ? 2 : 8;
    CK(challenger_step(s, V, st, B, pt.p[1] + (u64)(o - 1) * capw, pt.s[1], capw, dst, dst_stride, plonk_challenges_after_cap(o, nch, has_lookup)));
  }
  CK(challenger_step(s, V, st, B, chal, 0, 0, v->zeta.p, 2, 2));
  CK(challenger_step(s, V, st, B, pt.p[2], pt.s[2], pt.n[2], chal, 8, 0));
  CK(challenger_step(s, V, st, B, chal, 0, 0, v->fri_alpha.p, 2, 2));
  for (u32 li = 0; li < P.n_layers; li++)
    CK(challenger_step(s, V, st, B, pt.p[3] + (u64)li * capw, pt.s[3], capw, v->fri_betas.p + 2 * li, 16, 2));
  CK(challenger_step(s, V, st, B, pt.p[3] + L.final_off, pt.s[3], 2 * L.final_len, chal, 8, 0));
  CK(challenger_step(s, V, st, B, pt.p[3] + L.pow_off, pt.s[3], 1, v->pow_resp.p, 1, 1));
  if (P.num_queries) CK(challenger_step(s, V, st, B, chal, 0, 0, v->qchal.p, P.num_queries, P.num_queries));
  if (has_lookup) CK(lookup_table_polys(s, B, v->lookups, v->bg.p, 8, nch, v->lut_eval.p));
  if (sh.max_j) {
    const u32 total = B * (sh.num_constants + P.oracle_w[1]) * sh.T;
    hipLaunchKernelGGL(verifier_line_kernel, dim3((total + 255) / 256), dim3(256), 0, s, sh, v->ol, pt, B, d_status, v->lc.p, v->lw.p);
    CK(hipGetLastError());
    CK(gate_constraints_points_batch(s, B, v->gates, v->lc.p, (u64)sh.num_constants * sh.T, v->lw.p, (u64)P.oracle_w[1] * sh.T, sh.T,
                                     sh.max_j, v->pih.p, v->gate_vals.p));
  }
  hipLaunchKernelGGL(verifier_identity_kernel, dim3((B + 63) / 64), dim3(64), 0, s, sh, v->ol, (LookupGeometry)v->lookups, pt, B, v->bg.p, v->alphas.p,
                     v->zeta.p, v->lut_eval.p, v->gate_vals.p, v->interp.p, d_status);
  hipLaunchKernelGGL(verifier_pow_kernel, dim3((B + 63) / 64), dim3(64), 0, s, sh, v->ol, pt, B, v->pow_resp.p, v->fri_alpha.p, d_status, v->red.p);
  CK(hipGetLastError());
  if (P.num_queries) {
    const u32 n_tasks = B * P.num_queries * L.n_paths;
    if (V == MP2G_POSEIDON2)
      hipLaunchKernelGGL((verifier_paths_kernel<MP2G_POSEIDON2>), dim3((n_tasks + 255) / 256), dim3(256), 0, s, L, sh, pt, B, v->cap0.p, v->qchal.p, d_status, d_qstat);
    else
      hipLaunchKernelGGL((verifier_paths_kernel<MP2G_POSEIDON>), dim3((n_tasks + 255) / 256), dim3(256), 0, s, L, sh, pt, B, v->cap0.p, v->qchal.p, d_status, d_qstat);
    hipLaunchKernelGGL(verifier_fold_kernel, dim3((B * P.num_queries + 63) / 64), dim3(64), 0, s, sh, v->fs, L, pt, B, v->qchal.p, v->zeta.p,
                       v->fri_alpha.p, v->fri_betas.p, v->red.p, d_status, d_qstat);
    hipLaunchKernelGGL(verifier_status_kernel, dim3((B + 63) / 64), dim3(64), 0, s, B, d_qstat, d_status);
    CK(hipGetLastError());
  }
  CK(hipMemcpyAsync(status, d_status, B * sizeof(u32), hipMemcpyDeviceToHost, s));
  CK(hipStreamSynchronize(s));
  v->last_count = B;
  return 0;
}

namespace mp2g {
// ... 167 lines not shown
```

mapreduce-plonky2_amd/csrc/zperm.h:

```cpp
#pragma once
#include "gl.cuh"
namespace mp2g {
size_t perm_table_words(u32 log_n, u32 num_routed);
size_t quotient_table_words(u32 log_n);
void perm_tables_host(u32 log_n, u32 num_routed, u64* out);
void quotient_tables_host(u32 log_n, u64* out);
inline size_t quotient_unshift_offset(u32 log_n) { return ((size_t)16 << log_n) + 8; }
hipError_t zpp_compute(hipStream_t s, u32 B, const u64* wires, u64 wires_bstride, const u64* sigmas, u32 log_n, u32 num_routed,
                       u32 degree, const u64* betas, const u64* gammas, u64 chal_bstride, u32 nc, const u64* ptab, u64* chunk_q,
                       u64* out, u64 out_bstride);
hipError_t quotient_perm_values(hipStream_t s, u32 B, const u64* W, u64 w_bstride, const u64* S, const u64* Z, u64 z_bstride,
                                u32 log_n, u32 num_routed, u32 degree, const u64* bg, u64 bg_bstride, const u64* apw, u32 apw_len,
                                u32 nc, bool gates, const u64* ptab, const u64* qtab, u64* q);
hipError_t zpp_wrap_check(hipStream_t s, u32 B, const u64* chunk_q, const u64* zs, u64 zs_bstride, u32 log_n, u32 chunks, u32 nc,
                          u32* flags);
}
```

mapreduce-plonky2_amd/csrc/zperm.hip:

```cpp
#include "zperm.h"
#include <vector>

namespace mp2g {

#define ZP_MAX_CHUNKS 16
#define ZP_MAX_ROUTED 256
#define ZP_MAX_TERMS (2 * (1 + ZP_MAX_CHUNKS))
__device__ __forceinline__ void fill_k_is(u64* kis, const u64* __restrict__ ktab, u32 num_routed) {
  for (u32 j = threadIdx.x; j < num_routed; j += blockDim.x) kis[j] = ktab[j];
  __syncthreads();
}

__global__ void __launch_bounds__(256) zpp_chunk_kernel(const u64* __restrict__ wires, u64 wires_bstride, const u64* __restrict__ sigmas,
                                                        u32 log_n, u32 num_routed, u32 degree, const u64* __restrict__ betas,
                                                        const u64* __restrict__ gammas, u64 chal_bstride, u32 nc,
                                                        const u64* __restrict__ ptab, u64* __restrict__ chunk_q) {
  const u32 n = 1u << log_n, i = blockIdx.x * 256 + threadIdx.x, c = blockIdx.y, b = blockIdx.z;
  __shared__ u64 kis[ZP_MAX_ROUTED];
  fill_k_is(kis, ptab + n, num_routed);
  if (i >= n) return;
  const u32 chunks = num_routed / degree;
  const u64 beta = betas[b * chal_bstride + c], gamma = gammas[b * chal_bstride + c];
  const u64 bx = gl_mul(beta, ptab[i]);
  const u64* w = wires + b * wires_bstride + i;
  const u64* sg = sigmas + i;
  u64 num[ZP_MAX_CHUNKS], den[ZP_MAX_CHUNKS];
  u32 j = 0;
  for (u32 k = 0; k < chunks; k++) {
    u64 pn = 1, pd = 1;
    for (u32 t = 0; t < degree; t++, j++) {
      u64 wv = w[(u64)j << log_n];
      const u64 wg = gl_addw(wv, gamma);
      pn = gl_mulw(pn, gl_mul_addw(bx, kis[j], wg));
      pd = gl_mulw(pd, gl_mul_addw(beta, sg[(u64)j << log_n], wg));
    }
    num[k] = pn; den[k] = gl_canon(pd);
  }
  u64 pre[ZP_MAX_CHUNKS];
  u64 acc = 1;
  for (u32 k = 0; k < chunks; k++) { pre[k] = acc; acc = gl_mul(acc, den[k] ? den[k] : 1); }
  u64 inv = gl_inv(acc);
  u64* out = chunk_q + ((u64)(b * nc + c) * chunks << log_n) + i;
  for (int k = (int)chunks - 1; k >= 0; k--) {
    u64 dinv = den[k] ? gl_mul(inv, pre[k]) : 0;
    inv = gl_mul(inv, den[k] ? den[k] : 1);
    out[(u64)k << log_n] = gl_mul(num[k], dinv);
  }
}
__global__ void __launch_bounds__(1024) zpp_scan_kernel(const u64* __restrict__ chunk_q, u32 log_n, u32 chunks, u32 nc, u64* __restrict__ out,
                                                        u64 out_bstride) {
  const u32 n = 1u << log_n, c = blockIdx.x, b = blockIdx.y, t = threadIdx.x;
  const u32 T = n < 1024 ? n : 1024, S = n / T;
  const u32 num_prods = chunks - 1;
  const u64* q = chunk_q + ((u64)(b * nc + c) * chunks << log_n);
  __shared__ u64 sc[1024];
  u64 local = 1;
  if (t < T)
    for (u32 r = 0; r < S; r++)
      for (u32 k = 0; k < chunks; k++) local = gl_mul(local, q[((u64)k << log_n) + t * S + r]);
  sc[t] = local;
  __syncthreads();
  for (u32 d = 1; d < T; d <<= 1) {
    u64 v = (t >= d && t < T) ? sc[t - d] : 1;
    __syncthreads();
    if (t < T) sc[t] = gl_mul(sc[t], v);
    __syncthreads();
  }
  if (t >= T) return;
  u64 z = t ? sc[t - 1] : 1;
  u64* zrow = out + b * out_bstride + ((u64)c << log_n);
  u64* pp = out + b * out_bstride + ((u64)nc << log_n) + ((u64)c * num_prods << log_n);
  for (u32 r = 0; r < S; r++) {
    u32 i = t * S + r;
    zrow[i] = z;
    u64 acc = z;
    for (u32 k = 0; k < chunks; k++) {
      acc = gl_mul(acc, q[((u64)k << log_n) + i]);
      if (k < num_prods) pp[((u64)k << log_n) + i] = acc;
    }
    z = acc;
  }
}

__global__ void __launch_bounds__(256) quotient_perm_kernel(const u64* __restrict__ W, u64 w_bstride, const u64* __restrict__ S,
                                                            const u64* __restrict__ Z, u64 z_bstride, u32 log_n, u32 num_routed,
                                                            u32 degree, const u64* __restrict__ bg, u64 bg_bstride,
                                                            const u64* __restrict__ apw, u32 apw_len, u32 nc, bool gates,
                                                            const u64* __restrict__ ptab, const u64* __restrict__ qtab,
                                                            u64* __restrict__ q) {
  const u32 lg = log_n + 3;
  const u64 N = (u64)1 << lg;
  const u32 p = blockIdx.x * 256 + threadIdx.x, b = blockIdx.y;
  const u32 i = bitrev32(p, lg);
  const u32 chunks = num_routed / degree, num_prods = chunks - 1, n_terms = nc * (1 + chunks);
  __shared__ u64 zh_inv[8];
  __shared__ u64 kis[ZP_MAX_ROUTED];
  __shared__ u64 al[2][ZP_MAX_TERMS + 1];
  if (threadIdx.x < 8) zh_inv[threadIdx.x] = qtab[2 * N + threadIdx.x];
  for (u32 e = threadIdx.x; e < 2 * (n_terms + 1); e += 256) {
    const u32 a = e / (n_terms + 1), k = e % (n_terms + 1);
    al[a][k] = apw[((u64)b * 2 + a) * apw_len + k];
  }
  fill_k_is(kis, ptab + (N >> 3), num_routed);
  if (p >= N) return;
  const u64 pn = bitrev32((i + 8) & (u32)(N - 1), lg);
  const u64 x = qtab[p], l0 = qtab[N + p];
  const u64* w = W + b * w_bstride + p;
  const u64* sg = S + p;
  const u64* z = Z + b * z_bstride;
  gl_cols acc[2];
  u32 kt = 0;
  auto push = [&](u64 term) {
    for (u32 a = 0; a < nc; a++) acc[a].add(term, al[a][kt]);
    kt++;
  };
  for (u32 c = 0; c < nc; c++) push(gl_mul(l0, gl_sub(z[((u64)c << lg) + p], 1)));
  for (u32 c = 0; c < nc; c++) {
    const u64 beta = bg[b * bg_bstride + c], gamma = bg[b * bg_bstride + nc + c];
    const u64 bx = gl_mul(beta, x);
    const u64* pp = z + ((u64)(nc + c * num_prods) << lg);
    u32 j = 0;
    u64 prev = z[((u64)c << lg) + p];
    for (u32 k = 0; k < chunks; k++) {
      u64 num = 1, den = 1;
      for (u32 t = 0; t < degree; t++, j++) {
        u64 wv = w[(u64)j << lg];
        const u64 wg = gl_addw(wv, gamma);
        num = gl_mulw(num, gl_mul_addw(bx, kis[j], wg));
        den = gl_mulw(den, gl_mul_addw(beta, sg[(u64)j << lg], wg));
      }
      u64 next = k == chunks - 1 ? z[((u64)c << lg) + pn] : pp[((u64)k << lg) + p];
      push(gl_sub(gl_mul(prev, num), gl_mul(next, den)));
      prev = next;
    }
  }
  if (gates)
    for (u32 a = 0; a < nc; a++) acc[a].add(q[(((u64)b * nc + a) << lg) + i], al[a][n_terms]);
  for (u32 a = 0; a < nc; a++) q[(((u64)b * nc + a) << lg) + i] = gl_mul(acc[a].value(), zh_inv[i & 7]);
}
hipError_t quotient_perm_values(hipStream_t s, u32 B, const u64* W, u64 w_bstride, const u64* S, const u64* Z, u64 z_bstride,
                                u32 log_n, u32 num_routed, u32 degree, const u64* bg, u64 bg_bstride, const u64* apw, u32 apw_len,
                                u32 nc, bool gates, const u64* ptab, const u64* qtab, u64* q) {
  if (nc < 1 || nc > 2 || !degree || num_routed % degree || num_routed > ZP_MAX_ROUTED || num_routed / degree > ZP_MAX_CHUNKS ||
      apw_len < nc * (1 + num_routed / degree) + 1)
    return hipErrorInvalidValue;
  const u64 N = (u64)8 << log_n;
  hipLaunchKernelGGL(quotient_perm_kernel, dim3((u32)((N + 255) / 256), B), dim3(256), 0, s, W, w_bstride, S, Z, z_bstride, log_n,
                     num_routed, degree, bg, bg_bstride, apw, apw_len, nc, gates, ptab, qtab, q);
  return hipGetLastError();
}

__global__ void zpp_wrap_check_kernel(const u64* __restrict__ chunk_q, const u64* __restrict__ zs, u64 zs_bstride, u32 log_n, u32 chunks,
                                      u32 nc, u32 B, u32* __restrict__ flags) {
  const u32 t = blockIdx.x * blockDim.x + threadIdx.x;
  if (t >= B * nc) return;
  const u32 b = t / nc, c = t % nc, last = (1u << log_n) - 1;
  u64 acc = zs[b * zs_bstride + ((u64)c << log_n) + last];
  const u64* q = chunk_q + ((u64)(b * nc + c) * chunks << log_n);
  for (u32 k = 0; k < chunks; k++) acc = gl_mul(acc, q[((u64)k << log_n) + last]);
  if (acc != 1) atomicOr(&flags[b], 1u);
}
hipError_t zpp_wrap_check(hipStream_t s, u32 B, const u64* chunk_q, const u64* zs, u64 zs_bstride, u32 log_n, u32 chunks, u32 nc,
                          u32* flags) {
  hipLaunchKernelGGL(zpp_wrap_check_kernel, dim3((B * nc + 63) / 64), dim3(64), 0, s, chunk_q, zs, zs_bstride, log_n, chunks, nc, B, flags);
  return hipGetLastError();
}

hipError_t zpp_compute(hipStream_t s, u32 B, const u64* wires, u64 wires_bstride, const u64* sigmas, u32 log_n, u32 num_routed,
                       u32 degree, const u64* betas, const u64* gammas, u64 chal_bstride, u32 nc, const u64* ptab, u64* chunk_q,
                       u64* out, u64 out_bstride) {
  if (!degree || num_routed % degree || num_routed / degree > ZP_MAX_CHUNKS || num_routed / degree < 1 || num_routed > ZP_MAX_ROUTED)
    return hipErrorInvalidValue;
  const u32 n = 1u << log_n, chunks = num_routed / degree;
  hipLaunchKernelGGL(zpp_chunk_kernel, dim3((n + 255) / 256, nc, B), dim3(256), 0, s, wires, wires_bstride, sigmas, log_n, num_routed,
                     degree, betas, gammas, chal_bstride, nc, ptab, chunk_q);
  hipLaunchKernelGGL(zpp_scan_kernel, dim3(nc, B), dim3(1024), 0, s, chunk_q, log_n, chunks, nc, out, out_bstride);
  return hipGetLastError();
}

size_t perm_table_words(u32 log_n, u32 num_routed) { return ((size_t)1 << log_n) + num_routed; }
size_t quotient_table_words(u32 log_n) { return quotient_unshift_offset(log_n) + ((size_t)8 << log_n); }
void perm_tables_host(u32 log_n, u32 num_routed, u64* out) {
  const size_t n = (size_t)1 << log_n;
  const u64 w = gl_root_of_unity(log_n);
  u64 v = 1;
  for (size_t i = 0; i < n; i++, v = gl_mul(v, w)) out[i] = v;
  v = 1;
  for (u32 j = 0; j < num_routed; j++, v = gl_mul(v, GL_MULT_GEN)) out[n + j] = v;
}
void quotient_tables_host(u32 log_n, u64* out) {
  const u32 lg = log_n + 3;
  const size_t N = (size_t)1 << lg;
  u64 *tx = out, *tl = out + N, *zh_inv = out + 2 * N, *unshift = out + quotient_unshift_offset(log_n);
  u64 zh[8];
  const u64 gn = gl_pow(GL_MULT_GEN, (u64)1 << log_n), w8 = gl_root_of_unity(3);
  for (u32 r = 0; r < 8; r++) {
    zh[r] = gl_sub(gl_mul(gn, gl_pow(w8, r)), 1);
    zh_inv[r] = gl_inv(zh[r]);
  }
  std::vector<u64> x(N), pre(N);
  const u64 wN = gl_root_of_unity(lg), n_mod = ((u64)1 << log_n) % GL_P;
  u64 v = GL_MULT_GEN, acc = 1;
  for (size_t i = 0; i < N; i++, v = gl_mul(v, wN)) {
    x[i] = v;
    pre[i] = acc;
    acc = gl_mul(acc, gl_mul(n_mod, gl_sub(v, 1)));
  }
  u64 inv = gl_inv(acc);
  for (size_t i = N; i-- > 0;) {
    const u64 d = gl_mul(n_mod, gl_sub(x[i], 1));
    const u32 p = bitrev32((u32)i, lg);
    tx[p] = x[i];
    tl[p] = gl_mul(zh[i & 7], gl_mul(inv, pre[i]));
    inv = gl_mul(inv, d);
  }
  const u64 g_inv = gl_inv(GL_MULT_GEN);
  v = 1;
  for (size_t k = 0; k < N; k++, v = gl_mul(v, g_inv)) unshift[k] = v;
}
}
```

Baseline: 925.3.

## Use limb-split lazy accumulation for alpha-weighted constraint sums

Adds a new lazy sum that splits each alpha power into three 22-bit limbs precomputed once on device. Each term is then accumulated with six 32x32 multiplies into 64-bit columns and reduced once at the end, replacing the four-column 64x64 product accumulation. The alpha-powers kernel now also writes the limb form. Gate kernels choose the limb or old form per gate kind at compile time, and the permutation quotient and light-gate kernels use the limb form. This trades more multiplies and registers per term for cheaper carry handling, bounded by a maximum term count.

```diff
diff --git a/mapreduce-plonky2_amd/csrc/fri.hip b/mapreduce-plonky2_amd/csrc/fri.hip
--- a/mapreduce-plonky2_amd/csrc/fri.hip
+++ b/mapreduce-plonky2_amd/csrc/fri.hip
@@ -132,7 +132,7 @@
     else fri_batch_poly(sh, 0, j, o, p);
     c[q] = sh.o[o].coeffs + b * sh.o[o].coeff_bstride + ((u64)p << sh.log_n);
   }
-  gl_cols sa[OP_POLYS], sb[OP_POLYS];
+  gl_cols4 sa[OP_POLYS], sb[OP_POLYS];
   for (u32 i = t; i < n; i += 256) {
     const u64 za = pa[i], zb = pb[i];
 #pragma unroll
@@ -165,7 +165,7 @@
   if (i >= n) return;
   const u64* pa = apw + b * apw_bstride;
   const u64* pb = pa + apw_len;
-  gl_cols sa, sb;
+  gl_cols4 sa, sb;
   u32 m = 0;
   const u32 zo = sh.zs_oracle, wz = sh.o[zo].w - sh.lookup_count;
   auto run = [&](u32 o, u32 first, u32 count) {
diff --git a/mapreduce-plonky2_amd/csrc/gates.h b/mapreduce-plonky2_amd/csrc/gates.h
--- a/mapreduce-plonky2_amd/csrc/gates.h
+++ b/mapreduce-plonky2_amd/csrc/gates.h
@@ -27,8 +27,8 @@
   return n_gates ? gate_table_check(out, num_constants, wires_w) : nullptr;
 }
 hipError_t gate_constraints_lde(hipStream_t s, u32 B, const GateTable& t, const u64* C, const u64* W, u64 w_bstride, u32 lg,
-                                const u64* apw, u32 nc, const u64* pi_hash, u64* q);
-hipError_t alpha_powers(hipStream_t s, u32 B, const u64* alphas, u64 al_bstride, u32 nc, u64* apw);
+                                const u64* apw, const gl_limbs* apw_limbs, u32 nc, const u64* pi_hash, u64* q);
+hipError_t alpha_powers(hipStream_t s, u32 B, const u64* alphas, u64 al_bstride, u32 nc, u64* powers, gl_limbs* limbs);
 hipError_t gate_constraints_points(hipStream_t s, const GateTable& t, const u64* consts, const u64* wires, u64 npts, u32 max_j,
                                    const u64* pi_hash, u64* out);
 hipError_t gate_constraints_points_batch(hipStream_t s, u32 B, const GateTable& t, const u64* consts, u64 c_bstride, const u64* wires,
diff --git a/mapreduce-plonky2_amd/csrc/gates.hip b/mapreduce-plonky2_amd/csrc/gates.hip
--- a/mapreduce-plonky2_amd/csrc/gates.hip
+++ b/mapreduce-plonky2_amd/csrc/gates.hip
@@ -113,7 +113,29 @@
   bool br = __builtin_sub_overflow(a, b, &r);
   return r - (br ? GL_EPS : 0);
 }
-typedef gl_cols LazySum;
+static_assert(MP2G_MAX_GATE_CONSTRAINTS <= GL_COLS_MAX_TERMS, "a gate's constraints must fit one gl_cols sum");
+template <bool MOVE_FREE> struct GateSum;
+template <> struct GateSum<true> {
+  typedef gl_cols Sum;
+  typedef gl_limbs Power;
+  static GLHD const Power* table(const u64*, const gl_limbs* limbs) { return limbs; }
+  static GLHD void add(Sum& s, u64 v, const Power& k) { s.add_limbs(v, k); }
+};
+template <> struct GateSum<false> {
+  typedef gl_cols4 Sum;
+  typedef u64 Power;
+  static GLHD const Power* table(const u64* powers, const gl_limbs*) { return powers; }
+  static GLHD void add(Sum& s, u64 v, const Power& k) { s.add(v, k); }
+};
+constexpr bool gate_sum_move_free(u32 kind) {
+  switch (kind) {
+    case MP2G_GATE_CONSTANT: case MP2G_GATE_PUBLIC_INPUT:
+    case MP2G_GATE_ARITHMETIC: case MP2G_GATE_BASE_SUM: case MP2G_GATE_ARITHMETIC_EXT: case MP2G_GATE_MUL_EXT: case MP2G_GATE_REDUCING:
+    case MP2G_GATE_REDUCING_EXT: case MP2G_GATE_RANDOM_ACCESS: case MP2G_GATE_POSEIDON: case MP2G_GATE_POSEIDON_MDS:
+    case MP2G_GATE_COSET_INTERPOLATION: return false;
+    default: return true;
+  }
+}
 template <int BITS, class WireF, class Emit>
 GLD void ra_copy(WireF& wire, Emit& emit, u32 w0, u32 b0) {
   constexpr int VS = 1 << BITS;
@@ -599,10 +621,12 @@
 template <u32 KIND>
 __global__ void __launch_bounds__(256) gate_constraints_lde_kernel(mp2g_gate g, u32 gi, u32 num_selectors, u32 cst_off, u32 n_cons,
                                                                    const u64* __restrict__ C, const u64* __restrict__ W,
-                                                                   u64 w_bstride, u32 lg, const u64* __restrict__ apw_tab,
-                                                                   u32 nc, const u64* __restrict__ pi_hash,
-                                                                   u64* __restrict__ q, int first) {
-  __shared__ u64 apw[2][MP2G_MAX_GATE_CONSTRAINTS];
+                                                                   u64 w_bstride, u32 lg, const u64* __restrict__ apw_powers,
+                                                                   const gl_limbs* __restrict__ apw_limbs, u32 nc,
+                                                                   const u64* __restrict__ pi_hash, u64* __restrict__ q, int first) {
+  typedef GateSum<gate_sum_move_free(KIND)> GS;
+  __shared__ typename GS::Power apw[2][MP2G_MAX_GATE_CONSTRAINTS];
+  const typename GS::Power* apw_tab = GS::table(apw_powers, apw_limbs);
   const u64 N = (u64)1 << lg;
   const u32 p = blockIdx.x * 256 + threadIdx.x, b = blockIdx.y;
   for (u32 j = threadIdx.x; j < 2 * n_cons; j += 256) {
@@ -624,18 +648,24 @@
       if (r != gi) f = gl_mul(f, gl_sub(r, s));
     if (num_selectors > 1) f = gl_mul(f, gl_sub(0xFFFFFFFFull, s));
   }
-  LazySum acc[2];
+  typename GS::Sum acc[2];
   u32 j = 0;
   eval_gate<true>(g, wire, cst, pih, [&](u64 v) {
 #pragma unroll
-    for (u32 a = 0; a < 2; a++) acc[a].add(v, apw[a][j]);
+    for (u32 a = 0; a < 2; a++) GS::add(acc[a], v, apw[a][j]);
     j++;
   });
   const u32 i = bitrev32(p, lg);
-  for (u32 a = 0; a < nc; a++) {
+  auto store = [&](u32 a) {
     u64 r = gl_mul(f, acc[a].value());
     u64* dst = q + (((u64)b * nc + a) << lg) + i;
     *dst = first ? r : gl_add(*dst, r);
+  };
+  if constexpr (gate_sum_move_free(KIND)) {
+    store(0);
+    if (nc > 1) store(1);
+  } else {
+    for (u32 a = 0; a < nc; a++) store(a);
   }
 }
 
@@ -654,10 +684,10 @@
 }
 __global__ void __launch_bounds__(256) gate_constraints_lde_light_kernel(LightGates lg_, u32 num_selectors, u32 cst_off, u32 max_cons,
                                                                          const u64* __restrict__ C, const u64* __restrict__ W,
-                                                                         u64 w_bstride, u32 lg, const u64* __restrict__ apw_tab,
+                                                                         u64 w_bstride, u32 lg, const gl_limbs* __restrict__ apw_tab,
                                                                          u32 nc, const u64* __restrict__ pi_hash,
                                                                          u64* __restrict__ q, int first) {
-  __shared__ u64 apw[2][MP2G_MAX_GATE_CONSTRAINTS];
+  __shared__ gl_limbs apw[2][MP2G_MAX_GATE_CONSTRAINTS];
   const u64 N = (u64)1 << lg;
   const u32 p = blockIdx.x * 256 + threadIdx.x, b = blockIdx.y;
   for (u32 j = threadIdx.x; j < 2 * max_cons; j += 256) {
@@ -682,11 +712,11 @@
         if (r != gi) f = gl_mul(f, gl_sub(r, s));
       if (num_selectors > 1) f = gl_mul(f, gl_sub(0xFFFFFFFFull, s));
     }
-    LazySum acc[2];
+    gl_cols acc[2];
     u32 j = 0;
     auto emit = [&](u64 v) {
 #pragma unroll
-      for (u32 a = 0; a < 2; a++) acc[a].add(v, apw[a][j]);
+      for (u32 a = 0; a < 2; a++) acc[a].add_limbs(v, apw[a][j]);
       j++;
     };
     switch (g.kind) {
@@ -700,7 +730,9 @@
 #undef LIGHT_CASE
       default: break;
     }
-    for (u32 a = 0; a < nc; a++) total[a] = gl_add(total[a], gl_mul(f, acc[a].value()));
+#pragma unroll
+    for (u32 a = 0; a < 2; a++)
+      if (a < nc) total[a] = gl_add(total[a], gl_mul(f, acc[a].value()));
   }
   const u32 i = bitrev32(p, lg);
   for (u32 a = 0; a < nc; a++) {
@@ -783,21 +815,24 @@
   return hipGetLastError();
 }
 
-__global__ void alpha_powers_kernel(const u64* __restrict__ alphas, u64 al_bstride, u32 nc, u32 B, u64* __restrict__ apw) {
+__global__ void alpha_powers_kernel(const u64* __restrict__ alphas, u64 al_bstride, u32 nc, u32 B, u64* __restrict__ powers,
+                                    gl_limbs* __restrict__ limbs) {
   const u32 t = blockIdx.x * blockDim.x + threadIdx.x;
   if (t >= B * 2 * MP2G_MAX_GATE_CONSTRAINTS) return;
   const u32 e = t % MP2G_MAX_GATE_CONSTRAINTS, a = (t / MP2G_MAX_GATE_CONSTRAINTS) & 1, b = t / (2 * MP2G_MAX_GATE_CONSTRAINTS);
-  apw[t] = a < nc ? gl_pow(alphas[b * al_bstride + a], e) : 0;
-}
-hipError_t alpha_powers(hipStream_t s, u32 B, const u64* alphas, u64 al_bstride, u32 nc, u64* apw) {
+  const u64 pw = a < nc ? gl_pow(alphas[b * al_bstride + a], e) : 0;
+  powers[t] = pw;
+  limbs[t] = gl_split(pw);
+}
+hipError_t alpha_powers(hipStream_t s, u32 B, const u64* alphas, u64 al_bstride, u32 nc, u64* powers, gl_limbs* limbs) {
   if (nc < 1 || nc > 2) return hipErrorInvalidValue;
   const u32 total = B * 2 * MP2G_MAX_GATE_CONSTRAINTS;
-  hipLaunchKernelGGL(alpha_powers_kernel, dim3((total + 255) / 256), dim3(256), 0, s, alphas, al_bstride, nc, B, apw);
+  hipLaunchKernelGGL(alpha_powers_kernel, dim3((total + 255) / 256), dim3(256), 0, s, alphas, al_bstride, nc, B, powers, limbs);
   return hipGetLastError();
 }
 
 hipError_t gate_constraints_lde(hipStream_t s, u32 B, const GateTable& t, const u64* C, const u64* W, u64 w_bstride, u32 lg,
-                                const u64* apw, u32 nc, const u64* pi_hash, u64* q) {
+                                const u64* apw, const gl_limbs* apw_limbs, u32 nc, const u64* pi_hash, u64* q) {
   if (nc < 1 || nc > 2) return hipErrorInvalidValue;
   const u64 N = (u64)1 << lg;
   const dim3 grid((u32)((N + 255) / 256), B), block(256);
@@ -814,7 +849,7 @@
   if (lgs.n < 2) lgs.n = 0;
   if (lgs.n) {
     hipLaunchKernelGGL(gate_constraints_lde_light_kernel, grid, block, 0, s, lgs, t.num_selectors, t.num_selectors + t.num_lookup_selectors,
-                       light_cons, C, W, w_bstride, lg, apw, nc, pi_hash, q, first);
+                       light_cons, C, W, w_bstride, lg, apw_limbs, nc, pi_hash, q, first);
     first = 0;
   }
   for (u32 gi = 0; gi < t.n_gates; gi++) {
@@ -827,8 +862,8 @@
 #define GATE_CASE(K)                                                                                                        \
   case K:                                                                                                                   \
     hipLaunchKernelGGL(gate_constraints_lde_kernel<K>, grid, block, 0, s, g, gi, t.num_selectors,                          \
-                       t.num_selectors + t.num_lookup_selectors, n_cons, C, W, w_bstride, lg, apw, nc, pi_hash, q,             \
-                       first);                                                                                              \
+                       t.num_selectors + t.num_lookup_selectors, n_cons, C, W, w_bstride, lg, apw, apw_limbs, nc, pi_hash,  \
+                       q, first);                                                                                              \
     break;
     switch (g.kind) {
       GATE_CASE(MP2G_GATE_CONSTANT)
diff --git a/mapreduce-plonky2_amd/csrc/gl.cuh b/mapreduce-plonky2_amd/csrc/gl.cuh
--- a/mapreduce-plonky2_amd/csrc/gl.cuh
+++ b/mapreduce-plonky2_amd/csrc/gl.cuh
@@ -179,7 +179,7 @@
   return gl_reduce128w(lo, hi);
 }
 
-struct gl_cols {
+struct gl_cols4 {
   u64 c0 = 0, c1 = 0, c2 = 0, c3 = 0;
   GLHD void add(u64 a, u64 b) {
     u64 pl, ph;
@@ -196,6 +196,50 @@
     return gl_sub(gl_reduce128(gl_mk((u32)c0, (u32)w1), gl_mk((u32)w2, (u32)w3)), (w3 >> 32) << 32);
   }
 };
+
+#define GL_COLS_MAX_TERMS 1024
+#define GL_LIMB_BITS 22
+#define GL_LIMB_MASK 0x3FFFFFu
+struct __attribute__((aligned(16))) gl_limbs { u32 k0, k1, k2, pad; };
+GLHD gl_limbs gl_split(u64 k) {
+  gl_limbs r;
+  r.k0 = (u32)k & GL_LIMB_MASK; r.k1 = (u32)(k >> GL_LIMB_BITS) & GL_LIMB_MASK; r.k2 = (u32)(k >> (2 * GL_LIMB_BITS)); r.pad = 0;
+  return r;
+}
+#if defined(__HIP_DEVICE_COMPILE__) || defined(GL_COLS_DEVICE_FORM)
+struct gl_cols {
+  u64 a00 = 0, a01 = 0, a02 = 0, a10 = 0, a11 = 0, a12 = 0;
+  GLHD void add_limbs(u64 c, u32 k0, u32 k1, u32 k2) {
+    const u64 cl = (u32)c, ch = c >> 32;
+    a00 += cl * k0; a01 += cl * k1; a02 += cl * k2;
+    a10 += ch * k0; a11 += ch * k1; a12 += ch * k2;
+  }
+  GLHD void add_limbs(u64 c, const gl_limbs& k) { add_limbs(c, k.k0, k.k1, k.k2); }
+  GLHD void add(u64 c, u64 k) {
+    add_limbs(c, (u32)k & GL_LIMB_MASK, (u32)(k >> GL_LIMB_BITS) & GL_LIMB_MASK, (u32)(k >> (2 * GL_LIMB_BITS)));
+  }
+  GLHD void add_scaled(u64 c, u64 k, u32 f) {
+    add_limbs(c, ((u32)k & GL_LIMB_MASK) * f, ((u32)(k >> GL_LIMB_BITS) & GL_LIMB_MASK) * f, (u32)(k >> (2 * GL_LIMB_BITS)) * f);
+  }
+  GLHD u64 value() const {
+    typedef unsigned __int128 u128;
+    const u128 lo = (u128)a00 + ((u128)a01 << GL_LIMB_BITS) + ((u128)a02 << (2 * GL_LIMB_BITS));
+    const u128 hi = (u128)a10 + ((u128)a11 << GL_LIMB_BITS) + ((u128)a12 << (2 * GL_LIMB_BITS));
+    const u64 h = gl_reduce128((u64)hi, (u64)(hi >> 64));
+    const u128 s = lo + ((u128)h << 32);
+    return gl_reduce128((u64)s, (u64)(s >> 64));
+  }
+  GLHD void flush(u64& partial) {
+    partial = gl_add(partial, value());
+    *this = gl_cols();
+  }
+};
+#else
+struct gl_cols : gl_cols4 {
+  GLHD void add_limbs(u64 c, u32 k0, u32 k1, u32 k2) { add(c, (u64)k0 + ((u64)k1 << GL_LIMB_BITS) + ((u64)k2 << (2 * GL_LIMB_BITS))); }
+  GLHD void add_limbs(u64 c, const gl_limbs& k) { add_limbs(c, k.k0, k.k1, k.k2); }
+};
+#endif
 
 struct gl2 { u64 a, b; };
 GLHD gl2 gl2_make(u64 a, u64 b) { gl2 r; r.a = a; r.b = b; return r; }
diff --git a/mapreduce-plonky2_amd/csrc/gl5.cuh b/mapreduce-plonky2_amd/csrc/gl5.cuh
--- a/mapreduce-plonky2_amd/csrc/gl5.cuh
+++ b/mapreduce-plonky2_amd/csrc/gl5.cuh
@@ -60,7 +60,7 @@
   gl5 r;
 #pragma unroll
   for (int i = 0; i < 5; i++) {
-    gl_cols acc;
+    gl_cols4 acc;
 #pragma unroll
     for (int j = 0; j < 5; j++) {
       if (j <= i) acc.add(a[j], b[i - j]); else acc.add(a3[j], b[i + 5 - j]);
@@ -77,7 +77,7 @@
   gl5 r;
 #pragma unroll
   for (int i = 0; i < 5; i++) {
-    gl_cols acc;
+    gl_cols4 acc;
 #pragma unroll
     for (int j = 0; j < 5; j++) {
 #pragma unroll
@@ -125,7 +125,7 @@
   gl5 q = gl5_mul(f12, f34);
   u64 n = 0;
   {
-    gl_cols acc;
+    gl_cols4 acc;
     acc.add(a.c[0], q.c[0]);
 #pragma unroll
     for (int j = 1; j < 5; j++) acc.add(gl_mul_small_w(a.c[j], 3), q.c[5 - j]);
diff --git a/mapreduce-plonky2_amd/csrc/prover.hip b/mapreduce-plonky2_amd/csrc/prover.hip
--- a/mapreduce-plonky2_amd/csrc/prover.hip
+++ b/mapreduce-plonky2_amd/csrc/prover.hip
@@ -34,7 +34,7 @@
   bool quotient = false;
   DevBuf pre_values, zs_values, chunk_q, bg, alphas, qvals;
   DevBuf ptab, qtab;
-  DevBuf apw;
+  DevBuf apw, apl;
   GateTable gates{};
   LookupDev lookups{};
   DevBuf lut_tables, lut_eval;
@@ -326,6 +326,7 @@
   NEED(P.log_n + 3 <= 24, "log_n <= 21");
   CK(pr->want(pr->qvals, (size_t)pr->Bcap * P.zs_count * ((size_t)8 << P.log_n) * sizeof(u64)));
   CK(pr->apw.alloc((size_t)pr->Bcap * 2 * MP2G_MAX_GATE_CONSTRAINTS * sizeof(u64)));
+  CK(pr->apl.alloc((size_t)pr->Bcap * 2 * MP2G_MAX_GATE_CONSTRAINTS * sizeof(gl_limbs)));
   CK(upload_table(pr->ctx, pr->qtab, quotient_table_words(P.log_n), [&](u64* h) { quotient_tables_host(P.log_n, h); }));
   pr->quotient = true;
   pr->drop_graph();
@@ -518,17 +519,17 @@
     }
     if (o == 3 && pr->quotient) {
       const u32 nc = P.zs_count;
-      CK(alpha_powers(s, B, pr->alphas.p, 2, nc, pr->apw.p));
+      CK(alpha_powers(s, B, pr->alphas.p, 2, nc, pr->apw.p, (gl_limbs*)pr->apl.p));
       if (pr->gates.n_gates)
-        CK(gate_constraints_lde(s, B, pr->gates, pr->values[0].p, pr->values[1].p, (u64)P.oracle_w[1] * N, P.log_n + 3, pr->apw.p, nc,
-                                (const u64*)d_pi_hash, pr->qvals.p));
+        CK(gate_constraints_lde(s, B, pr->gates, pr->values[0].p, pr->values[1].p, (u64)P.oracle_w[1] * N, P.log_n + 3, pr->apw.p,
+                                (const gl_limbs*)pr->apl.p, nc, (const u64*)d_pi_hash, pr->qvals.p));
       if (pr->lookups.n_luts)
         CK(quotient_lookup_values(s, B, pr->lookups, pr->values[0].p, pr->gates.num_selectors, pr->values[1].p, (u64)P.oracle_w[1] * N,
                                   pr->values[2].p, (u64)P.oracle_w[2] * N, nc * (pr->num_routed / pr->degree), P.log_n, pr->bg.p, 8,
                                   pr->lut_eval.p, pr->alphas.p, 2, nc, pr->qvals.p));
       CK(quotient_perm_values(s, B, pr->values[1].p, (u64)P.oracle_w[1] * N, pr->values[0].p + (u64)(P.oracle_w[0] - pr->num_routed) * N,
                               pr->values[2].p, (u64)P.oracle_w[2] * N, P.log_n, pr->num_routed, pr->degree, pr->bg.p, 8,
-                              pr->apw.p, MP2G_MAX_GATE_CONSTRAINTS, nc, pr->gates.n_gates != 0, pr->ptab.p, pr->qtab.p, pr->qvals.p));
+                              (const gl_limbs*)pr->apl.p, MP2G_MAX_GATE_CONSTRAINTS, nc, pr->gates.n_gates != 0, pr->ptab.p, pr->qtab.p, pr->qvals.p));
       CK(c->ntt.run(pr->qvals.p, pr->coeffs[3].p, P.log_n + 3, B * nc, 0, N, N, true, nullptr, false));
       CK(c->ntt.scale_table(pr->coeffs[3].p, P.log_n + 3, B * nc, pr->qtab.p + quotient_unshift_offset(P.log_n)));
       CK(commit_oracle_coeffs(pr, 3, B));
diff --git a/mapreduce-plonky2_amd/csrc/verifier.hip b/mapreduce-plonky2_amd/csrc/verifier.hip
--- a/mapreduce-plonky2_amd/csrc/verifier.hip
+++ b/mapreduce-plonky2_amd/csrc/verifier.hip
@@ -166,7 +166,7 @@
   }
   const u64* gv = gate_vals + (u64)b * sh.max_j * sh.T;
   for (u32 j = 0; j < sh.max_j; j++) {
-    gl_cols c0, c1;
+    gl_cols4 c0, c1;
     for (u32 t = 0; t < sh.T; t++) {
       const u64 v = gv[j * sh.T + t];
       c0.add(v, interp[t]);
diff --git a/mapreduce-plonky2_amd/csrc/zperm.h b/mapreduce-plonky2_amd/csrc/zperm.h
--- a/mapreduce-plonky2_amd/csrc/zperm.h
+++ b/mapreduce-plonky2_amd/csrc/zperm.h
@@ -10,7 +10,7 @@
                        u32 degree, const u64* betas, const u64* gammas, u64 chal_bstride, u32 nc, const u64* ptab, u64* chunk_q,
                        u64* out, u64 out_bstride);
 hipError_t quotient_perm_values(hipStream_t s, u32 B, const u64* W, u64 w_bstride, const u64* S, const u64* Z, u64 z_bstride,
-                                u32 log_n, u32 num_routed, u32 degree, const u64* bg, u64 bg_bstride, const u64* apw, u32 apw_len,
+                                u32 log_n, u32 num_routed, u32 degree, const u64* bg, u64 bg_bstride, const gl_limbs* apw, u32 apw_len,
                                 u32 nc, bool gates, const u64* ptab, const u64* qtab, u64* q);
 hipError_t zpp_wrap_check(hipStream_t s, u32 B, const u64* chunk_q, const u64* zs, u64 zs_bstride, u32 log_n, u32 chunks, u32 nc,
                           u32* flags);
diff --git a/mapreduce-plonky2_amd/csrc/zperm.hip b/mapreduce-plonky2_amd/csrc/zperm.hip
--- a/mapreduce-plonky2_amd/csrc/zperm.hip
+++ b/mapreduce-plonky2_amd/csrc/zperm.hip
@@ -85,7 +85,7 @@
 __global__ void __launch_bounds__(256) quotient_perm_kernel(const u64* __restrict__ W, u64 w_bstride, const u64* __restrict__ S,
                                                             const u64* __restrict__ Z, u64 z_bstride, u32 log_n, u32 num_routed,
                                                             u32 degree, const u64* __restrict__ bg, u64 bg_bstride,
-                                                            const u64* __restrict__ apw, u32 apw_len, u32 nc, bool gates,
+                                                            const gl_limbs* __restrict__ apw, u32 apw_len, u32 nc, bool gates,
                                                             const u64* __restrict__ ptab, const u64* __restrict__ qtab,
                                                             u64* __restrict__ q) {
   const u32 lg = log_n + 3;
@@ -95,7 +95,7 @@
   const u32 chunks = num_routed / degree, num_prods = chunks - 1, n_terms = nc * (1 + chunks);
   __shared__ u64 zh_inv[8];
   __shared__ u64 kis[ZP_MAX_ROUTED];
-  __shared__ u64 al[2][ZP_MAX_TERMS + 1];
+  __shared__ gl_limbs al[2][ZP_MAX_TERMS + 1];
   if (threadIdx.x < 8) zh_inv[threadIdx.x] = qtab[2 * N + threadIdx.x];
   for (u32 e = threadIdx.x; e < 2 * (n_terms + 1); e += 256) {
     const u32 a = e / (n_terms + 1), k = e % (n_terms + 1);
@@ -108,10 +108,13 @@
   const u64* w = W + b * w_bstride + p;
   const u64* sg = S + p;
   const u64* z = Z + b * z_bstride;
+  static_assert(ZP_MAX_TERMS + 1 <= GL_COLS_MAX_TERMS, "the vanishing terms must fit one gl_cols sum");
   gl_cols acc[2];
   u32 kt = 0;
   auto push = [&](u64 term) {
-    for (u32 a = 0; a < nc; a++) acc[a].add(term, al[a][kt]);
+#pragma unroll
+    for (u32 a = 0; a < 2; a++)
+      if (a < nc) acc[a].add_limbs(term, al[a][kt]);
     kt++;
   };
   for (u32 c = 0; c < nc; c++) push(gl_mul(l0, gl_sub(z[((u64)c << lg) + p], 1)));
@@ -134,12 +137,15 @@
       prev = next;
     }
   }
-  if (gates)
-    for (u32 a = 0; a < nc; a++) acc[a].add(q[(((u64)b * nc + a) << lg) + i], al[a][n_terms]);
-  for (u32 a = 0; a < nc; a++) q[(((u64)b * nc + a) << lg) + i] = gl_mul(acc[a].value(), zh_inv[i & 7]);
+#pragma unroll
+  for (u32 a = 0; a < 2; a++) {
+    if (a >= nc) break;
+    if (gates) acc[a].add_limbs(q[(((u64)b * nc + a) << lg) + i], al[a][n_terms]);
+    q[(((u64)b * nc + a) << lg) + i] = gl_mul(acc[a].value(), zh_inv[i & 7]);
+  }
 }
 hipError_t quotient_perm_values(hipStream_t s, u32 B, const u64* W, u64 w_bstride, const u64* S, const u64* Z, u64 z_bstride,
-                                u32 log_n, u32 num_routed, u32 degree, const u64* bg, u64 bg_bstride, const u64* apw, u32 apw_len,
+                                u32 log_n, u32 num_routed, u32 degree, const u64* bg, u64 bg_bstride, const gl_limbs* apw, u32 apw_len,
                                 u32 nc, bool gates, const u64* ptab, const u64* qtab, u64* q) {
   if (nc < 1 || nc > 2 || !degree || num_routed % degree || num_routed > ZP_MAX_ROUTED || num_routed / degree > ZP_MAX_CHUNKS ||
       apw_len < nc * (1 + num_routed / degree) + 1)
```

Result: no change. 929.4 (median of 6 runs) (+0.4%).
